# thanard/me-trpo

Measured on AMD Instinct MI355X. Metric: imagined env-steps/sec (KxBxH) over the full TRPO iteration, higher is better.
Workload: dtype f32

## Files before the change

include/metrpo.h:

```cpp
#ifndef METRPO_H
#define METRPO_H

#include <stddef.h>
#include <stdint.h>

#ifdef __cplusplus
extern "C" {
#endif

#define METRPO_ABI_VERSION 4
#define METRPO_MAX_LAYERS 6

typedef struct metrpo_ctx metrpo_ctx;

typedef enum {
    METRPO_OK = 0,
    METRPO_EINVAL = -1,
    METRPO_ENULL = -2,
    METRPO_EHIP = -3,
    METRPO_EUNSUPPORTED = -4,
    METRPO_ESTATE = -5,
    METRPO_UNSET = -100
} metrpo_status;

// ... 24 lines not shown
    int32_t pol_n_hidden;
    int32_t pol_hidden[METRPO_MAX_LAYERS];
} metrpo_dims;

int32_t metrpo_abi_version(void);
const char* metrpo_status_string(int32_t status);

int32_t metrpo_create(metrpo_ctx** out, int32_t device, const metrpo_dims* dims);
int32_t metrpo_destroy(metrpo_ctx* ctx);
int32_t metrpo_set_exclusive(metrpo_ctx* ctx, int32_t exclusive);
int32_t metrpo_set_option(metrpo_ctx* ctx, const char* key, const char* value);
int32_t metrpo_get_option(metrpo_ctx* ctx, const char* key, char* buf, int32_t cap);
const char* metrpo_option_name(int32_t index);
const char* metrpo_last_error(const metrpo_ctx* ctx);
int32_t metrpo_dyn_param_count(const metrpo_ctx* ctx);
int32_t metrpo_policy_param_count(const metrpo_ctx* ctx);

int32_t metrpo_set_dynamics(metrpo_ctx* ctx, const float* d_params, const float* d_in_mean,
                            const float* d_in_std, const float* d_diff_mean, const float* d_diff_std,
                            void* stream);
int32_t metrpo_set_policy(metrpo_ctx* ctx, const float* d_theta, void* stream);
int32_t metrpo_get_policy(metrpo_ctx* ctx, float* d_theta_out, void* stream);

int32_t metrpo_policy_actions(metrpo_ctx* ctx, const float* d_obs, const float* d_eps, int32_t B,
                              float* d_actions, float* d_mean, void* stream);
int32_t metrpo_step(metrpo_ctx* ctx, const float* d_s, const float* d_a, int32_t B, int32_t sam_mode,
                    const int32_t* d_model_idx, const float* d_noise, float* d_s_next, float* d_reward,
                    uint8_t* d_done, float* d_next_all, void* stream);

typedef struct {
    int32_t B, T, H;
    int32_t sam_mode;
    int32_t determ;
    int32_t eval_all_heads;
    const float* d_pool;
    int32_t n_pool;
    uint64_t seed;
    uint64_t stream_offset;
    const float* d_eps;
    const int32_t* d_model_idx;
    const float* d_sel_noise;
    const int32_t* d_reset_idx;
    const int32_t* d_reset_model;
    float* d_obs;
    float* d_act;
    float* d_rew;
    float* d_mean;
    uint8_t* d_done;
    int32_t* d_tpath;
    float* d_last_obs;
    int32_t t0;
    const float* d_init_obs;
    const int32_t* d_init_ts;
    const int32_t* d_init_model;
    int32_t* d_last_ts;
    int32_t* d_last_model;
    const int32_t* d_stop;
    int64_t stop_batch;
    const double* d_stop_cum;
} metrpo_rollout_args;
int32_t metrpo_rollout(metrpo_ctx* ctx, const metrpo_rollout_args* args, void* stream);
int32_t metrpo_last_rollout_kernel(const metrpo_ctx* ctx);
const char* metrpo_rollout_note(const metrpo_ctx* ctx);

typedef enum { METRPO_DYN_F32 = 0, METRPO_DYN_BF16 = 1 } metrpo_dyn_precision;
int32_t metrpo_set_dyn_precision(metrpo_ctx* ctx, int32_t precision);
int32_t metrpo_get_dyn_precision(const metrpo_ctx* ctx);

int32_t metrpo_sampler_progress(metrpo_ctx* ctx, const uint8_t* d_done, const int32_t* d_tpath, int32_t T, int32_t B,
                                int32_t t0, int64_t batch_size, double* d_counts, double* d_state, int32_t* d_stop,
                                void* stream);

int32_t metrpo_validation_cost(metrpo_ctx* ctx, const float* d_s0, int32_t Bv, int32_t T, double gamma,
                               double* d_costs, void* stream);

int32_t metrpo_gae(metrpo_ctx* ctx, const float* d_obs, const float* d_rew, const uint8_t* d_done,
                   const int32_t* d_tpath, int32_t T, int32_t B, const double* d_coeffs, double gamma,
                   double lam, float* d_adv, float* d_ret, uint8_t* d_valid, double* d_stats, void* stream);
int32_t metrpo_process_begin(metrpo_ctx* ctx, float* d_old_log_std, double* d_acc, int64_t n_acc, void* stream);
int32_t metrpo_center_advantages(metrpo_ctx* ctx, float* d_adv, const uint8_t* d_valid, int64_t N,
                                 const double* d_stats, void* stream);
int32_t metrpo_baseline_gram(metrpo_ctx* ctx, const float* d_obs, const float* d_ret, const int32_t* d_tpath,
                             const uint8_t* d_valid, int64_t N, double* d_AtA, double* d_Aty, void* stream);
int32_t metrpo_baseline_solve(metrpo_ctx* ctx, const double* d_AtA, const double* d_Aty, double reg_coeff, double* d_coeffs, void* stream);

typedef struct {
    const float* d_obs;
    const float* d_act;
    const float* d_adv;
    const float* d_old_mean;
    const float* d_old_log_std;
    int32_t old_log_std_stride;
    const uint8_t* d_valid;
    int64_t N;
    double inv_n_global;
} metrpo_batch;

int32_t metrpo_loss_grad(metrpo_ctx* ctx, const metrpo_batch* batch, double* d_out, void* stream);
int32_t metrpo_fvp(metrpo_ctx* ctx, const metrpo_batch* batch, const double* d_v, double* d_hv, void* stream);
int32_t metrpo_loss_kl(metrpo_ctx* ctx, const metrpo_batch* batch, const float* d_theta, double* d_out,
                       void* stream);

int32_t metrpo_vpg_loss_grad(metrpo_ctx* ctx, const metrpo_batch* batch, double* d_out, void* stream);
typedef struct {
    double lr, beta1, beta2, eps;
} metrpo_vpg_params;
int32_t metrpo_vpg_update(metrpo_ctx* ctx, const metrpo_batch* batch, const metrpo_vpg_params* params, double* d_loss, void* stream);

typedef struct {
    double clip_lr, entropy_bonus_coeff;
    double lr, beta1, beta2, eps;
} metrpo_ppo_params;
int32_t metrpo_ppo_loss_grad(metrpo_ctx* ctx, const metrpo_batch* batch, const metrpo_ppo_params* params, double* d_out, void* stream);
int32_t metrpo_ppo_update(metrpo_ctx* ctx, const metrpo_batch* batch, const metrpo_ppo_params* params, int32_t n_epochs, double* d_losses, void* stream);

typedef struct { double kl_penalty, step_size; } metrpo_ppo_kl_params;
int32_t metrpo_ppo_kl_loss_grad(metrpo_ctx* ctx, const metrpo_batch* batch, const metrpo_ppo_params* params, const metrpo_ppo_kl_params* kl,
                                const double* d_mean_kl, double* d_out, void* stream);
int32_t metrpo_ppo_kl_update(metrpo_ctx* ctx, const metrpo_batch* batch, const metrpo_ppo_params* params, const metrpo_ppo_kl_params* kl, int32_t n_epochs,
                             double* d_losses, double* d_mean_kls, void* stream);

#define METRPO_COMM_ID_BYTES 128
int32_t metrpo_comm_get_unique_id(void* id_out );
int32_t metrpo_comm_init(metrpo_ctx* ctx, const void* id , int32_t world, int32_t rank);
int32_t metrpo_comm_destroy(metrpo_ctx* ctx);
int32_t metrpo_allreduce_sum_f64(metrpo_ctx* ctx, double* d_buf, int64_t count, void* stream);

#define METRPO_COMM_IPC_BLOB_BYTES 128
int32_t metrpo_comm_ipc_export(metrpo_ctx* ctx, void* blob_out );
int32_t metrpo_comm_ipc_attach(metrpo_ctx* ctx, const void* blobs , int32_t world, int32_t rank);
int32_t metrpo_comm_ipc_detach(metrpo_ctx* ctx);
int32_t metrpo_comm_set_timeout_ms(metrpo_ctx* ctx, int64_t ms);
int32_t metrpo_comm_transport(const metrpo_ctx* ctx);
int32_t metrpo_comm_check(metrpo_ctx* ctx, void* stream);

typedef int32_t (*metrpo_allreduce_fn)(void* user, double* d_buf, int64_t count, void* stream);

typedef struct {
    double max_kl;
    int32_t cg_iters;
    double reg_coeff;
    double backtrack_ratio;
    int32_t max_backtracks;
    int32_t accept_violation;
    double residual_tol;
    metrpo_allreduce_fn allreduce;
    void* allreduce_user;
    int32_t explicit_final_hvp;
} metrpo_trpo_params;

typedef struct {
    double loss_before, loss, kl, beta;
    int32_t n_backtrack, accepted, cg_iters_run;
} metrpo_trpo_diag;

int32_t metrpo_trpo_update(metrpo_ctx* ctx, const metrpo_batch* batch, const metrpo_trpo_params* params,
                           metrpo_trpo_diag* diag, double* d_g_out, double* d_dir_out, void* stream);

int32_t metrpo_trpo_update_begin(metrpo_ctx* ctx, const metrpo_batch* batch, const metrpo_trpo_params* params, int32_t spec_trials,
                                 double* d_g_out, double* d_dir_out, void* stream);
int32_t metrpo_trpo_update_end(metrpo_ctx* ctx, metrpo_trpo_diag* diag, int32_t* late_out, void* stream);

int32_t metrpo_subsample_batch(metrpo_ctx* ctx, const metrpo_batch* batch, const int32_t* d_idx, int64_t m, double inv_n_global, metrpo_batch* out,
                               double* d_valid_count, void* stream);
int32_t metrpo_trpo_update_fvp(metrpo_ctx* ctx, const metrpo_batch* batch, const metrpo_batch* fvp_batch, const metrpo_trpo_params* params,
                               metrpo_trpo_diag* diag, double* d_g_out, double* d_dir_out, void* stream);
// ... 88 lines not shown
```

me-trpo_amd/_lib.py:

```python
import ctypes as C
import os

import torch

_HERE = os.path.dirname(os.path.abspath(__file__))
LIB_PATH = os.path.join(_HERE, "libmetrpo.so")
MAX_LAYERS = 6

ENV_IDS = {'swimmer': 0, 'half_cheetah': 1, 'half-cheetah': 1, 'ant': 2, 'humanoid': 3, 'hopper': 4, 'snake': 5}
SAM_MODES = {'step_rand': 0, 'eps_rand': 1, 'model_mean_std': 2, 'model_mean': 3, 'model_med': 4, 'one_model': 5}
DYN_PRECISIONS = {'f32': 0, 'bf16': 1}
ACTS = {'identity': 0, 'tf.identity': 0, 'relu': 1, 'tf.nn.relu': 1, 'tanh': 2, 'tf.nn.tanh': 2, 'tf.tanh': 2}


class Dims(C.Structure):
    _fields_ = [('env', C.c_int32), ('ns', C.c_int32), ('na', C.c_int32), ('n_models', C.c_int32),
                ('dyn_n_hidden', C.c_int32), ('dyn_hidden', C.c_int32 * MAX_LAYERS), ('dyn_act', C.c_int32 * MAX_LAYERS),
                ('n_drop', C.c_int32), ('pol_n_hidden', C.c_int32), ('pol_hidden', C.c_int32 * MAX_LAYERS)]


class RolloutArgs(C.Structure):
    _fields_ = [('B', C.c_int32), ('T', C.c_int32), ('H', C.c_int32), ('sam_mode', C.c_int32), ('determ', C.c_int32),
                ('eval_all_heads', C.c_int32), ('d_pool', C.c_void_p), ('n_pool', C.c_int32), ('seed', C.c_uint64),
                ('stream_offset', C.c_uint64), ('d_eps', C.c_void_p), ('d_model_idx', C.c_void_p),
# ... 21 lines not shown
                ('explicit_final_hvp', C.c_int32)]


class TrainParams(C.Structure):
    _fields_ = [('lr', C.c_double), ('beta1', C.c_double), ('beta2', C.c_double), ('eps', C.c_double),
                ('reg_constant', C.c_double), ('batch_size', C.c_int32)]


class TrpoDiag(C.Structure):
    _fields_ = [('loss_before', C.c_double), ('loss', C.c_double), ('kl', C.c_double), ('beta', C.c_double),
                ('n_backtrack', C.c_int32), ('accepted', C.c_int32), ('cg_iters_run', C.c_int32)]


class VpgParams(C.Structure):
    _fields_ = [('lr', C.c_double), ('beta1', C.c_double), ('beta2', C.c_double), ('eps', C.c_double)]


class PpoParams(C.Structure):
    _fields_ = [('clip_lr', C.c_double), ('entropy_bonus_coeff', C.c_double), ('lr', C.c_double), ('beta1', C.c_double), ('beta2', C.c_double),
                ('eps', C.c_double)]


class PpoKlParams(C.Structure):
    _fields_ = [('kl_penalty', C.c_double), ('step_size', C.c_double)]


class LbfgsOpts(C.Structure):
    _fields_ = [('m', C.c_int32), ('maxls', C.c_int32), ('maxiter', C.c_int32), ('maxfun', C.c_int32), ('ftol', C.c_double),
                ('gtol', C.c_double), ('lookahead', C.c_int32), ('round_f32', C.c_int32)]


class LbfgsResult(C.Structure):
    _fields_ = [('fun', C.c_double), ('nit', C.c_int32), ('nfev', C.c_int32), ('status', C.c_int32), ('task', C.c_int32),
                ('task_code', C.c_int32), ('pad_', C.c_int32)]


class ModelErrorArgs(C.Structure):
    _fields_ = [('d_Os', C.c_void_p), ('d_As', C.c_void_p), ('d_Rs', C.c_void_p), ('n', C.c_int32), ('T', C.c_int32),
                ('hs', C.POINTER(C.c_int32)), ('n_h', C.c_int32), ('model', C.c_int32), ('known_actions', C.c_int32), ('t0_only', C.c_int32),
                ('signed_diff', C.c_int32), ('d_state_diff', C.c_void_p), ('d_cost_diff', C.c_void_p), ('d_valid', C.c_void_p), ('d_sums', C.c_void_p),
                ('d_dbg_obs', C.c_void_p), ('d_dbg_rew', C.c_void_p), ('d_dbg_done', C.c_void_p), ('d_dbg_last_obs', C.c_void_p)]


class RolloutActionsArgs(C.Structure):
    _fields_ = [('B', C.c_int32), ('T', C.c_int32), ('sam_mode', C.c_int32), ('uniform_model', C.c_int32), ('force_step_loop', C.c_int32),
                ('d_init_obs', C.c_void_p), ('d_actions', C.c_void_p), ('d_model', C.c_void_p), ('d_model_idx', C.c_void_p), ('d_sel_noise', C.c_void_p),
                ('d_obs', C.c_void_p), ('d_rew', C.c_void_p), ('d_done', C.c_void_p)]


MODEL_ERROR_MAX_HORIZONS = 32


_P, _I, _L, _D = C.c_void_p, C.c_int32, C.c_int64, C.c_double
SYMBOLS = {
    'metrpo_abi_version': (_I, []),
    'metrpo_status_string': (C.c_char_p, [_I]),
    'metrpo_create': (_I, [C.POINTER(_P), _I, C.POINTER(Dims)]),
    'metrpo_destroy': (_I, [_P]),
    'metrpo_last_error': (C.c_char_p, [_P]),
    'metrpo_dyn_param_count': (_I, [_P]),
    'metrpo_policy_param_count': (_I, [_P]),
    'metrpo_set_dynamics': (_I, [_P, _P, _P, _P, _P, _P, _P]),
    'metrpo_set_policy': (_I, [_P, _P, _P]),
    'metrpo_get_policy': (_I, [_P, _P, _P]),
    'metrpo_policy_actions': (_I, [_P, _P, _P, _I, _P, _P, _P]),
    'metrpo_step': (_I, [_P, _P, _P, _I, _I, _P, _P, _P, _P, _P, _P, _P]),
    'metrpo_rollout': (_I, [_P, C.POINTER(RolloutArgs), _P]),
    'metrpo_comm_get_unique_id': (_I, [_P]),
    'metrpo_comm_init': (_I, [_P, _P, _I, _I]),
    'metrpo_comm_destroy': (_I, [_P]),
    'metrpo_allreduce_sum_f64': (_I, [_P, _P, _L, _P]),
    'metrpo_comm_ipc_export': (_I, [_P, _P]),
    'metrpo_comm_ipc_attach': (_I, [_P, _P, _I, _I]),
    'metrpo_comm_ipc_detach': (_I, [_P]),
    'metrpo_comm_set_timeout_ms': (_I, [_P, _L]),
    'metrpo_comm_transport': (_I, [_P]),
    'metrpo_comm_check': (_I, [_P, _P]),
    'metrpo_sampler_progress': (_I, [_P, _P, _P, _I, _I, _I, _L, _P, _P, _P, _P]),
    'metrpo_validation_cost': (_I, [_P, _P, _I, _I, _D, _P, _P]),
    'metrpo_gae': (_I, [_P, _P, _P, _P, _P, _I, _I, _P, _D, _D, _P, _P, _P, _P, _P]),
    'metrpo_process_begin': (_I, [_P, _P, _P, _L, _P]),
    'metrpo_center_advantages': (_I, [_P, _P, _P, _L, _P, _P]),
    'metrpo_baseline_gram': (_I, [_P, _P, _P, _P, _P, _L, _P, _P, _P]),
    'metrpo_baseline_solve': (_I, [_P, _P, _P, _D, _P, _P]),
    'metrpo_loss_grad': (_I, [_P, C.POINTER(Batch), _P, _P]),
    'metrpo_fvp': (_I, [_P, C.POINTER(Batch), _P, _P, _P]),
    'metrpo_loss_kl': (_I, [_P, C.POINTER(Batch), _P, _P, _P]),
    'metrpo_vpg_loss_grad': (_I, [_P, C.POINTER(Batch), _P, _P]),
    'metrpo_vpg_update': (_I, [_P, C.POINTER(Batch), C.POINTER(VpgParams), _P, _P]),
    'metrpo_ppo_loss_grad': (_I, [_P, C.POINTER(Batch), C.POINTER(PpoParams), _P, _P]),
    'metrpo_ppo_update': (_I, [_P, C.POINTER(Batch), C.POINTER(PpoParams), C.c_int32, _P, _P]),
    'metrpo_ppo_kl_loss_grad': (_I, [_P, C.POINTER(Batch), C.POINTER(PpoParams), C.POINTER(PpoKlParams), _P, _P, _P]),
    'metrpo_ppo_kl_update': (_I, [_P, C.POINTER(Batch), C.POINTER(PpoParams), C.POINTER(PpoKlParams), C.c_int32, _P, _P, _P]),
    'metrpo_trpo_update': (_I, [_P, C.POINTER(Batch), C.POINTER(TrpoParams), C.POINTER(TrpoDiag), _P, _P, _P]),
    'metrpo_trpo_update_begin': (_I, [_P, C.POINTER(Batch), C.POINTER(TrpoParams), _I, _P, _P, _P]),
    'metrpo_trpo_update_end': (_I, [_P, C.POINTER(TrpoDiag), C.POINTER(C.c_int32), _P]),
    'metrpo_subsample_batch': (_I, [_P, C.POINTER(Batch), _P, _L, _D, C.POINTER(Batch), _P, _P]),
    'metrpo_trpo_update_fvp': (_I, [_P, C.POINTER(Batch), C.POINTER(Batch), C.POINTER(TrpoParams), C.POINTER(TrpoDiag), _P, _P, _P]),
    'metrpo_trpo_update_fvp_begin': (_I, [_P, C.POINTER(Batch), C.POINTER(Batch), C.POINTER(TrpoParams), _I, _P, _P, _P]),
    'metrpo_model_error_windows': (_I, [_P, _P, _I, _I, _P, _P]),
    'metrpo_model_error': (_I, [_P, C.POINTER(ModelErrorArgs), _P]),
    'metrpo_rollout_actions': (_I, [_P, C.POINTER(RolloutActionsArgs), _P]),
    'metrpo_last_rollout_actions_kernel': (_I, [_P]),
    'metrpo_dyn_train_reset': (_I, [_P, _P]),
    'metrpo_dyn_train_step': (_I, [_P, _P, _P, C.POINTER(TrainParams), _P, _P]),
    'metrpo_dyn_eval_losses': (_I, [_P, _P, _P, _L, _D, _P, _P]),
    'metrpo_get_dynamics': (_I, [_P, _P, _P]),
    'metrpo_set_dynamics_model': (_I, [_P, _I, _P, _P]),
    'metrpo_set_normalizers': (_I, [_P, _P, _P, _P, _P, _P]),
    'metrpo_rms_accumulate': (_I, [_P, _P, _L, _I, _P, _P, _P]),
    'metrpo_bptt_grad': (_I, [_P, _P, _I, _I, _D, _P, _P, _P]),
    'metrpo_bptt_grad_stochastic': (_I, [_P, _P, _I, _I, _D, _P, C.c_uint64, _P, _P, _P, _P]),
    'metrpo_set_exclusive': (_I, [_P, _I]),
    'metrpo_set_option': (_I, [_P, C.c_char_p, C.c_char_p]),
    'metrpo_get_option': (_I, [_P, C.c_char_p, C.c_char_p, _I]),
    'metrpo_option_name': (C.c_char_p, [_I]),
    'metrpo_last_rollout_kernel': (_I, [_P]),
    'metrpo_rollout_note': (C.c_char_p, [_P]),
    'metrpo_set_dyn_precision': (_I, [_P, _I]),
    'metrpo_get_dyn_precision': (_I, [_P]),
    'metrpo_policy_adam_reset': (_I, [_P, _P]),
    'metrpo_policy_adam_step': (_I, [_P, _P, _D, _D, _D, _D, _D, _P]),
    'metrpo_lbfgs_begin': (_I, [_P, _I, _P, C.POINTER(LbfgsOpts), _P, _P]),
    'metrpo_lbfgs_iterate': (_I, [_P, _P, _P, _P, _P, _P]),
    'metrpo_lbfgs_get_result': (_I, [_P, C.POINTER(LbfgsResult), _P]),
    'metrpo_lbfgs_policy': (_I, [_P, _P, _I, _I, _D, C.POINTER(LbfgsOpts), C.POINTER(LbfgsResult), _P]),
    'metrpo_get_dyn_adam': (_I, [_P, _P, _P, C.POINTER(_L), _P]),
    'metrpo_set_dyn_adam': (_I, [_P, _P, _P, _L, _P]),
    'metrpo_get_policy_adam': (_I, [_P, _P, _P, C.POINTER(_L), _P]),
    'metrpo_set_policy_adam': (_I, [_P, _P, _P, _L, _P]),
}
EXTRA_SYMBOLS = {
    'metrpo_rollout_generic': (_I, [_P, C.POINTER(RolloutArgs), _P]),
    'metrpo_has_mfma_path': (_I, [_P]),
    'metrpo_set_update_path': (_I, [_P, _I]),
    'metrpo_update_path': (_I, [_P, _L]),
    'metrpo_set_rollout_variant': (_I, [_P, _I]),
    'metrpo_set_det_path': (_I, [_P, _I]),
    'metrpo_probe_peaks': (_I, [_P, _P, _P]),
    'metrpo_schedulable_cus': (_I, [_P, _P]),
    'metrpo_debug_fvp_us': (_I, [_P, _P, _P]),
    'metrpo_debug_last_update': (_I, [_P, _P]),
    'metrpo_debug_persist_stats': (_I, [_P, _P, _I, _P]),
    'metrpo_debug_ws_retired': (_I, [_P, _P, _I]),
}


def load():
    if not os.path.exists(LIB_PATH):
        raise ImportError("libmetrpo.so not found at %s -- build it with `python -c 'import __graft_entry__ as g; "
                          "g.build()'` (hipcc --offload-arch=gfx950); there is no CPU fallback" % LIB_PATH)
    lib = C.CDLL(LIB_PATH)
    for table in (SYMBOLS, EXTRA_SYMBOLS):
        for name, (res, args) in table.items():
            fn = getattr(lib, name)
            fn.restype, fn.argtypes = res, args
    if lib.metrpo_abi_version() != 4:
        raise ImportError("libmetrpo.so ABI version mismatch")
    return lib


lib = load()


class MetrpoError(RuntimeError):
    pass
# ... 9 lines not shown
```

me-trpo_amd/csrc/api.hip:

```cpp
#include "metrpo_internal.h"
#include <atomic>
#include <chrono>
#include <cstring>
#include "cg_device.h"
#include "trace.h"
#include <algorithm>
#include <cmath>
#include <cstring>
#include <mutex>
#include <new>

static std::mutex g_err_mutex;
int set_err(metrpo_ctx* c, int code, const std::string& msg) {
    if (c) { std::lock_guard<std::mutex> lock(g_err_mutex); c->err = msg; }
    return code;
}

extern "C" int32_t metrpo_abi_version(void) { return METRPO_ABI_VERSION; }

extern "C" const char* metrpo_status_string(int32_t s) {
    switch (s) {
    case METRPO_OK: return "ok";
    case METRPO_EINVAL: return "invalid argument";
    case METRPO_ENULL: return "null pointer";
// ... 370 lines not shown

extern "C" int32_t metrpo_sampler_progress(metrpo_ctx* c, const uint8_t* done, const int32_t* tpath, int32_t T, int32_t B, int32_t t0,
                                           int64_t batch_size, double* counts, double* state, int32_t* stop, void* stream) {
    if (!c) return METRPO_ENULL;
    if (!done || !tpath || !counts || !state || !stop) return set_err(c, METRPO_ENULL, "sampler_progress: NULL pointer");
    if (T < 0 || B < 0 || t0 < 0 || batch_size < 0) return set_err(c, METRPO_EINVAL, "sampler_progress: bad T/B/t0/batch_size");
    if (T == 0 || B == 0) return METRPO_OK;
    return launch_sampler_progress(c, done, tpath, T, B, t0, batch_size, counts, state, stop, (hipStream_t)stream);
}

extern "C" int32_t metrpo_rollout_generic(metrpo_ctx* c, const metrpo_rollout_args* a, void* stream) {
    if (!c) return METRPO_ENULL;
    if (!a) return set_err(c, METRPO_ENULL, "rollout: args NULL");
    NEED_DYN(c); NEED_POL(c);
    if (!sam_ok(a->sam_mode)) return set_err(c, METRPO_EINVAL, "sam mode is not defined");
    if (a->B <= 0 || a->T <= 0 || a->H <= 0 || a->n_pool <= 0) return set_err(c, METRPO_EINVAL, "rollout: bad B/T/H/n_pool");
    if (!a->d_pool || !a->d_obs || !a->d_act || !a->d_rew || !a->d_mean || !a->d_done || !a->d_tpath)
        return set_err(c, METRPO_ENULL, "rollout: required pointer is NULL");
    return launch_rollout_generic(c, a, (hipStream_t)stream);
}
extern "C" int32_t metrpo_has_mfma_path(const metrpo_ctx* c) { return (c && c->mfma_cfg >= 0) ? 1 : 0; }
extern "C" int32_t metrpo_set_rollout_variant(metrpo_ctx* c, int32_t v) {
    if (!c) return METRPO_ENULL;
    c->rollout_variant = v;
    return (v != 1 && (c->coop_cfg >= 0 || (v == 0 && c->coop_pad_cfg >= 0))) ? 2 : (c->mfma_cfg >= 0 ? 1 : (gemm_path_applicable(c) ? 3 : 0));
}
extern "C" int32_t metrpo_update_path(const metrpo_ctx* c, int64_t N) {
    if (!c) return METRPO_ENULL;
    return policy_gemm_applicable(c, N, false) ? 2 : ((c->pol_mfma >= 0 || f3_active(c, false)) ? 1 : 0);
}
extern "C" int32_t metrpo_set_update_path(metrpo_ctx* c, int32_t use_mfma) {
    if (!c) return METRPO_ENULL;
    c->pol_path = (use_mfma == 2) ? 2 : (use_mfma ? 1 : 0);
    c->pol_mfma = (use_mfma == 1) ? policy_mfma_select(c->pd) : -1;
    c->pol_f3 = (use_mfma == 1) ? policy_f3_select(c->pd) : 0;
    c->pg_fwd_rows = -1; c->f3_rows = -1;
    return (c->pol_mfma >= 0 || f3_active(c, false)) ? 1 : (c->pol_path == 2 ? 2 : 0);
}

extern "C" int32_t metrpo_validation_cost(metrpo_ctx* c, const float* s0, int32_t Bv, int32_t T, double gamma,
                                          double* costs, void* stream) {
    TraceRange trace_("metrpo:validation_cost");
    if (!c) return METRPO_ENULL;
    NEED_DYN(c); NEED_POL(c);
    if (!s0 || !costs) return set_err(c, METRPO_ENULL, "validation_cost: NULL pointer");
    if (Bv <= 0 || T < 0) return set_err(c, METRPO_EINVAL, "validation_cost: bad Bv/T");
    return launch_validation_cost(c, s0, Bv, T, gamma, costs, (hipStream_t)stream);
}

extern "C" int32_t metrpo_gae(metrpo_ctx* c, const float* obs, const float* rew, const uint8_t* done,
                              const int32_t* tpath, int32_t T, int32_t B, const double* coeffs, double gamma, double lam,
                              float* adv, float* ret, uint8_t* valid, double* stats, void* stream) {
    TraceRange trace_("metrpo:process_samples:gae");
    if (!c) return METRPO_ENULL;
    if (!obs || !rew || !done || !tpath || !adv || !ret || !valid || !stats) return set_err(c, METRPO_ENULL, "gae: NULL pointer");
    if (T < 0 || B < 0) return set_err(c, METRPO_EINVAL, "gae: bad T/B");
    if (T == 0 || B == 0) return METRPO_OK;
    return launch_gae(c, obs, rew, done, tpath, T, B, coeffs, gamma, lam, adv, ret, valid, stats, (hipStream_t)stream);
}

extern "C" int32_t metrpo_process_begin(metrpo_ctx* c, float* old_log_std, double* acc, int64_t n_acc, void* stream) {
    TraceRange trace_("metrpo:process_samples:begin");
    if (!c) return METRPO_ENULL;
    if (n_acc < 0 || n_acc > (1LL << 30) || (n_acc > 0 && !acc)) return set_err(c, METRPO_EINVAL, "process_begin: bad accumulator range");
    if (!old_log_std && n_acc == 0) return METRPO_OK;
    return launch_process_begin(c, old_log_std, n_acc > 0 ? acc : nullptr, n_acc, (hipStream_t)stream);
}

extern "C" int32_t metrpo_center_advantages(metrpo_ctx* c, float* adv, const uint8_t* valid, int64_t N,
                                            const double* stats, void* stream) {
    TraceRange trace_("metrpo:process_samples:center");
    if (!c) return METRPO_ENULL;
    if (!adv || !stats) return set_err(c, METRPO_ENULL, "center: NULL pointer");
    if (N <= 0) return METRPO_OK;
    return launch_center(c, adv, valid, N, stats, (hipStream_t)stream);
}

extern "C" int32_t metrpo_baseline_gram(metrpo_ctx* c, const float* obs, const float* ret, const int32_t* tpath,
                                        const uint8_t* valid, int64_t N, double* AtA, double* Aty, void* stream) {
    TraceRange trace_("metrpo:process_samples:baseline_gram");
    if (!c) return METRPO_ENULL;
    if (!obs || !ret || !tpath || !AtA || !Aty) return set_err(c, METRPO_ENULL, "gram: NULL pointer");
    if (N <= 0) return METRPO_OK;
    return launch_gram(c, obs, ret, tpath, valid, N, AtA, Aty, (hipStream_t)stream);
}

extern "C" int32_t metrpo_baseline_solve(metrpo_ctx* c, const double* AtA, const double* Aty, double reg_coeff, double* coeffs, void* stream) {
    TraceRange trace_("metrpo:process_samples:baseline_solve");
    if (!c) return METRPO_ENULL;
    if (!AtA || !Aty || !coeffs) return set_err(c, METRPO_ENULL, "baseline_solve: NULL pointer");
    if (!(reg_coeff >= 0.0)) return set_err(c, METRPO_EINVAL, "baseline_solve: reg_coeff must be >= 0");
    return launch_baseline_solve(c, AtA, Aty, reg_coeff, coeffs, (hipStream_t)stream);
}

extern "C" int32_t metrpo_loss_grad(metrpo_ctx* c, const metrpo_batch* b, double* out, void* stream) {
    if (!c) return METRPO_ENULL;
    NEED_POL(c);
    if (!out) return set_err(c, METRPO_ENULL, "loss_grad: out NULL");
    return launch_loss_grad(c, b, out, (hipStream_t)stream);
}
extern "C" int32_t metrpo_vpg_loss_grad(metrpo_ctx* c, const metrpo_batch* b, double* out, void* stream) {
    if (!c) return METRPO_ENULL;
    if (!out) return set_err(c, METRPO_ENULL, "vpg_loss_grad: out NULL");
    NEED_POL(c);
    return launch_vpg_loss_grad(c, b, out, (hipStream_t)stream);
}
extern "C" int32_t metrpo_vpg_update(metrpo_ctx* c, const metrpo_batch* b, const metrpo_vpg_params* pr, double* d_loss, void* stream) {
    if (!c) return METRPO_ENULL;
    if (!pr) return set_err(c, METRPO_ENULL, "vpg_update: params NULL");
    NEED_POL(c);
    if (c->upd_pending) return set_err(c, METRPO_ESTATE, "vpg_update: a TRPO update is still open (metrpo_trpo_update_end first)");
    return run_vpg_update(c, b, pr, d_loss, (hipStream_t)stream);
}
extern "C" int32_t metrpo_ppo_loss_grad(metrpo_ctx* c, const metrpo_batch* b, const metrpo_ppo_params* pr, double* out, void* stream) {
    if (!c) return METRPO_ENULL;
    if (!pr) return set_err(c, METRPO_ENULL, "ppo_loss_grad: params NULL");
    if (!out) return set_err(c, METRPO_ENULL, "ppo_loss_grad: out NULL");
    NEED_POL(c);
    return launch_ppo_loss_grad(c, b, pr, out, (hipStream_t)stream);
}
extern "C" int32_t metrpo_ppo_update(metrpo_ctx* c, const metrpo_batch* b, const metrpo_ppo_params* pr, int32_t n_epochs, double* d_losses, void* stream) {
    if (!c) return METRPO_ENULL;
    if (!pr) return set_err(c, METRPO_ENULL, "ppo_update: params NULL");
    NEED_POL(c);
    if (c->upd_pending) return set_err(c, METRPO_ESTATE, "ppo_update: a TRPO update is still open (metrpo_trpo_update_end first)");
    return run_ppo_update(c, b, pr, n_epochs, d_losses, (hipStream_t)stream);
}
extern "C" int32_t metrpo_ppo_kl_loss_grad(metrpo_ctx* c, const metrpo_batch* b, const metrpo_ppo_params* pr, const metrpo_ppo_kl_params* kp, const double* d_mean_kl,
                                           double* out, void* stream) {
    if (!c) return METRPO_ENULL;
    if (!pr || !kp) return set_err(c, METRPO_ENULL, "ppo_kl_loss_grad: params NULL");
    if (!out) return set_err(c, METRPO_ENULL, "ppo_kl_loss_grad: out NULL");
    NEED_POL(c);
    return launch_ppo_kl_loss_grad(c, b, pr, kp, d_mean_kl, out, (hipStream_t)stream);
}
extern "C" int32_t metrpo_ppo_kl_update(metrpo_ctx* c, const metrpo_batch* b, const metrpo_ppo_params* pr, const metrpo_ppo_kl_params* kp, int32_t n_epochs, double* d_losses,
                                        double* d_mean_kls, void* stream) {
    if (!c) return METRPO_ENULL;
    if (!pr || !kp) return set_err(c, METRPO_ENULL, "ppo_kl_update: params NULL");
    NEED_POL(c);
    if (c->upd_pending) return set_err(c, METRPO_ESTATE, "ppo_kl_update: a TRPO update is still open (metrpo_trpo_update_end first)");
    return run_ppo_kl_update(c, b, pr, kp, n_epochs, d_losses, d_mean_kls, (hipStream_t)stream);
}
static int lbfgs_opts_check(metrpo_ctx* c, const metrpo_lbfgs_opts* o, const char* who) {
    if (!o) return set_err(c, METRPO_ENULL, std::string(who) + ": opts NULL");
    if (o->m <= 0 || o->maxls <= 0) return set_err(c, METRPO_EINVAL, std::string(who) + ": m and maxls must be positive");
    if (!(o->ftol >= 0.0) || !(o->gtol >= 0.0)) return set_err(c, METRPO_EINVAL, std::string(who) + ": ftol and gtol must be >= 0");
    return METRPO_OK;
}
extern "C" int32_t metrpo_lbfgs_begin(metrpo_ctx* c, int32_t n, const double* x0, const metrpo_lbfgs_opts* o, double* x_eval, void* stream) {
    if (!c) return METRPO_ENULL;
    if (!x0 || !x_eval) return set_err(c, METRPO_ENULL, "lbfgs_begin: NULL pointer");
    if (n <= 0) return set_err(c, METRPO_EINVAL, "lbfgs_begin: n must be positive");
    int rc;
    if ((rc = lbfgs_opts_check(c, o, "lbfgs_begin"))) return rc;
    return lbfgs_begin(c, n, x0, nullptr, o, x_eval, (hipStream_t)stream);
}
extern "C" int32_t metrpo_lbfgs_iterate(metrpo_ctx* c, const double* f, const double* g, double* x_eval, int32_t* task, void* stream) {
    if (!c) return METRPO_ENULL;
    if (!f || !g || !x_eval || !task) return set_err(c, METRPO_ENULL, "lbfgs_iterate: NULL pointer");
    if (!c->lb_open) return set_err(c, METRPO_ESTATE, "lbfgs_iterate: no minimisation open (metrpo_lbfgs_begin first)");
    return lbfgs_iterate(c, f, g, x_eval, task, (hipStream_t)stream);
}
extern "C" int32_t metrpo_lbfgs_get_result(metrpo_ctx* c, metrpo_lbfgs_result* out, void* stream) {
    if (!c) return METRPO_ENULL;
    if (!out) return set_err(c, METRPO_ENULL, "lbfgs_get_result: out NULL");
    if (!c->lb_open) return set_err(c, METRPO_ESTATE, "lbfgs_get_result: no minimisation open (metrpo_lbfgs_begin first)");
// ... 536 lines not shown
```

me-trpo_amd/csrc/cg_device.h:

```cpp
#pragma once
#include "metrpo_internal.h"
#ifndef CG_MARK
#define CG_MARK(i)
#endif

enum { S_RDOTR = 0, S_DONE = 1, S_BETA = 2, S_XHX = 3, S_ITERS = 4, S_LOSS0 = 5, S_COMMERR = 6, S_ROLLERR = 7 };

struct CgTail {
    int op;
    int P, last;
    int implicit_hd;
    double reg, tol, max_kl;
    double *x, *r, *p, *z, *step, *scal;
    const double* gout;
    float* pf;
    const int* vpos; float* imgval;
    unsigned int* ticket;
    double* ls;
    const double* lk;
    float* th; const float* th_try;
    int trial, accept_violation;
    double* pub_dst;
    unsigned long long pub_stamp;
    float* nx_try = nullptr; const float* nx_prev = nullptr; double nx_ratio = 1.0; double* nx_ls = nullptr;
};

struct PfOut {
    float* pf; const int* vpos; float* imgval;
    __device__ __forceinline__ void put(int i, float v) const { pf[i] = v; if (vpos != nullptr) { const int q = vpos[i]; if (q >= 0) imgval[q] = v; } }
};
__device__ __forceinline__ void cg_init_body(int P, const double* gout, double* x, double* r, double* p, PfOut pf, double* scal, double* sh);

template <int CTRL> __device__ __forceinline__ double dpp_add_f64(double v) {
    const long long b = __double_as_longlong(v);
    const int lo = __builtin_amdgcn_update_dpp(0, (int)b, CTRL, 0xF, 0xF, true), hi = __builtin_amdgcn_update_dpp(0, (int)(b >> 32), CTRL, 0xF, 0xF, true);
    return v + __longlong_as_double(((long long)hi << 32) | (unsigned int)lo);
}
__device__ __forceinline__ double wave_sum_f64(double v) {
    v = dpp_add_f64<0xB1>(v); v = dpp_add_f64<0x4E>(v); v = dpp_add_f64<0x141>(v); v = dpp_add_f64<0x140>(v);
    const long long b = __double_as_longlong(v);
    double t = 0.0;
#pragma unroll
    for (int r = 0; r < 4; ++r) {
        const int lo = __builtin_amdgcn_readlane((int)b, 16 * r), hi = __builtin_amdgcn_readlane((int)(b >> 32), 16 * r);
        t += __longlong_as_double(((long long)hi << 32) | (unsigned int)lo);
    }
    return t;
}
__device__ __forceinline__ double blk_sum(double v, double* sh) {
    v = wave_sum_f64(v);
    const int w = threadIdx.x >> 6, l = threadIdx.x & 63;
    __syncthreads();
    if (l == 0) sh[w] = v;
    __syncthreads();
    double r = 0.0;
    const int nw = (blockDim.x + 63) >> 6;
    for (int i = 0; i < nw; ++i) r += sh[i];
    return r;
}

__device__ __forceinline__ void cg_finish_implicit(int P, double max_kl, const double* x, const double* r, const double* g,
                                                   double* step, double* scal, double* sh) {
    double acc = 0.0;
    for (int i = threadIdx.x; i < P; i += blockDim.x) acc += x[i] * (g[i] - r[i]);
    const double xhx = blk_sum(acc, sh);
    double beta = sqrt(2.0 * max_kl * (1.0 / (xhx + 1e-8)));
    if (isnan(beta)) beta = 1.0;
    for (int i = threadIdx.x; i < P; i += blockDim.x) step[i] = beta * x[i];
    if (threadIdx.x == 0) { scal[S_BETA] = beta; scal[S_XHX] = xhx; }
}

__device__ __forceinline__ void cg_init_body(int P, const double* gout, double* x, double* r, double* p, PfOut pf, double* scal, double* sh) {
    double acc = 0.0;
    for (int i = threadIdx.x; i < P; i += blockDim.x) {
        const double g = gout[1 + i];
        x[i] = 0.0; r[i] = g; p[i] = g; pf.put(i, (float)g);
        acc += g * g;
    }
    const double rdotr = blk_sum(acc, sh);
    if (threadIdx.x == 0) { scal[S_RDOTR] = rdotr; scal[S_DONE] = 0.0; scal[S_ITERS] = 0.0; scal[S_LOSS0] = gout[0]; }
}

constexpr int CG_R = 2;
constexpr int CG_RBIG = 13;
struct CgPre { double pv[CG_R], rv[CG_R], xv[CG_R], done, rdotr; bool have; };
__device__ __forceinline__ void cg_prefetch(const CgTail& t, CgPre& pre) {
    pre.have = (t.op == 1 && t.P <= CG_R * (int)blockDim.x);
    if (!pre.have) return;
    pre.done = t.scal[S_DONE]; pre.rdotr = t.scal[S_RDOTR];
// ... 17 lines not shown
            pv[j] = zv[j] = rv[j] = xv[j] = 0.0;
            const int ic = (i < P) ? i : P - 1;
            const double pl = pf_ ? 0.0 : p[ic], rl = pf_ ? 0.0 : r[ic], xl = pf_ ? 0.0 : x[ic], zl = z[ic];
            if (i < P) {
                if (pf_) { pv[j] = pre->pv[j < CG_R ? j : 0]; rv[j] = pre->rv[j < CG_R ? j : 0]; xv[j] = pre->xv[j < CG_R ? j : 0]; } else { pv[j] = pl; rv[j] = rl; xv[j] = xl; }
                zv[j] = zl + reg * pv[j]; acc += pv[j] * zv[j];
            }
        }
        CG_MARK(5)
        const double pz = blk_sum(acc, sh);
        CG_MARK(6)
        const double v = rdotr / pz;
        acc = 0.0;
#pragma unroll
        for (int j = 0; j < R; ++j) { xv[j] += v * pv[j]; rv[j] -= v * zv[j]; acc += rv[j] * rv[j]; }
        const double newrdotr = blk_sum(acc, sh);
        CG_MARK(7)
        const double mu = newrdotr / rdotr;
#pragma unroll
        for (int j = 0; j < R; ++j) {
            const int i = threadIdx.x + j * blockDim.x;
            if (i < P) {
                const double pn = rv[j] + mu * pv[j];
                z[i] = zv[j]; x[i] = xv[j]; r[i] = rv[j]; p[i] = pn;
                pf.put(i, last ? (float)xv[j] : (float)pn);
            }
        }
        __syncthreads();
        if (threadIdx.x == 0) {
            scal[S_RDOTR] = newrdotr;
            scal[S_ITERS] += 1.0;
            if (newrdotr < tol) scal[S_DONE] = 1.0;
        }
        }

__device__ __forceinline__ void cg_step_body(int P, double reg, double tol, int last, double* x, double* r, double* p, double* z,
                                             PfOut pf, double* scal, double* sh, const CgPre* pre = nullptr) {
    const bool pf_ = (pre != nullptr && pre->have);
    if ((pf_ ? pre->done : scal[S_DONE]) != 0.0) {
        if (last) for (int i = threadIdx.x; i < P; i += blockDim.x) pf.put(i, (float)x[i]);
        return;
    }
    const double rdotr = pf_ ? pre->rdotr : scal[S_RDOTR];
    if (P <= CG_R * (int)blockDim.x) { cg_step_regs<CG_R>(P, reg, tol, last, x, r, p, z, pf, scal, sh, rdotr, pre); return; }
    if (P <= 4 * (int)blockDim.x) { cg_step_regs<4>(P, reg, tol, last, x, r, p, z, pf, scal, sh, rdotr, nullptr); return; }
    if (P <= CG_RBIG * (int)blockDim.x) { cg_step_regs<CG_RBIG>(P, reg, tol, last, x, r, p, z, pf, scal, sh, rdotr, nullptr); return; }
    double acc = 0.0;
    for (int i = threadIdx.x; i < P; i += blockDim.x) { const double zi = z[i] + reg * p[i]; z[i] = zi; acc += p[i] * zi; }
    const double pz = blk_sum(acc, sh);
    const double v = rdotr / pz;
    acc = 0.0;
    for (int i = threadIdx.x; i < P; i += blockDim.x) {
        x[i] += v * p[i];
        const double ri = r[i] - v * z[i];
        r[i] = ri;
        acc += ri * ri;
    }
    const double newrdotr = blk_sum(acc, sh);
    const double mu = newrdotr / rdotr;
    for (int i = threadIdx.x; i < P; i += blockDim.x) {
        const double pn = r[i] + mu * p[i];
        p[i] = pn;
        pf.put(i, last ? (float)x[i] : (float)pn);
    }
    __syncthreads();
    if (threadIdx.x == 0) {
        scal[S_RDOTR] = newrdotr;
        scal[S_ITERS] += 1.0;
        if (newrdotr < tol) scal[S_DONE] = 1.0;
    }
}

__device__ __forceinline__ void cg_finish_body(int P, double reg, double max_kl, const double* x, double* z, double* step,
                                               double* scal, double* sh) {
    double acc = 0.0;
    for (int i = threadIdx.x; i < P; i += blockDim.x) acc += x[i] * (z[i] + reg * x[i]);
    const double xhx = blk_sum(acc, sh);
    double beta = sqrt(2.0 * max_kl * (1.0 / (xhx + 1e-8)));
    if (isnan(beta)) beta = 1.0;
    for (int i = threadIdx.x; i < P; i += blockDim.x) step[i] = beta * x[i];
    if (threadIdx.x == 0) { scal[S_BETA] = beta; scal[S_XHX] = xhx; }
}

__device__ __forceinline__ void ls_decide(const CgTail& t) {
    const double loss = t.lk[0], kl = t.lk[1], lb = t.scal[S_LOSS0];
    if (loss < lb && kl <= t.max_kl) {
        const bool acc = !(isnan(loss) || isnan(kl) || loss >= lb || kl >= t.max_kl) || t.accept_violation != 0;
        if (acc) for (int i = threadIdx.x; i < t.P; i += blockDim.x) t.th[i] = t.th_try[i];
        if (threadIdx.x == 0) { t.ls[0] = (double)t.trial; t.ls[1] = loss; t.ls[2] = kl; t.ls[3] = acc ? 1.0 : 0.0; }
    } else if (threadIdx.x == 0) { t.ls[1] = loss; t.ls[2] = kl; }
}

__device__ __forceinline__ void ls_next_theta(const CgTail& t) {
    for (int i = threadIdx.x; i < t.P; i += blockDim.x) t.nx_try[i] = (float)((double)t.nx_prev[i] - t.nx_ratio * t.step[i]);
}
__device__ __forceinline__ void ls_open_and_first_theta(const CgTail& t) {
    if (t.nx_try == nullptr) return;
    __syncthreads();
    if (t.nx_ls != nullptr && threadIdx.x == 0) { t.nx_ls[0] = -1.0; t.nx_ls[1] = NAN; t.nx_ls[2] = NAN; t.nx_ls[3] = 0.0; }
    ls_next_theta(t);
}

__device__ __forceinline__ void ls_publish(const double* __restrict__ src, double* dst, unsigned long long stamp) {
    if (threadIdx.x >= 64) return;
    if (threadIdx.x < 14) __hip_atomic_store(dst + threadIdx.x, src[threadIdx.x], __ATOMIC_RELAXED, __HIP_MEMORY_SCOPE_SYSTEM);
    asm volatile("s_waitcnt vmcnt(0)" ::: "memory");
    if (threadIdx.x == 0) __hip_atomic_store((unsigned long long*)(dst + 16), stamp, __ATOMIC_RELAXED, __HIP_MEMORY_SCOPE_SYSTEM);
}

__device__ __forceinline__ void cg_tail_run(const CgTail& t, double* sh, const CgPre* pre = nullptr) {
    if (t.op == 1) {
        cg_step_body(t.P, t.reg, t.tol, t.last, t.x, t.r, t.p, t.z, PfOut{t.pf, t.vpos, t.imgval}, t.scal, sh, pre);
        if (t.last && t.implicit_hd) {
            __syncthreads();
            cg_finish_implicit(t.P, t.max_kl, t.x, t.r, t.gout + 1, t.step, t.scal, sh);
            ls_open_and_first_theta(t);
        }
    } else if (t.op == 2) { cg_finish_body(t.P, t.reg, t.max_kl, t.x, t.z, t.step, t.scal, sh); ls_open_and_first_theta(t); }
    else if (t.op == 3) cg_init_body(t.P, t.gout, t.x, t.r, t.p, PfOut{t.pf, t.vpos, t.imgval}, t.scal, sh);
    else if (t.op == 4) {
        ls_decide(t);
        if (t.nx_try != nullptr && !(t.lk[0] < t.scal[S_LOSS0] && t.lk[1] <= t.max_kl)) ls_next_theta(t);
        if (t.pub_dst != nullptr) { asm volatile("s_waitcnt vmcnt(0)" ::: "memory"); __syncthreads(); ls_publish(t.scal, t.pub_dst, t.pub_stamp); }
    }
}
```

me-trpo_amd/csrc/metrpo_internal.h:

```cpp
#pragma once
#include <hip/hip_runtime.h>
#include <stdint.h>
#include <string>
#include <atomic>
#include <utility>
#include <vector>
#include "metrpo.h"
#include "xchg_device.h"

#define MAXL (METRPO_MAX_LAYERS + 1)
#define WAVE 64

struct NetDesc {
    int n_layers;
    int dims[MAXL + 1];
    int act[MAXL];
    int w_off[MAXL];
    int b_off[MAXL];
    int n_params;
    int api_w_off[MAXL];
    int api_b_off[MAXL];
    int api_n_params;
    int max_width;
};
// ... 131 lines not shown
struct RolloutK {
    int B, T, H, sam_mode, determ, eval_all, n_pool;
    uint64_t seed, stream_offset;
    const float* pool;
    const float* eps;
    const int32_t* model_idx;
    const float* sel_noise;
    const int32_t* reset_idx;
    const int32_t* reset_model;
    float* obs; float* act; float* rew; float* mean; uint8_t* done; int32_t* tpath; float* last_obs;
    int t0; const float* init_obs; const int32_t* init_ts; const int32_t* init_model;
    int32_t* last_ts; int32_t* last_model; const int32_t* stop;
    long long stop_batch; const double* stop_cum;
    int32_t* mig_flag; float* mig_obs; int32_t* mig_ts; int32_t* mig_model; int mig_epoch; double* mig_err;
    int vB, vR;
};
#define RK_ENV(r, b) ((r).vB ? (b) % (r).vB : (b))
#define RK_TOFF(r, b) ((r).vB ? ((b) / (r).vB) * (r).H : 0)
#define RK_STRIDE(r) ((r).vB ? (r).vB : (r).B)
#define RK_LAST_ROUND(r, b) (!(r).vB || (b) / (r).vB == (r).vR - 1)

static inline RolloutK make_rollout_k(const metrpo_rollout_args* a) {
    RolloutK r;
    r.B = a->B; r.T = a->T; r.H = a->H; r.sam_mode = a->sam_mode; r.determ = a->determ; r.eval_all = a->eval_all_heads;
    r.n_pool = a->n_pool; r.seed = a->seed; r.stream_offset = a->stream_offset; r.pool = a->d_pool; r.eps = a->d_eps;
    r.model_idx = a->d_model_idx; r.sel_noise = a->d_sel_noise; r.reset_idx = a->d_reset_idx;
    r.reset_model = a->d_reset_model; r.obs = a->d_obs; r.act = a->d_act; r.rew = a->d_rew; r.mean = a->d_mean;
    r.done = a->d_done; r.tpath = a->d_tpath; r.last_obs = a->d_last_obs;
    r.t0 = a->t0; r.init_obs = a->d_init_obs; r.init_ts = a->d_init_ts; r.init_model = a->d_init_model;
    r.last_ts = a->d_last_ts; r.last_model = a->d_last_model; r.stop = a->d_stop;
    r.stop_batch = a->stop_batch; r.stop_cum = a->d_stop_cum;
    r.mig_flag = nullptr; r.mig_obs = nullptr; r.mig_ts = nullptr; r.mig_model = nullptr; r.mig_epoch = 0; r.mig_err = nullptr;
    r.vB = 0; r.vR = 0;
    return r;
}

struct PolK {
    const float* obs; const float* act; const float* adv; const float* old_mean; const float* old_ls;
    int ls_stride;
    float clip_lo;
    const uint8_t* valid; long long N; float inv_n;
    float clip_hi;
    const float* gm;
    const int* img_map;
    const double* skip;
    float* imgval;
    float* hcache;
    const double* mean_kl; double kl_delta; float kl_beta;
};

enum UpdOp {
    OP_GRAD = 0,
    OP_FVP = 1,
    OP_LOSSKL = 2,
    OP_FVPC = 3,
    OP_VPG = 4,
    OP_PPO = 5,
    OP_PPOKL = 6,
};
struct SolveScope {
    bool cache_activations = false;
    bool publish_image = false;
    bool exchange_in_tail = false;
};
struct CgTail;
struct AdamTail;
struct UpdCall {
    UpdOp op;
    PolK k;
    const float* theta;
    const float* vf;
    const double* v64;
    double* out;
    const CgTail* tail;
    const AdamTail* adam;
    double ent_coeff;
    bool ent_in_reduction;
    SolveScope scope;
};

int policy_mfma_select(const ProblemDesc& pd);
int policy_mfma_image_buffers(metrpo_ctx*);
int policy_mfma_launch(metrpo_ctx*, const UpdCall&, float* partials, int nblocks, hipStream_t);

#define HIP_TRY(c, expr)                                                                      \
    do {                                                                                      \
        hipError_t _e = (expr);                                                               \
        if (_e != hipSuccess)                                                                 \
            return set_err((c), METRPO_EHIP, std::string(#expr) + ": " + hipGetErrorString(_e)); \
    } while (0)

int launch_policy_actions(metrpo_ctx*, const float*, const float*, int, float*, float*, hipStream_t);
int launch_step(metrpo_ctx*, const float*, const float*, int, int, const int32_t*, const float*, float*, float*,
                uint8_t*, float*, hipStream_t);
int launch_rollout_generic(metrpo_ctx*, const metrpo_rollout_args*, hipStream_t);
bool gemm_path_applicable(const metrpo_ctx*);
int sched_cus(metrpo_ctx*, hipStream_t);
bool grid_is_coresident(metrpo_ctx*, const void* kernel, int threads, size_t lds, long long grid, hipStream_t);
int launch_rollout_gemm(metrpo_ctx*, const metrpo_rollout_args*, hipStream_t);
struct Bf16Img { int Kp[MAXL]; size_t off[MAXL]; size_t per_head; };
Bf16Img bf16_img_layout(const ProblemDesc&);
int launch_bf16_dyn_image(metrpo_ctx*, hipStream_t);
size_t bf16_hidden_floats(const ProblemDesc&, int B);
int launch_bf16_layers(metrpo_ctx*, const float* X, int ldx, void* HA, void* HB, float* OUT, int B, hipStream_t);
int launch_rollout_resident(metrpo_ctx*, const metrpo_rollout_args*, hipStream_t);
struct BpttNoise {
    const float* eps;
    const float* log_std;
    int* n_sat;
    unsigned long long seed;
    int T;
};
int launch_bptt_grad(metrpo_ctx*, const float* init, int B, int T, double gamma, double* costs, double* grad, hipStream_t, const BpttNoise* nz = nullptr);
int launch_policy_adam(metrpo_ctx*, const double* grad, double lr, double b1, double b2, double eps, double clip_val, bool reset, hipStream_t);
int ensure_policy_adam(metrpo_ctx*);
int ensure_dyn_adam(metrpo_ctx*);
size_t dyn_adam_floats(const metrpo_ctx*);
int det_mfma_select(const metrpo_ctx*);
int launch_det_forward(metrpo_ctx*, int idx, const float* s0, int B, int T, double gamma, float* XS, float* WT, double* part, double* costs, hipStream_t,
                       const BpttNoise* nz = nullptr);
int launch_det_backward(metrpo_ctx*, int idx, int B, int T, const float* XS, const float* WT, float* GM, hipStream_t, const BpttNoise* nz = nullptr);
int ensure_detpart(metrpo_ctx*, int B);
int ensure_detpart_n(metrpo_ctx*, size_t n_doubles);
int launch_det_cost_reduce(metrpo_ctx*, int n_part, const double* part, double* costs, hipStream_t, const double* err = nullptr);
int launch_validation_resident(metrpo_ctx*, const float* s0, int Bv, int T, double gamma, double* costs, hipStream_t);
bool det_gemm_applicable(const metrpo_ctx*);
int launch_dg_forward(metrpo_ctx*, const float* s0, int B, int T, double gamma, float* XS, float* WT, double* costs, hipStream_t,
                      const BpttNoise* nz = nullptr);
int launch_dg_backward(metrpo_ctx*, int B, int T, const float* XS, const float* WT, float* GM, hipStream_t, const BpttNoise* nz = nullptr);
int launch_policy_vjp(metrpo_ctx*, const float* obs, const float* gm, long long N, double* out, hipStream_t);
int launch_dyn_train_step(metrpo_ctx*, const float*, const float*, const metrpo_train_params*, double*, hipStream_t);
int launch_dyn_eval_losses(metrpo_ctx*, const float*, const float*, long long, double, double*, hipStream_t);
int launch_rms_accumulate(metrpo_ctx*, const float*, long long, int, double*, double*, hipStream_t);
int launch_rollout_mfma(metrpo_ctx*, const metrpo_rollout_args*, hipStream_t, int* coop = nullptr);
int mfma_prepare_dynamics(metrpo_ctx*, hipStream_t);
int mfma_prepare_policy(metrpo_ctx*, hipStream_t);
int mfma_select_config(metrpo_ctx*);
int mfma_shape_config(const metrpo_ctx*);
int coop_select_config(metrpo_ctx*);
int launch_rollout_coop(metrpo_ctx*, int idx, const RolloutK&, hipStream_t, bool padded = false);
int launch_pad_dyn(metrpo_ctx*, hipStream_t);
int launch_validation_cost(metrpo_ctx*, const float*, int, int, double, double*, hipStream_t);
int launch_gae(metrpo_ctx*, const float*, const float*, const uint8_t*, const int32_t*, int, int, const double*,
               double, double, float*, float*, uint8_t*, double*, hipStream_t);
int launch_center(metrpo_ctx*, float*, const uint8_t*, int64_t, const double*, hipStream_t);
int launch_process_begin(metrpo_ctx*, float*, double*, int64_t, hipStream_t);
int launch_sampler_progress(metrpo_ctx*, const uint8_t*, const int32_t*, int, int, int, long long, double*, double*, int32_t*, hipStream_t);
int launch_baseline_solve(metrpo_ctx*, const double* AtA, const double* Aty, double reg, double* coeffs, hipStream_t);
int launch_gram(metrpo_ctx*, const float*, const float*, const int32_t*, const uint8_t*, int64_t, double*, double*,
                hipStream_t);
int launch_loss_grad(metrpo_ctx*, const metrpo_batch*, double*, hipStream_t, const CgTail* tail = nullptr, SolveScope = {});
int launch_vpg_loss_grad(metrpo_ctx*, const metrpo_batch*, double* out, hipStream_t);
int run_vpg_update(metrpo_ctx*, const metrpo_batch*, const metrpo_vpg_params*, double* d_loss, hipStream_t);
int launch_ppo_loss_grad(metrpo_ctx*, const metrpo_batch*, const metrpo_ppo_params*, double* out, hipStream_t);
int run_ppo_update(metrpo_ctx*, const metrpo_batch*, const metrpo_ppo_params*, int n_epochs, double* d_losses, hipStream_t);
int launch_ppo_kl_loss_grad(metrpo_ctx*, const metrpo_batch*, const metrpo_ppo_params*, const metrpo_ppo_kl_params*, const double* d_mean_kl, double* out, hipStream_t);
int run_ppo_kl_update(metrpo_ctx*, const metrpo_batch*, const metrpo_ppo_params*, const metrpo_ppo_kl_params*, int n_epochs, double* d_losses, double* d_mean_kls, hipStream_t);
int lbfgs_begin(metrpo_ctx*, int n, const double* x0, const float* x0_f32, const metrpo_lbfgs_opts*, double* x_eval, hipStream_t);
int lbfgs_iterate(metrpo_ctx*, const double* f, const double* g, double* x_eval, int32_t* task, hipStream_t);
int lbfgs_get_result(metrpo_ctx*, metrpo_lbfgs_result*, hipStream_t);
int run_lbfgs_policy(metrpo_ctx*, const float* init, int B, int T, double gamma, const metrpo_lbfgs_opts*, metrpo_lbfgs_result*, hipStream_t);
int comm_allreduce_f64(metrpo_ctx*, double* buf, long long count, hipStream_t);
XchgK xchg_next(metrpo_ctx*);
static inline XchgK xchg_none() { XchgK x = {}; return x; }
static inline double* comm_err_cell(metrpo_ctx* c) { return c->d_cg.p + (size_t)(1 + c->pd.P) + 5 * (size_t)c->pd.P + 6; }
static inline double* val_err_cell(metrpo_ctx* c) { return comm_err_cell(c) + 8; }
static inline double* sub_err_cell(metrpo_ctx* c) { return comm_err_cell(c) + 9; }
static inline int rollout_error_seen(metrpo_ctx* c, hipStream_t st) {
    (void)hipMemsetAsync(comm_err_cell(c) + 1, 0, sizeof(double), st);
    const bool was_resident = (c->last_rollout_kernel == 4);
    if (was_resident) c->res_failed = 1;
    if (c->last_rollout_kernel == 6) {
        c->persist_failed = 1;
        return set_err(c, METRPO_EHIP, "rollout: the persistent stream-K kernel's wait for a row block timed out (a workgroup of its grid never ran: is another process using "
                                       "this GPU?); the trajectories of that launch are invalid, later rollouts of this context use the launch-per-step path");
    }
    return set_err(c, METRPO_EHIP, was_resident ? "rollout: the resident kernel's hand-over timed out (a workgroup of its grid never ran: is another process using this GPU?); "
                                                  "the trajectories of that launch are invalid, later rollouts of this context use the step-wise path"
                                                : "rollout: a migrating tile's hand-over timed out (producer workgroup never ran); trajectories are invalid");
}
bool policy_gemm_applicable(const metrpo_ctx*, long long N, bool vjp);
struct UpdFusion {
    bool fused;
    bool exchange_in_tail;
    bool finalize_reduces;
    bool carries_next_step() const { return fused && finalize_reduces; }
};
static inline UpdFusion update_fusion(const metrpo_ctx* c, long long N, bool has_callback) {
    const bool xg = !has_callback && c->xg_world > 1;
    UpdFusion f;
    f.finalize_reduces = !policy_gemm_applicable(c, N, false);
    f.exchange_in_tail = xg && f.finalize_reduces && c->pd.P + 1 <= c->xg_cap;
    f.fused = !has_callback && ((c->nccl_comm == nullptr && !xg) || f.exchange_in_tail);
    return f;
}
int policy_f3_select(const ProblemDesc& pd);
int policy_f3_launch(metrpo_ctx*, const UpdCall&, float* partials, int nblocks, hipStream_t);
int policy_gemm_run(metrpo_ctx*, const UpdCall&, hipStream_t);
int launch_fvp(metrpo_ctx*, const metrpo_batch*, const double*, double*, hipStream_t);
int launch_fvp_tail(metrpo_ctx*, const metrpo_batch*, const float* vf, const double* v, double* hv, const CgTail* tail, hipStream_t, SolveScope = {});
int launch_loss_kl(metrpo_ctx*, const metrpo_batch*, const float*, double*, hipStream_t, const CgTail* decide = nullptr, SolveScope = {});
int run_trpo_update(metrpo_ctx*, const metrpo_batch*, const metrpo_trpo_params*, metrpo_trpo_diag*, double*,
                    double*, hipStream_t, int phase = 0, int spec = 0, const metrpo_batch* fvp_batch = nullptr);
int launch_window_starts(metrpo_ctx*, const float* Os, int n, int T, int Tw, float* init_obs, hipStream_t);
int run_model_error(metrpo_ctx*, const metrpo_model_error_args*, hipStream_t);
int run_rollout_actions(metrpo_ctx*, const metrpo_rollout_actions_args*, hipStream_t);
int launch_subsample(metrpo_ctx*, const metrpo_batch* b, const int32_t* d_idx, long long m, double inv_n_global, metrpo_batch* out, double* d_valid_count, hipStream_t);
```

me-trpo_amd/csrc/policy_mfma.hip:

```cpp
#include <type_traits>
#include "device_common.h"
#include "cg_device.h"

typedef float f32x4 __attribute__((ext_vector_type(4)));
typedef float f32x2 __attribute__((ext_vector_type(2)));
#define PKFMA(a, b, c) __builtin_elementwise_fma((a), (b), (c))
#define MFMA16(a, b, c) __builtin_amdgcn_mfma_f32_16x16x4f32((a), (b), (c), 0, 0, 0)
#define PART_EXTRA 3
#ifndef POL_SKIP
#define POL_SKIP 0
#endif
#ifndef POL_SPLIT_R
#define POL_SPLIT_R 13
#endif
#ifndef POL_SPLIT_R_FVP
#define POL_SPLIT_R_FVP 7
#endif
#ifndef NWAVES
#define NWAVES 8
#endif
constexpr int cdiv_(int a, int b) { return (a + b - 1) / b; }
static_assert(POL_SPLIT_R == 0 || (NWAVES == 8 && (POL_SPLIT_R & 1) == 1 && POL_SPLIT_R >= 3 && (POL_SPLIT_R_FVP & 1) == 1 && POL_SPLIT_R_FVP >= 3), "the uneven deal pairs wave w with wave w + 4");
#ifdef POL_TIMING
__device__ unsigned long long g_pol_phase[16][8];
#define PT_MARK(i) { if (MODE_ == OP_FVPC && blockIdx.x == 0 && lane == 0) g_pol_phase[wave][i] = __builtin_readcyclecounter(); }
extern "C" int32_t metrpo_debug_pol_phases(unsigned long long* out) { return hipMemcpyFromSymbol(out, HIP_SYMBOL(g_pol_phase), sizeof(unsigned long long) * 128) == hipSuccess ? 0 : -1; }
#else
#define PT_MARK(i)
#endif


__device__ __forceinline__ void wave_sync_lds() {
    __builtin_amdgcn_fence(__ATOMIC_SEQ_CST, "wavefront");
    __builtin_amdgcn_wave_barrier();
}
__device__ __forceinline__ float xsum_q(float v) {
    typedef unsigned u32x2_ __attribute__((ext_vector_type(2)));
    const u32x2_ a = __builtin_amdgcn_permlane16_swap(__float_as_uint(v), __float_as_uint(v), false, false);
    const float s = __uint_as_float(a[0]) + __uint_as_float(a[1]);
    const u32x2_ b = __builtin_amdgcn_permlane32_swap(__float_as_uint(s), __float_as_uint(s), false, false);
    return __uint_as_float(b[0]) + __uint_as_float(b[1]);
}
template <int CTRL> __device__ __forceinline__ float dpp_add(float v) {
    return v + __int_as_float(__builtin_amdgcn_update_dpp(0, __float_as_int(v), CTRL, 0xF, 0xF, true));
}
__device__ __forceinline__ float xsum_c(float v) {
    v = dpp_add<0xB1>(v); v = dpp_add<0x4E>(v); v = dpp_add<0x141>(v); v = dpp_add<0x140>(v);
    return v;
}


template <int NS, int NA, int PH>
struct PolImg {
    static constexpr int NS_KS = cdiv_(NS, 4), HB = cdiv_(PH, 16), KK = HB * 4;
    static constexpr int O_W0F = 0, O_W1F = O_W0F + NS_KS * 64 * HB, O_V0F = O_W1F + KK * 64 * HB, O_V1F = O_V0F + NS_KS * 64 * HB,
                         O_W2B = O_V1F + KK * 64 * HB, O_W1B = O_W2B + 4 * 64 * HB, O_W2F = O_W1B + KK * 64 * HB,
                         O_V2F = O_W2F + KK * 64, TOTAL = O_V2F + KK * 64;
};


template <int NS, int NA, int PH, int MODE_>
__device__ __forceinline__ void pol_body(const PolK& k, const float* __restrict__ theta, const float* __restrict__ v, float* __restrict__ partials) {
    using I = PolImg<NS, NA, PH>;
    constexpr bool CACHED = (MODE_ == OP_FVPC), VPG = (MODE_ == OP_VPG), PPOKL = (MODE_ == OP_PPOKL), PPO = (MODE_ == OP_PPO) || PPOKL;
    constexpr int MODE = CACHED ? OP_FVP : (VPG || PPO) ? OP_GRAD : MODE_;
    constexpr int NS_KS = I::NS_KS, NSI = cdiv_(NS, 16), HB = I::HB, KK = I::KK;
    constexpr int pW0 = 0, pb0 = NS * PH, pW1 = pb0 + PH, pb1 = pW1 + PH * PH, pW2 = pb1 + PH, pb2 = pW2 + PH * NA,
                  pLS = pb2 + NA, P = pLS + NA, ROW = P + PART_EXTRA;
    constexpr int TS = 20, TILE = 16 * TS;
    constexpr int WTL = (3 * HB + (NA <= 2 ? 0 : 1)) * TILE;
    extern __shared__ __attribute__((aligned(16))) float lds[];
    const int tid = threadIdx.x, lane = tid & 63, wave = __builtin_amdgcn_readfirstlane(tid >> 6);
    const int c = lane & 15, q = lane >> 4;
    if (MODE_ == OP_LOSSKL && k.skip != nullptr && k.skip[0] >= 0.0) return;
    float* IMG = lds;
    float* TL = lds + I::TOTAL + wave * WTL;
    PT_MARK(0)
    const long long ntiles = (k.N + 15) / 16;
    const f32x4* __restrict__ hc = (const f32x4*)k.hcache;
    const bool ols_const = !VPG && (MODE != OP_FVP) && k.ls_stride == 0 && k.old_ls != nullptr;
    struct TileIn {
        float xB[NS_KS]; float xTs[4][NSI]; float ols[4], omu[4], act[4], adv; f32x4 gmv; int vld, nrem; f32x4 h[2 * HB];
    };
    auto fetch = [&](long long tile_, TileIn& in) {
        const long long tile = (tile_ < ntiles) ? tile_ : ntiles - 1;
        const long long n0 = tile * 16;
        const int nrem = (int)((k.N - n0 < 16) ? k.N - n0 : 16);
        in.nrem = nrem;
        const int cl = (c < nrem) ? c : nrem - 1;
        const float* __restrict__ ob = k.obs + n0 * NS;
#pragma unroll
        for (int s = 0; s < NS_KS; ++s) { const int f = 4 * s + q; in.xB[s] = ob[cl * NS + ((f < NS) ? f : NS - 1)]; }
        if (MODE != OP_LOSSKL) {
#pragma unroll
            for (int s = 0; s < 4; ++s) {
                const int sl = 4 * q + s, slc = (sl < nrem) ? sl : nrem - 1;
#pragma unroll
                for (int ci = 0; ci < NSI; ++ci) { const int f = 16 * ci + c; in.xTs[s][ci] = ob[slc * NS + ((f < NS) ? f : NS - 1)]; }
            }
        }
        in.vld = (k.valid == nullptr) ? 1 : (int)k.valid[n0 + cl];
        if (MODE != OP_FVP) {
            const long long nl = n0 + cl;
            if (MODE == OP_GRAD && k.gm != nullptr) {
#pragma unroll
                for (int r = 0; r < 4; ++r) { const int d = 4 * q + r; in.gmv[r] = k.gm[nl * NA + ((d < NA) ? d : NA - 1)]; }
            } else {
#pragma unroll
                for (int r = 0; r < 4; ++r) {
                    const int d = 4 * q + r, dc = (d < NA) ? d : NA - 1;
                    if (VPG) { in.act[r] = k.act[nl * NA + dc]; continue; }
                    in.ols[r] = ols_const ? 0.f : k.old_ls[(size_t)nl * k.ls_stride + dc]; in.omu[r] = k.old_mean[nl * NA + dc]; in.act[r] = k.act[nl * NA + dc];
                }
                in.adv = k.adv[nl];
            }
        }
        if (CACHED) {
            const f32x4* __restrict__ hb_ = hc + tile * (2 * HB) * 64;
#pragma unroll
            for (int j = 0; j < 2 * HB; ++j) in.h[j] = hb_[j * 64 + lane];
        }
    };
    auto mask_tile = [&](TileIn& in) {
#pragma unroll
        for (int s = 0; s < NS_KS; ++s) if (4 * s + 3 >= NS && 4 * s + q >= NS) in.xB[s] = 0.f;
        if (in.nrem == 16) return;
        const bool inr = c < in.nrem;
#pragma unroll
        for (int s = 0; s < NS_KS; ++s) if (!inr) in.xB[s] = 0.f;
#pragma unroll
        for (int s = 0; s < 4; ++s)
#pragma unroll
            for (int ci = 0; ci < NSI; ++ci) if (4 * q + s >= in.nrem) in.xTs[s][ci] = 0.f;
        if (!inr) { in.vld = 0; in.adv = 0.f; }
#pragma unroll
        for (int r = 0; r < 4; ++r) if (!inr) { in.ols[r] = 0.f; in.omu[r] = 0.f; in.act[r] = 0.f; in.gmv[r] = 0.f; }
    };
    TileIn nxt;

#define FRAG2(off, row, cb) IMG[(off) + ((row) * 64 + lane) * HB + (cb)]
#define FRAG1(off, row) IMG[(off) + (row) * 64 + lane]
    f32x4 b0f[HB], b1f[HB], b2f;
#pragma unroll
    for (int cb = 0; cb < HB; ++cb)
#pragma unroll
        for (int r = 0; r < 4; ++r) { const int u = 16 * cb + 4 * q + r; b0f[cb][r] = (u < PH) ? theta[pb0 + u] : 0.f; b1f[cb][r] = (u < PH) ? theta[pb1 + u] : 0.f; }
#pragma unroll
    for (int r = 0; r < 4; ++r) b2f[r] = (4 * q + r < NA) ? theta[pb2 + 4 * q + r] : 0.f;
    float ls[4], inv_std[4];
#pragma unroll
    for (int r = 0; r < 4; ++r) { ls[r] = (4 * q + r < NA) ? fmaxf(theta[pLS + 4 * q + r], LOG_MIN_STD) : 0.f; inv_std[r] = expf(-ls[r]); }
    float fisher_w[4];
#pragma unroll
    for (int r = 0; r < 4; ++r) fisher_w[r] = 1.0f / (expf(2.f * ls[r]) + 0.5f * KL_EPS);
    float ols_c[4] = {0.f, 0.f, 0.f, 0.f}, eo_c[4] = {1.f, 1.f, 1.f, 1.f}, os2_c[4] = {1.f, 1.f, 1.f, 1.f};
    if (ols_const) {
#pragma unroll
// ... 369 lines not shown
            for (int ci = 0; ci < HB; ++ci)
#pragma unroll
                for (int cj = 0; cj < HB; ++cj) gW1[ci][cj] = MFMA16(a0_[ci], b1_[cj], gW1[ci][cj]);
#pragma unroll
            for (int ci = 0; ci < NSI; ++ci)
#pragma unroll
                for (int cj = 0; cj < HB; ++cj) gW0[ci][cj] = MFMA16(xT[ci], b0_[cj], gW0[ci][cj]);
        }
        wave_sync_lds();
    }
#undef FRAG2
#undef FRAG1

    PT_MARK(3)
    __syncthreads();
    PT_MARK(4)
    float* RB = lds;
    float* row = RB + wave * ROW;
    if (MODE != OP_GRAD && lane < NA) row[pLS + lane] = 0.f;
    wave_sync_lds();
    if (MODE != OP_LOSSKL) {
#pragma unroll
        for (int r = 0; r < 4; ++r) {
#pragma unroll
            for (int cj = 0; cj < HB; ++cj) {
                const int j = 16 * cj + c;
#pragma unroll
                for (int ci = 0; ci < NSI; ++ci) { const int i = 16 * ci + 4 * q + r; if (i < NS && j < PH) row[pW0 + i * PH + j] = gW0[ci][cj][r]; }
#pragma unroll
                for (int ci = 0; ci < HB; ++ci) { const int i = 16 * ci + 4 * q + r; if (i < PH && j < PH) row[pW1 + i * PH + j] = gW1[ci][cj][r]; }
            }
            if (L2V) {
#pragma unroll
                for (int ci = 0; ci < HB; ++ci)
#pragma unroll
                    for (int d = 0; d < NAV; ++d) {
                        const float sg = xsum_c(gw2l[ci][r][d]);
                        const int i = 16 * ci + 4 * q + r;
                        if (c == 0 && i < PH) row[pW2 + i * NA + d] = sg;
                    }
            } else {
#pragma unroll
                for (int ci = 0; ci < HB; ++ci) { const int i = 16 * ci + 4 * q + r; if (i < PH && c < NA) row[pW2 + i * NA + c] = gW2[ci][r]; }
            }
#pragma unroll
            for (int cb = 0; cb < HB; ++cb) {
                const float s1 = xsum_c(gb1[cb][r]);
                const int u = 16 * cb + 4 * q + r;
                if (c == 0 && u < PH) row[pb1 + u] = s1;
            }
            if (r == 0) {
#pragma unroll
                for (int cb = 0; cb < HB; ++cb) {
                    const float s0 = xsum_q((gb0[cb][0] + gb0[cb][1]) + (gb0[cb][2] + gb0[cb][3]));
                    if (q == 0 && 16 * cb + c < PH) row[pb0 + 16 * cb + c] = s0;
                }
            }
            const float s2 = xsum_c(gb2[r]), sl = xsum_c(dls[r]);
            if (c == 0 && 4 * q + r < NA) {
                row[pb2 + 4 * q + r] = s2;
                if (MODE == OP_GRAD) row[pLS + 4 * q + r] = (theta[pLS + 4 * q + r] > LOG_MIN_STD) ? sl : 0.f;
            }
        }
    }
    if (PPO) {
        acc1 = 0.f;
        if (blockIdx.x == 0 && wave == 0 && c == 0) {
            acc1 = (q == 0) ? NA * ENTROPY_CONST : 0.f;
#pragma unroll
            for (int r = 0; r < 4; ++r) if (4 * q + r < NA) acc1 += ls[r];
        }
    }
    {
        const float a0 = xsum_c(xsum_q(acc0)), a1 = xsum_c(xsum_q(acc1)), aw = xsum_c(xsum_q(accw));
        if (lane == 0) { row[P] = a0; row[P + 1] = a1; row[P + 2] = aw; }
    }
    __syncthreads();
    PT_MARK(5)
    float* out = partials + (size_t)blockIdx.x * ROW;
    for (int i = (MODE == OP_LOSSKL ? P : 0) + tid; i < ROW; i += NWAVES * 64) {
        float a = 0.f;
#pragma unroll
        for (int w = 0; w < NWAVES; w += 4) a += (RB[w * ROW + i] + RB[(w + 1) * ROW + i]) + (RB[(w + 2) * ROW + i] + RB[(w + 3) * ROW + i]);
        out[i] = a;
    }
    PT_MARK(6)
}

template <int NS, int NA, int PH, int MODE_>
__global__ void __launch_bounds__(NWAVES * 64, 1) k_policy_mfma(PolK k, const float* __restrict__ theta, const float* __restrict__ v,
                                                        float* __restrict__ partials) {
    if constexpr (MODE_ == OP_PPOKL) {
        if (!ppo_kl_open(k.mean_kl, k.kl_delta)) { pol_body<NS, NA, PH, OP_PPO>(k, theta, v, partials); return; }
    }
    pol_body<NS, NA, PH, MODE_>(k, theta, v, partials);
}


template <int NS, int NA, int PH>
static void pol_image_map(std::vector<int>& map) {
    using I = PolImg<NS, NA, PH>;
    constexpr int HB = I::HB;
    constexpr int pW0 = 0, pb0 = NS * PH, pW1 = pb0 + PH, pb1 = pW1 + PH * PH, pW2 = pb1 + PH;
    const int VFLAG = 0x40000000;
    map.assign(I::TOTAL, -1);
    for (int i = 0; i < I::TOTAL; ++i) {
        int m = -1;
        if (i < I::O_W2F) {
            int t, base;
            if (i < I::O_W1F) { t = 0; base = I::O_W0F; } else if (i < I::O_V0F) { t = 1; base = I::O_W1F; }
            else if (i < I::O_V1F) { t = 2; base = I::O_V0F; } else if (i < I::O_W2B) { t = 3; base = I::O_V1F; }
            else if (i < I::O_W1B) { t = 4; base = I::O_W2B; } else { t = 5; base = I::O_W1B; }
            const int j = i - base, cb = j % HB, ln = (j / HB) & 63, row = j / (HB * 64), cc = ln & 15, qq = ln >> 4;
            const int flag = (t == 2 || t == 3) ? VFLAG : 0;
            if (t == 0 || t == 2) { const int in = 4 * row + qq, o = 16 * cb + cc; if (in < NS && o < PH) m = (pW0 + in * PH + o) | flag; }
            else if (t == 1 || t == 3) { const int in = 16 * (row >> 2) + 4 * qq + (row & 3), o = 16 * cb + cc; if (in < PH && o < PH) m = (pW1 + in * PH + o) | flag; }
            else if (t == 4) { const int ii = 16 * cb + cc, d = 4 * qq + row; if (ii < PH && d < NA) m = pW2 + ii * NA + d; }
            else { const int ii = 16 * cb + cc, jj = 16 * (row >> 2) + 4 * qq + (row & 3); if (ii < PH && jj < PH) m = pW1 + ii * PH + jj; }
        } else {
            const bool isv = i >= I::O_V2F;
            const int j = i - (isv ? I::O_V2F : I::O_W2F), ln = j & 63, row = j >> 6, cc = ln & 15, qq = ln >> 4;
            const int in = 16 * (row >> 2) + 4 * qq + (row & 3);
            if (in < PH && cc < NA) m = (pW2 + in * NA + cc) | (isv ? VFLAG : 0);
        }
        map[i] = m;
    }
}

typedef void (*pol_kernel_t)(PolK, const float*, const float*, float*);
struct PolEntry { int ns, na, ph; pol_kernel_t kern[7] ; int lds_floats, lds_floats_eval; void (*build_map)(std::vector<int>&); };
template <int NS, int NA, int PH> constexpr int pol_lds() {
    constexpr int HB = cdiv_(PH, 16);
    constexpr int a = PolImg<NS, NA, PH>::TOTAL + NWAVES * (3 * HB + (NA <= 2 ? 0 : 1)) * 16 * 20;
    constexpr int P = NS * PH + PH + PH * PH + PH + PH * NA + NA + NA;
    constexpr int b = NWAVES * (P + PART_EXTRA);
    return a > b ? a : b;
}
template <int NS, int NA, int PH> constexpr int pol_lds_eval() {
    constexpr int P = NS * PH + PH + PH * PH + PH + PH * NA + NA + NA;
    constexpr int a = PolImg<NS, NA, PH>::TOTAL, b = NWAVES * (P + PART_EXTRA);
    return a > b ? a : b;
}
#define PENTRY(NS, NA, PH) {NS, NA, PH, {k_policy_mfma<NS, NA, PH, OP_GRAD>, k_policy_mfma<NS, NA, PH, OP_FVP>, k_policy_mfma<NS, NA, PH, OP_LOSSKL>, k_policy_mfma<NS, NA, PH, OP_FVPC>, k_policy_mfma<NS, NA, PH, OP_VPG>, k_policy_mfma<NS, NA, PH, OP_PPO>, k_policy_mfma<NS, NA, PH, OP_PPOKL>}, pol_lds<NS, NA, PH>(), pol_lds_eval<NS, NA, PH>(), pol_image_map<NS, NA, PH>}
static const PolEntry kPol[] = {
    PENTRY(10, 2, 32),
    PENTRY(18, 6, 32),
    PENTRY(11, 3, 32),
    PENTRY(14, 4, 32),
    PENTRY(29, 8, 32),
};

int policy_mfma_select(const ProblemDesc& pd) {
    if (pd.pol.n_layers != 3 || pd.pol.dims[1] != pd.pol.dims[2]) return -1;
    for (int i = 0; i < (int)(sizeof(kPol) / sizeof(kPol[0])); ++i)
        if (kPol[i].ns == pd.ns && kPol[i].na == pd.na && kPol[i].ph == pd.pol.dims[1]) return i;
    return -1;
}

int policy_mfma_image_buffers(metrpo_ctx* c) {
    const int idx = c->pol_mfma;
    if (idx < 0) return set_err(c, METRPO_EUNSUPPORTED, "no MFMA policy kernels for this shape");
    if (c->pol_img_idx == idx) return METRPO_OK;
    const PolEntry& en = kPol[idx];
    std::vector<int> map;
    en.build_map(map);
    std::vector<int> vpos((size_t)c->pd.P, -1);
    for (size_t i = 0; i < map.size(); ++i)
        if (map[i] >= 0 && (map[i] & 0x40000000)) {
            const int j = map[i] & 0x3FFFFFFF;
            if (j >= c->pd.P || vpos[j] != -1) return set_err(c, METRPO_EINVAL, "policy image map: tangent entry out of range or stored twice");
            vpos[j] = (int)i;
        }
    c->pol_img_idx = -1;
    int rc;
    if ((rc = ws_grow(c, c->d_pol_img, sizeof(int) * map.size())) || (rc = ws_grow(c, c->d_pol_vpos, sizeof(int) * vpos.size())) ||
        (rc = ws_grow(c, c->d_pol_imgval, sizeof(float) * map.size())))
        return rc;
    HIP_TRY(c, hipMemcpy(c->d_pol_img.p, map.data(), sizeof(int) * map.size(), hipMemcpyHostToDevice));
    HIP_TRY(c, hipMemcpy(c->d_pol_vpos.p, vpos.data(), sizeof(int) * vpos.size(), hipMemcpyHostToDevice));
    HIP_TRY(c, hipMemset(c->d_pol_imgval.p, 0, sizeof(float) * map.size()));
    c->pol_img_idx = idx;
    return METRPO_OK;
}

int policy_mfma_launch(metrpo_ctx* c, const UpdCall& u, float* partials, int nblocks, hipStream_t st) {
    const PolEntry& en = kPol[c->pol_mfma];
    { const int rc = policy_mfma_image_buffers(c); if (rc) return rc; }
    PolK k = u.k;
    int mode = u.op;
    k.img_map = (const int*)c->d_pol_img.p;
    k.hcache = nullptr;
    const bool cached = u.scope.cache_activations && (mode == OP_GRAD || mode == OP_FVP) && k.gm == nullptr;
    k.imgval = (u.scope.publish_image && cached) ? c->d_pol_imgval.p : nullptr;
    if (cached) {
        const size_t need = (size_t)((k.N + 15) / 16) * 2 * (size_t)cdiv_(en.ph, 16) * 64 * 4;
        { const int rc = ws_grow(c, c->d_hcache, need * sizeof(float)); if (rc) return rc; }
        k.hcache = c->d_hcache.p;
        if (mode == OP_FVP) mode = OP_FVPC;
    }
    size_t sh = sizeof(float) * (size_t)en.lds_floats;
    if (mode == OP_LOSSKL) sh = sizeof(float) * (size_t)en.lds_floats_eval;
    if (sh > 64 * 1024) HIP_TRY(c, hipFuncSetAttribute((const void*)en.kern[mode], hipFuncAttributeMaxDynamicSharedMemorySize, (int)sh));
    hipLaunchKernelGGL(en.kern[mode], dim3(nblocks), dim3(NWAVES * 64), sh, st, k, u.theta, u.vf, partials);
    HIP_TRY(c, hipGetLastError());
    return METRPO_OK;
}
```

me-trpo_amd/csrc/policy_update.hip:

```cpp
#include "device_common.h"
#ifdef FIN_TIMING
__device__ unsigned long long g_fin_phase[512][8];
#define CG_MARK(i) { if (threadIdx.x == 0 && blockIdx.x < 512) g_fin_phase[blockIdx.x][i] = __builtin_readcyclecounter(); }
#endif
#include "cg_device.h"



__device__ __forceinline__ int hrow(const NetDesc& net, int l) {
    int o = 0;
    for (int i = 0; i < l; ++i) o += net.dims[i];
    return o;
}

template <int PT>
__device__ __forceinline__ void forward_store(const NetDesc& net, const float* __restrict__ th, float* H, float* DM, int tid) {
    constexpr int PLD = PT + 1;
    for (int l = 0; l < net.n_layers; ++l) {
        float* dst = (l == net.n_layers - 1) ? DM : (H + hrow(net, l + 1) * PLD);
        dense_col(th + net.w_off[l], th + net.b_off[l], net.dims[l], net.dims[l + 1], net.act[l], H + hrow(net, l) * PLD,
                  dst, PLD, tid);
    }
}

// ... 186 lines not shown
                dst[(j0 + jj) * PLD + tid] = o;
            }
    }
}

template <int PT>
__global__ void __launch_bounds__(PT) k_fvp(ProblemDesc pd, PolK k, const float* __restrict__ theta, const float* __restrict__ v,
                                            float* __restrict__ partials) {
    constexpr int PLD = PT + 1;
    extern __shared__ __attribute__((aligned(16))) float lds[];
    __shared__ double red[16];
    const NetDesc& net = pd.pol;
    const int tid = threadIdx.x, ns = pd.ns, na = pd.na, P = pd.P, L = net.n_layers;
    int hrows = 0;
    for (int l = 0; l < L; ++l) hrows += net.dims[l];
    float* H = lds;
    float* DM = H + hrows * PLD;
    float* dH = DM + na * PLD;
    float* part = partials + (size_t)blockIdx.x * (P + PART_EXTRA);
    for (int p = tid; p < P + PART_EXTRA; p += PT) part[p] = 0.0f;
    const float* __restrict__ raw_ls = theta + net.n_params;
    double wsum = 0.0;
    for (long long base = (long long)blockIdx.x * PT; base < k.N; base += (long long)gridDim.x * PT) {
        __syncthreads();
        const bool ok = load_obs_tile<PT>(k, ns, base, H, tid);
        forward_store<PT>(net, theta, H, DM, tid);
        for (int l = 0; l < L; ++l) {
            const float* Hl = H + hrow(net, l) * PLD;
            const float* dHl = (l == 0) ? nullptr : dH + (hrow(net, l) - net.dims[0]) * PLD;
            const float* Hn = (l == L - 1) ? nullptr : H + hrow(net, l + 1) * PLD;
            float* dst = (l == L - 1) ? DM : dH + (hrow(net, l + 1) - net.dims[0]) * PLD;
            tangent_layer<PT>(net, l, theta, v, Hl, dHl, Hn, dst, tid);
        }
        for (int d = 0; d < na; ++d) {
            const float ls = fmaxf(raw_ls[d], LOG_MIN_STD);
            const float s2 = expf(2.0f * ls);
            DM[d * PLD + tid] = ok ? DM[d * PLD + tid] / (s2 + 0.5f * KL_EPS) * k.inv_n : 0.0f;
        }
        if (ok) wsum += (double)k.inv_n;
        backward_accumulate<PT>(net, theta, H, DM, part, tid);
    }
    const double wtot = block_sum(wsum, red);
    if (tid == 0) part[P + 2] = (float)wtot;
}

template <int PT>
__global__ void __launch_bounds__(PT) k_loss_kl(ProblemDesc pd, PolK k, const float* __restrict__ theta, float* __restrict__ partials) {
    constexpr int PLD = PT + 1;
    extern __shared__ __attribute__((aligned(16))) float lds[];
    __shared__ double red[16];
    if (k.skip != nullptr && k.skip[0] >= 0.0) return;
    const NetDesc& net = pd.pol;
    const int tid = threadIdx.x, ns = pd.ns, na = pd.na;
    float* S = lds;
    float* A = S + ns * PLD;
    float* Bq = A + net.max_width * PLD;
    const float* __restrict__ raw_ls = theta + net.n_params;
    double loss_acc = 0.0, kl_acc = 0.0;
    for (long long base = (long long)blockIdx.x * PT; base < k.N; base += (long long)gridDim.x * PT) {
        const bool ok = load_obs_tile<PT>(k, ns, base, S, tid);
        const float* m = mlp_col(net, theta, S, A, Bq, PLD, tid);
        if (ok) {
            const long long n = base + tid;
            float llr = 0.0f, kl = 0.0f;
            for (int d = 0; d < na; ++d) {
                const float ls = fmaxf(raw_ls[d], LOG_MIN_STD), ols = k.old_ls[(size_t)n * k.ls_stride + d];
                const float mu = m[d * PLD + tid], omu = k.old_mean[n * na + d], a = k.act[n * na + d];
                const float z = (a - mu) * expf(-ls), zo = (a - omu) * expf(-ols);
                llr += (ols - ls) + 0.5f * (zo * zo - z * z);
                const float s2 = expf(2.0f * ls), os2 = expf(2.0f * ols);
                const float dm = omu - mu;
                kl += (dm * dm + os2 - s2) / (2.0f * s2 + KL_EPS) + ls - ols;
            }
            loss_acc -= (double)(expf(llr) * k.adv[n]) * (double)k.inv_n;
            kl_acc += (double)kl * (double)k.inv_n;
        }
    }
    const double l = block_sum(loss_acc, red);
    const double q = block_sum(kl_acc, red);
    if (tid == 0) { partials[blockIdx.x * 2] = (float)l; partials[blockIdx.x * 2 + 1] = (float)q; }
}

#define FIN_C 32
#ifdef FIN_TIMING
#define FT_MARK(i) { if (threadIdx.x == 0 && tail.op == 1 && blockIdx.x < 512) g_fin_phase[blockIdx.x][i] = __builtin_readcyclecounter(); }
extern "C" int32_t metrpo_debug_fin_phases(unsigned long long* out) { return hipMemcpyFromSymbol(out, HIP_SYMBOL(g_fin_phase), sizeof(unsigned long long) * 4096) == hipSuccess ? 0 : -1; }
#else
#define FT_MARK(i)
#endif
struct AdamTail {
    float* theta; float* m; float* v;
    float lr_t, b1, b2, eps;
    double* loss;
    double ent_coeff;
};
__device__ __forceinline__ double ppo_entropy_term(const ProblemDesc& pd, int p, const float* __restrict__ partials, const float* __restrict__ theta, double coeff) {
    if (p == 0) return -coeff * (double)partials[pd.P + 1];
    return (p - 1 >= pd.pol.n_params && theta[p - 1] > LOG_MIN_STD) ? -coeff : 0.0;
}
template <bool ADAM, bool ENT>
__global__ void __launch_bounds__(1024) k_finalize(ProblemDesc pd, int mode, int nrows, int stride, int lk_col,
                                                   const float* __restrict__ partials, const float* __restrict__ theta,
                                                   const double* __restrict__ v, double* __restrict__ out, CgTail tail, XchgK xc, AdamTail ad) {
    constexpr int NSL = 1024 / FIN_C;
    __shared__ double sh[NSL][FIN_C + 1];
    if (tail.op == 4 && tail.ls[0] >= 0.0) {
        if (xc.world > 1 && blockIdx.x == 0 && threadIdx.x < 2) { xchg_push(xc, (int)threadIdx.x, 0.0); (void)xchg_pull_sum(xc, (int)threadIdx.x); }
        if (tail.pub_dst != nullptr && blockIdx.x == 0) ls_publish(tail.scal, tail.pub_dst, tail.pub_stamp);
        return;
    }
    FT_MARK(0)
    CgPre pre;
    cg_prefetch(tail, pre);
    const int P = pd.P;
    const int nout = (mode == 0) ? P + 1 : (mode == 1) ? P : 2;
    const int lc = threadIdx.x % FIN_C, sl = threadIdx.x / FIN_C;
    const int p = blockIdx.x * FIN_C + lc;
    int col = p;
    if (mode == 0) col = (p == 0) ? P : p - 1;
    if (mode == 2) col = lk_col + p;
    const bool lsrow = (mode == 1 && p >= pd.pol.n_params && p < nout);
    if (lsrow) col = P + 2;
    double a = 0.0;
    if (p < nout) {
        int b = sl;
        for (; b + 3 * NSL < nrows; b += 4 * NSL) {
            const float v0 = partials[(size_t)b * stride + col], v1 = partials[(size_t)(b + NSL) * stride + col];
            const float v2 = partials[(size_t)(b + 2 * NSL) * stride + col], v3 = partials[(size_t)(b + 3 * NSL) * stride + col];
            a += (double)v0; a += (double)v1; a += (double)v2; a += (double)v3;
        }
        for (; b < nrows; b += NSL) a += (double)partials[(size_t)b * stride + col];
    }
    FT_MARK(1)
    sh[sl][lc] = a;
    __syncthreads();
    if (sl == 0 && p < nout) {
        double t = 0.0;
        for (int w = 0; w < NSL; ++w) t += sh[w][lc];
        if (lsrow) {
            const double raw = (double)theta[p];
            const double s2 = exp(2.0 * fmax(raw, (double)LOG_MIN_STD));
            const double c = 4.0 * s2 * (2.0 * s2 - 1e-8) / ((2.0 * s2 + 1e-8) * (2.0 * s2 + 1e-8));
            t = (raw > (double)LOG_MIN_STD) ? c * v[p] * t : 0.0;
        }
        if (ADAM) {
            if (xc.world > 1) { xchg_push(xc, p, t); t = xchg_pull_sum(xc, p); }
            if (ENT) t += ppo_entropy_term(pd, p, partials, ad.theta, ad.ent_coeff);
            out[p] = t;
            if (p == 0) { if (ad.loss != nullptr) *ad.loss = t; }
            else tf_adam_elem((float)t, ad.theta, ad.m, ad.v, p - 1, ad.lr_t, ad.b1, ad.b2, ad.eps);
            return;
        }
#if !defined(__gfx942__) && !defined(__gfx950__) && defined(__HIP_DEVICE_COMPILE__)
#error "k_finalize's fence-free hand-over is written for gfx942 / gfx950 (sc1 write-through stores); other targets need fence(release, agent) before the ticket"
#endif
        if (ENT) t += ppo_entropy_term(pd, p, partials, theta, ad.ent_coeff);
        if (tail.op != 0 || xc.world > 1) __hip_atomic_store(out + p, t, __ATOMIC_RELAXED, __HIP_MEMORY_SCOPE_AGENT);
        else out[p] = t;
        if (xc.world > 1) xchg_push(xc, p, t);
    }
    if (ADAM || (tail.op == 0 && xc.world <= 1)) return;
    __shared__ unsigned int s_last;
    __shared__ double cgsh[16];
    FT_MARK(2)
    asm volatile("s_waitcnt vmcnt(0)" ::: "memory");
    __syncthreads();
    FT_MARK(3)
    if (threadIdx.x == 0) {
        const unsigned int tk = __hip_atomic_fetch_add(tail.ticket, 1u, __ATOMIC_RELAXED, __HIP_MEMORY_SCOPE_AGENT);
        s_last = (tk == gridDim.x - 1) ? 1u : 0u;
        if (s_last) __builtin_amdgcn_fence(__ATOMIC_ACQUIRE, "agent");
    }
    __syncthreads();
    FT_MARK(4)
    if (!s_last) return;
    if (xc.world > 1) {
        for (int i = threadIdx.x; i < nout; i += blockDim.x) out[i] = xchg_pull_sum(xc, i);
        __syncthreads();
    }
    if (tail.op != 0) cg_tail_run(tail, cgsh, &pre);
    if (threadIdx.x == 0) __hip_atomic_store(tail.ticket, 0u, __ATOMIC_RELAXED, __HIP_MEMORY_SCOPE_AGENT);
}

__global__ void k_d2f(const double* __restrict__ in, float* __restrict__ out, int n) {
    const int i = blockIdx.x * blockDim.x + threadIdx.x;
    if (i < n) out[i] = (float)in[i];
}

static int ensure_partials(metrpo_ctx* c, int nrows) {
    const size_t need = (size_t)nrows * (c->pd.P + PART_EXTRA);
    return ws_grow(c, c->d_partials, need * sizeof(float));
}

static int make_call(metrpo_ctx* c, UpdOp op, const metrpo_batch* b, UpdCall* u, const metrpo_ppo_params* pr = nullptr, const metrpo_ppo_kl_params* kp = nullptr) {
    const bool vpg = (op == OP_VPG), ppo = (op == OP_PPO || op == OP_PPOKL);
    if (!b || !b->d_obs) return set_err(c, METRPO_ENULL, "batch/d_obs is NULL");
    if (b->N <= 0) return set_err(c, METRPO_EINVAL, "batch N must be positive");
    if (c->pd.na > 32) return set_err(c, METRPO_EUNSUPPORTED, "na > 32");
    if (ppo) {
        if (!pr) return set_err(c, METRPO_ENULL, "ppo: params NULL");
        if (!b->d_old_mean || !b->d_old_log_std)
            return set_err(c, METRPO_EINVAL, "ppo: the PPO surrogate needs the old distribution (batch d_old_mean / d_old_log_std is NULL)");
        if (!(pr->clip_lr >= 0.0) || !std::isfinite(pr->entropy_bonus_coeff))
            return set_err(c, METRPO_EINVAL, "ppo: need clip_lr >= 0 and a finite entropy_bonus_coeff");
    }
    if (op == OP_PPOKL) {
        if (!kp) return set_err(c, METRPO_ENULL, "ppo_kl: KL penalty params NULL");
        if (!(kp->kl_penalty >= 0.0) || !std::isfinite(kp->kl_penalty) || !std::isfinite(kp->step_size))
            return set_err(c, METRPO_EINVAL, "ppo_kl: need a finite kl_penalty >= 0 and a finite step_size");
    }
    if (op != OP_FVP && (!b->d_act || !b->d_adv || (!vpg && (!b->d_old_mean || !b->d_old_log_std))))
        return set_err(c, METRPO_ENULL, "batch pointer is NULL");
    if ((vpg || ppo) && !(b->inv_n_global > 0.0)) return set_err(c, METRPO_EINVAL, "batch inv_n_global must be positive");
    *u = UpdCall{};
    u->op = op; u->theta = c->d_theta.p;
    PolK& k = u->k;
    k.obs = b->d_obs; k.act = b->d_act; k.adv = b->d_adv; k.old_mean = b->d_old_mean; k.old_ls = b->d_old_log_std;
    k.ls_stride = b->old_log_std_stride; k.valid = b->d_valid; k.N = b->N; k.inv_n = (float)b->inv_n_global;
    if (op == OP_PPOKL) { k.kl_beta = (float)kp->kl_penalty; k.kl_delta = kp->step_size; }
    if (ppo) { k.clip_lo = (float)(1.0 - pr->clip_lr); k.clip_hi = (float)(1.0 + pr->clip_lr); u->ent_coeff = pr->entropy_bonus_coeff; u->ent_in_reduction = true; }
    return METRPO_OK;
}

struct PartRows { int rc, nrows, stride, lk_col; };

static void finalize(metrpo_ctx* c, const UpdCall& u, const PartRows& r, hipStream_t st) {
    const int mode = (u.op == OP_LOSSKL) ? 2 : (u.op == OP_FVP) ? 1 : 0;
    const int nout = (mode == 0) ? c->pd.P + 1 : (mode == 1) ? c->pd.P : 2;
    CgTail none; none.op = 0; none.ticket = c->d_ticket.p; none.vpos = nullptr; none.imgval = nullptr; none.ls = nullptr; none.pub_dst = nullptr;
    const XchgK xc = (u.scope.exchange_in_tail && c->xg_world > 1) ? xchg_next(c) : xchg_none();
    const dim3 grid((nout + FIN_C - 1) / FIN_C);
    const bool ppo = (u.op == OP_PPO || u.op == OP_PPOKL);
    if (ppo && u.adam)
        hipLaunchKernelGGL((k_finalize<true, true>), grid, dim3(1024), 0, st, c->pd, mode, r.nrows, r.stride, r.lk_col,
                           c->d_partials.p, c->d_theta.p, u.v64, u.out, none, xc, *u.adam);
    else if (ppo && u.ent_in_reduction) {
        AdamTail ent = {}; ent.ent_coeff = u.ent_coeff;
        hipLaunchKernelGGL((k_finalize<false, true>), grid, dim3(1024), 0, st, c->pd, mode, r.nrows, r.stride, r.lk_col,
                           c->d_partials.p, c->d_theta.p, u.v64, u.out, none, xc, ent);
    }
    else if (u.adam)
        hipLaunchKernelGGL((k_finalize<true, false>), dim3((nout + FIN_C - 1) / FIN_C), dim3(1024), 0, st, c->pd, mode, r.nrows, r.stride, r.lk_col,
                           c->d_partials.p, c->d_theta.p, u.v64, u.out, none, xc, *u.adam);
    else
        hipLaunchKernelGGL((k_finalize<false, false>), dim3((nout + FIN_C - 1) / FIN_C), dim3(1024), 0, st, c->pd, mode, r.nrows, r.stride, r.lk_col,
                           c->d_partials.p, c->d_theta.p, u.v64, u.out, u.tail ? *u.tail : none, xc, AdamTail{});
}

template <int PT>
static int launch_generic(metrpo_ctx* c, const UpdCall& u, int* nrows, hipStream_t st) {
    const NetDesc& net = c->pd.pol;
    const PolK& k = u.k;
    int hrows = 0; for (int l = 0; l < net.n_layers; ++l) hrows += net.dims[l];
    size_t rows = (u.op == OP_GRAD || u.op == OP_VPG || u.op == OP_PPO || u.op == OP_PPOKL) ? hrows + c->pd.na : (u.op == OP_FVP) ? hrows + c->pd.na + (hrows - net.dims[0])
                                                                         : (size_t)c->pd.ns + 2 * net.max_width;
    const size_t sh = rows * (PT + 1) * sizeof(float);
    if (sh > 160 * 1024) return METRPO_EUNSUPPORTED;
    const long long tiles = (k.N + PT - 1) / PT;
    const int g = (int)std::max<long long>(1, std::min<long long>(tiles, (long long)c->n_sm * 2));
    int rc = ensure_partials(c, g); if (rc) return rc;
    *nrows = g;
    c->upd_last = {0, (int)u.op, -1, PT, g, 0, 0};
    if (u.op == OP_GRAD) {
        if (sh > 64 * 1024) HIP_TRY(c, hipFuncSetAttribute((const void*)k_loss_grad<PT, OP_GRAD>, hipFuncAttributeMaxDynamicSharedMemorySize, (int)sh));
        hipLaunchKernelGGL((k_loss_grad<PT, OP_GRAD>), dim3(g), dim3(PT), sh, st, c->pd, k, u.theta, c->d_partials.p);
    } else if (u.op == OP_VPG) {
        if (sh > 64 * 1024) HIP_TRY(c, hipFuncSetAttribute((const void*)k_loss_grad<PT, OP_VPG>, hipFuncAttributeMaxDynamicSharedMemorySize, (int)sh));
        hipLaunchKernelGGL((k_loss_grad<PT, OP_VPG>), dim3(g), dim3(PT), sh, st, c->pd, k, u.theta, c->d_partials.p);
    } else if (u.op == OP_PPO) {
        if (sh > 64 * 1024) HIP_TRY(c, hipFuncSetAttribute((const void*)k_loss_grad<PT, OP_PPO>, hipFuncAttributeMaxDynamicSharedMemorySize, (int)sh));
        hipLaunchKernelGGL((k_loss_grad<PT, OP_PPO>), dim3(g), dim3(PT), sh, st, c->pd, k, u.theta, c->d_partials.p);
    } else if (u.op == OP_PPOKL) {
        if (sh > 64 * 1024) HIP_TRY(c, hipFuncSetAttribute((const void*)k_loss_grad<PT, OP_PPOKL>, hipFuncAttributeMaxDynamicSharedMemorySize, (int)sh));
        hipLaunchKernelGGL((k_loss_grad<PT, OP_PPOKL>), dim3(g), dim3(PT), sh, st, c->pd, k, u.theta, c->d_partials.p);
    } else if (u.op == OP_FVP) {
        if (sh > 64 * 1024) HIP_TRY(c, hipFuncSetAttribute((const void*)k_fvp<PT>, hipFuncAttributeMaxDynamicSharedMemorySize, (int)sh));
        hipLaunchKernelGGL(k_fvp<PT>, dim3(g), dim3(PT), sh, st, c->pd, k, u.theta, u.vf, c->d_partials.p);
    } else {
        if (sh > 64 * 1024) HIP_TRY(c, hipFuncSetAttribute((const void*)k_loss_kl<PT>, hipFuncAttributeMaxDynamicSharedMemorySize, (int)sh));
        hipLaunchKernelGGL(k_loss_kl<PT>, dim3(g), dim3(PT), sh, st, c->pd, k, u.theta, c->d_partials.p);
    }
    return METRPO_OK;
}

static PartRows run_mode(metrpo_ctx* c, const UpdCall& u, hipStream_t st) {
    const int P = c->pd.P;
    const long long tiles = (u.k.N + 15) / 16;
    PartRows r = {METRPO_OK, 0, P + PART_EXTRA, P};
    const bool mfma = c->pol_mfma >= 0;
    if (mfma || f3_active(c, u.k.gm != nullptr)) {
        const long long per_block = (mfma ? 8ll : 4ll) * std::max(1, c->upd_tiles_per_wave);
        const long long max_blocks = (long long)c->n_sm * ((mfma && u.op == OP_LOSSKL) ? 2 : 1);
        r.nrows = (int)std::max<long long>(1, std::min<long long>((tiles + per_block - 1) / per_block, max_blocks));
        const bool fvpc = mfma && u.scope.cache_activations && u.op == OP_FVP && u.k.gm == nullptr;
        c->upd_last = {mfma ? 1 : 3, fvpc ? (int)OP_FVPC : (int)u.op, mfma ? c->pol_mfma : -1, 0, r.nrows, 0, 0};
        if (!(r.rc = ensure_partials(c, r.nrows)))
            r.rc = mfma ? policy_mfma_launch(c, u, c->d_partials.p, r.nrows, st) : policy_f3_launch(c, u, c->d_partials.p, r.nrows, st);
        return r;
    }
    r.stride = (u.op == OP_LOSSKL) ? 2 : P + PART_EXTRA; r.lk_col = 0;
    r.rc = launch_generic<128>(c, u, &r.nrows, st);
    if (r.rc == METRPO_EUNSUPPORTED) r.rc = launch_generic<64>(c, u, &r.nrows, st);
    if (r.rc == METRPO_EUNSUPPORTED) r.rc = launch_generic<32>(c, u, &r.nrows, st);
    if (r.rc == METRPO_EUNSUPPORTED) r.rc = set_err(c, r.rc, "policy too wide for the update kernels' LDS tile");
    return r;
}

static int run_update(metrpo_ctx* c, const UpdCall& u, hipStream_t st) {
    if (policy_gemm_applicable(c, u.k.N, u.k.gm != nullptr)) {
        if (u.op == OP_LOSSKL && u.tail) return set_err(c, METRPO_EUNSUPPORTED, "device-side line search: not on the GEMM update path");
        return policy_gemm_run(c, u, st);
    }
    const bool timed = u.op == OP_FVP && ctx_opt(c, OPT_TIME_FVP) != nullptr && c->fvp_ev_n + 2 <= 32;
    if (timed) {
        for (; c->fvp_ev_made < 32; ++c->fvp_ev_made) HIP_TRY(c, hipEventCreate(&c->fvp_ev[c->fvp_ev_made]));
        HIP_TRY(c, hipEventRecord(c->fvp_ev[c->fvp_ev_n], st));
    }
    const PartRows r = run_mode(c, u, st);
    if (r.rc) return r.rc;
    if (timed) { HIP_TRY(c, hipEventRecord(c->fvp_ev[c->fvp_ev_n + 1], st)); c->fvp_ev_n += 2; }
    finalize(c, u, r, st);
    HIP_TRY(c, hipGetLastError());
    return METRPO_OK;
}

int launch_loss_grad(metrpo_ctx* c, const metrpo_batch* b, double* out, hipStream_t st, const CgTail* tail, SolveScope scope) {
    UpdCall u; int rc = make_call(c, OP_GRAD, b, &u); if (rc) return rc;
    u.out = out; u.tail = tail; u.scope = scope;
    return run_update(c, u, st);
}

int launch_policy_vjp(metrpo_ctx* c, const float* obs, const float* gm, long long N, double* out, hipStream_t st) {
    if (!obs || !gm || !out) return set_err(c, METRPO_ENULL, "policy_vjp: NULL pointer");
    if (c->pd.na > 32) return set_err(c, METRPO_EUNSUPPORTED, "na > 32");
    UpdCall u = {};
    u.op = OP_GRAD; u.theta = c->d_theta.p; u.out = out;
    u.k.obs = obs; u.k.N = N; u.k.inv_n = 1.0f; u.k.gm = gm;
    return run_update(c, u, st);
}

int launch_fvp(metrpo_ctx* c, const metrpo_batch* b, const double* v, double* hv, hipStream_t st) {
    if (!v || !hv) return set_err(c, METRPO_ENULL, "v/hv is NULL");
    const int P = c->pd.P;
    hipLaunchKernelGGL(k_d2f, dim3((P + 127) / 128), dim3(128), 0, st, v, c->d_vf.p, P);
    return launch_fvp_tail(c, b, c->d_vf.p, v, hv, nullptr, st);
}

int launch_fvp_tail(metrpo_ctx* c, const metrpo_batch* b, const float* vf, const double* v, double* hv, const CgTail* tail, hipStream_t st, SolveScope scope) {
    UpdCall u; int rc = make_call(c, OP_FVP, b, &u); if (rc) return rc;
    u.vf = vf; u.v64 = v; u.out = hv; u.tail = tail; u.scope = scope;
    return run_update(c, u, st);
}

int launch_loss_kl(metrpo_ctx* c, const metrpo_batch* b, const float* theta, double* out, hipStream_t st, const CgTail* decide, SolveScope scope) {
    UpdCall u; int rc = make_call(c, OP_LOSSKL, b, &u); if (rc) return rc;
    if (theta) u.theta = theta;
    if (decide) u.k.skip = decide->ls;
    u.out = out; u.tail = decide; u.scope = scope;
    return run_update(c, u, st);
}

int launch_vpg_loss_grad(metrpo_ctx* c, const metrpo_batch* b, double* out, hipStream_t st) {
    UpdCall u; int rc = make_call(c, OP_VPG, b, &u); if (rc) return rc;
    u.out = out;
    return run_update(c, u, st);
}

__global__ void k_vpg_adam(const double* __restrict__ gout, int P, AdamTail ad) {
    const int i = blockIdx.x * blockDim.x + threadIdx.x;
    if (i == 0 && ad.loss != nullptr) *ad.loss = gout[0];
    if (i < P) tf_adam_elem((float)gout[1 + i], ad.theta, ad.m, ad.v, i, ad.lr_t, ad.b1, ad.b2, ad.eps);
}

int run_vpg_update(metrpo_ctx* c, const metrpo_batch* b, const metrpo_vpg_params* pr, double* d_loss, hipStream_t st) {
    const int P = c->pd.P;
    if (!pr) return set_err(c, METRPO_ENULL, "vpg_update: params NULL");
    if (!(pr->lr >= 0.0) || !(pr->beta1 >= 0.0 && pr->beta1 < 1.0) || !(pr->beta2 >= 0.0 && pr->beta2 < 1.0) || !(pr->eps >= 0.0))
        return set_err(c, METRPO_EINVAL, "vpg_update: need lr >= 0, 0 <= beta1, beta2 < 1, eps >= 0");
    UpdCall u; int rc = make_call(c, OP_VPG, b, &u); if (rc) return rc;
    if ((rc = ensure_policy_adam(c))) return rc;
    const int t1 = c->pol_adam_t + 1;
    const double lr_t = pr->lr * std::sqrt(1.0 - std::pow(pr->beta2, (double)t1)) / (1.0 - std::pow(pr->beta1, (double)t1));
    float* am = (float*)c->d_pol_adam.p;
    const AdamTail ad = {c->d_theta.p, am, am + P, (float)lr_t, (float)pr->beta1, (float)pr->beta2, (float)pr->eps, d_loss};
    double* gout = c->d_cg.p;
    const UpdFusion f = update_fusion(c, b->N, false);
    const bool fused = f.carries_next_step();
    u.out = gout; u.adam = fused ? &ad : nullptr; u.scope.exchange_in_tail = f.exchange_in_tail;
    if ((rc = run_update(c, u, st))) return rc;
    if (!fused) {
        if ((c->xg_world > 1 || c->nccl_comm) && (rc = comm_allreduce_f64(c, gout, P + 1, st))) return rc;
        hipLaunchKernelGGL(k_vpg_adam, dim3((P + 255) / 256), dim3(256), 0, st, (const double*)gout, P, ad);
    }
    HIP_TRY(c, hipGetLastError());
    c->pol_adam_t = t1;
    return METRPO_OK;
}

__global__ void __launch_bounds__(1024) k_ppo_step(double* __restrict__ gout, int P, int n_params, int na, int step, AdamTail ad) {
    const double coeff = ad.ent_coeff;
    __shared__ float s_h;
    if (threadIdx.x == 0) {
        float h = (float)na * ENTROPY_CONST;
        for (int d = 0; d < na; ++d) h += fmaxf(ad.theta[n_params + d], LOG_MIN_STD);
// ... 117 lines not shown
```

me-trpo_amd/csrc/process.hip:

```cpp
#include "device_common.h"

__device__ __forceinline__ double baseline_value(const float* __restrict__ obs_row, int ns, int tpath,
                                                 const double* __restrict__ coeffs) {
    double v = 0.0;
    for (int i0 = 0; i0 < ns; i0 += 8) {
        float ob[8];
#pragma unroll
        for (int u = 0; u < 8; ++u) ob[u] = (i0 + u < ns) ? obs_row[i0 + u] : 0.0f;
#pragma unroll
        for (int u = 0; u < 8; ++u) {
            if (i0 + u < ns) {
                const double o = fmin(fmax((double)ob[u], -10.0), 10.0);
                v += coeffs[i0 + u] * o + coeffs[ns + i0 + u] * o * o;
            }
        }
    }
    const double al = (double)tpath / 100.0;
    v += coeffs[2 * ns] * al + coeffs[2 * ns + 1] * al * al + coeffs[2 * ns + 2] * al * al * al + coeffs[2 * ns + 3];
    return v;
}

#ifndef GAE_CHUNK
#define GAE_CHUNK 7
#endif
// ... 68 lines not shown
#pragma unroll
            for (int i = 0; i < NR; ++i) { const int e = i * 64 + lane0; r[i] = (e < nv * NS) ? src[e] : 0.0f; }
        };
        int tp_cur = 0, tp_nxt = 0;
        auto load_tp = [&](int t) { return (lane0 < nv) ? tpath[(size_t)t * B + b0 + lane0] : 0; };
        if (w0 < T) { if (NS) load(w0, nxt); tp_nxt = load_tp(w0); }
        for (int t = w0; t < T; t += NW) {
            tp_cur = tp_nxt;
            if (t + NW < T) tp_nxt = load_tp(t + NW);
            if (NS) {
#pragma unroll
                for (int i = 0; i < NR; ++i) cur[i] = nxt[i];
                if (t + NW < T) load(t + NW, nxt);
#pragma unroll
                for (int i = 0; i < NR; ++i) S[i * 64 + lane0] = cur[i];
            } else {
                const float* __restrict__ src = obs + ((size_t)t * B + b0) * ns;
                for (int e = lane0; e < nv * ns; e += 64) S[e] = src[e];
            }
            __builtin_amdgcn_fence(__ATOMIC_SEQ_CST, "wavefront"); __builtin_amdgcn_wave_barrier();
            if (lane0 < nv) V[(size_t)t * B + b0 + lane0] = baseline_value(S + lane0 * ns, ns, tp_cur, coeffs);
            __builtin_amdgcn_fence(__ATOMIC_SEQ_CST, "wavefront"); __builtin_amdgcn_wave_barrier();
        }
        __syncthreads();
    } else V = nullptr;
    __shared__ double red[16];
    __shared__ double agg[NW][5][64];
    __shared__ uint8_t cut[NW][64];
    const int lane = threadIdx.x & 63, w = threadIdx.x >> 6;
    const int b = blockIdx.x * 64 + lane;
    const int Tc = (T + NW - 1) / NW;
    const int t_lo = min(T, w * Tc), t_hi = min(T, (w + 1) * Tc);
    const bool act = b < B;
    double s1 = 0.0, s2 = 0.0, cnt = 0.0;
    {
        double a_n = 0.0, v_n = 0.0, r_n = 0.0; bool comp = false;
        if (act) gae_chunk_pass<false>(V, rew, done, t_lo, t_hi, B, b, gamma, lam, a_n, v_n, r_n, comp, adv, ret, valid, s1, s2, cnt);
        const int len = t_hi - t_lo;
        agg[w][0][lane] = a_n; agg[w][1][lane] = r_n; agg[w][2][lane] = v_n;
        agg[w][3][lane] = (comp || len == 0) ? 0.0 : pow(gamma * lam, (double)(len - 1));
        agg[w][4][lane] = (comp || len == 0) ? 0.0 : pow(gamma, (double)len);
        cut[w][lane] = comp ? 1 : 0;
    }
    __syncthreads();
    double a_in = 0.0, v_in = 0.0, r_in = 0.0; bool c_in = false;
    for (int j = NW - 1; j > w; --j) {
        const int lo = min(T, j * Tc), hi = min(T, (j + 1) * Tc);
        if (hi <= lo) continue;
        const double E = gamma * v_in + gamma * lam * a_in;
        a_in = agg[j][0][lane] + agg[j][3][lane] * E;
        r_in = agg[j][1][lane] + agg[j][4][lane] * r_in;
        v_in = agg[j][2][lane];
        c_in = c_in || cut[j][lane];
    }
    if (act) gae_chunk_pass<true>(V, rew, done, t_lo, t_hi, B, b, gamma, lam, a_in, v_in, r_in, c_in, adv, ret, valid, s1, s2, cnt);
    const double t1s = block_sum(s1, red), t2s = block_sum(s2, red), t3s = block_sum(cnt, red);
    __shared__ unsigned int s_last;
    unsigned int* ticket = (unsigned int*)gpart;
    gpart += 1;
    if (threadIdx.x == 0) {
        gpart[3 * blockIdx.x + 0] = t1s; gpart[3 * blockIdx.x + 1] = t2s; gpart[3 * blockIdx.x + 2] = t3s;
        __builtin_amdgcn_fence(__ATOMIC_RELEASE, "agent");
        asm volatile("s_waitcnt vmcnt(0)" ::: "memory");
        const unsigned int tk = __hip_atomic_fetch_add(ticket, 1u, __ATOMIC_RELAXED, __HIP_MEMORY_SCOPE_AGENT);
        s_last = (tk == gridDim.x - 1) ? 1u : 0u;
        if (s_last) __builtin_amdgcn_fence(__ATOMIC_ACQUIRE, "agent");
    }
    __syncthreads();
    if (!s_last || threadIdx.x >= 64) return;
    double a0 = 0.0, a1 = 0.0, a2 = 0.0;
    for (int j = threadIdx.x; j < (int)gridDim.x; j += 64) {
        a0 += __hip_atomic_load(gpart + 3 * j + 0, __ATOMIC_RELAXED, __HIP_MEMORY_SCOPE_AGENT);
        a1 += __hip_atomic_load(gpart + 3 * j + 1, __ATOMIC_RELAXED, __HIP_MEMORY_SCOPE_AGENT);
        a2 += __hip_atomic_load(gpart + 3 * j + 2, __ATOMIC_RELAXED, __HIP_MEMORY_SCOPE_AGENT);
    }
#pragma unroll
    for (int o = 32; o > 0; o >>= 1) { a0 += __shfl_xor(a0, o, 64); a1 += __shfl_xor(a1, o, 64); a2 += __shfl_xor(a2, o, 64); }
    if (threadIdx.x == 0) {
        stats[0] += a0; stats[1] += a1; stats[2] += a2;
        __hip_atomic_store(ticket, 0u, __ATOMIC_RELAXED, __HIP_MEMORY_SCOPE_AGENT);
    }
}

__global__ void k_center(float* __restrict__ adv, const uint8_t* __restrict__ valid, int64_t N,
                         const double* __restrict__ stats) {
    const double n = stats[2];
    const double mean = stats[0] / n;
    const double var = fmax(stats[1] / n - mean * mean, 0.0);
    const double inv = 1.0 / (sqrt(var) + 1e-8);
    for (int64_t i = (int64_t)blockIdx.x * blockDim.x + threadIdx.x; i < N; i += (int64_t)gridDim.x * blockDim.x)
        adv[i] = (valid == nullptr || valid[i]) ? (float)(((double)adv[i] - mean) * inv) : 0.0f;
}

#define GRAM_TILE 64
__global__ void k_gram(const float* __restrict__ obs, const float* __restrict__ ret, const int32_t* __restrict__ tpath,
                       const uint8_t* __restrict__ valid, int64_t N, int ns, double* __restrict__ part) {
    extern __shared__ __attribute__((aligned(16))) double feat[];
    const int F = 2 * ns + 4, LDF = F + 1;
    const int nout = F * F + F;
    for (int p0 = 0; p0 < nout; p0 += blockDim.x * 8) {
        double acc[8] = {0, 0, 0, 0, 0, 0, 0, 0};
        for (int64_t base = (int64_t)blockIdx.x * GRAM_TILE; base < N; base += (int64_t)gridDim.x * GRAM_TILE) {
            __syncthreads();
            for (int e = threadIdx.x; e < GRAM_TILE * LDF; e += blockDim.x) {
                const int sidx = e / LDF, f = e % LDF;
                const int64_t n = base + sidx;
                double v = 0.0;
                if (n < N && (valid == nullptr || valid[n])) {
                    if (f < ns) v = fmin(fmax((double)obs[n * ns + f], -10.0), 10.0);
                    else if (f < 2 * ns) { const double o = fmin(fmax((double)obs[n * ns + f - ns], -10.0), 10.0); v = o * o; }
                    else if (f == F) v = (double)ret[n];
                    else {
                        const double al = (double)tpath[n] / 100.0;
                        const int q = f - 2 * ns;
                        v = (q == 0) ? al : (q == 1) ? al * al : (q == 2) ? al * al * al : 1.0;
                    }
                }
                feat[e] = v;
            }
            __syncthreads();
#pragma unroll
            for (int u = 0; u < 8; ++u) {
                const int p = p0 + u * blockDim.x + threadIdx.x;
                if (p < nout) {
                    const int i = (p < F * F) ? p / F : p - F * F;
                    const int j = (p < F * F) ? p % F : F;
                    double a = 0.0;
                    for (int sidx = 0; sidx < GRAM_TILE; ++sidx) a += feat[sidx * LDF + i] * feat[sidx * LDF + j];
                    acc[u] += a;
                }
            }
        }
#pragma unroll
        for (int u = 0; u < 8; ++u) {
            const int p = p0 + u * blockDim.x + threadIdx.x;
            if (p < nout) part[(size_t)blockIdx.x * nout + p] = acc[u];
        }
    }
}

typedef float f32x4 __attribute__((ext_vector_type(4)));
template <int NFB>
__global__ void __launch_bounds__(256) k_gram_mfma(const float* __restrict__ obs, const float* __restrict__ ret,
                                                   const int32_t* __restrict__ tpath, const uint8_t* __restrict__ valid,
                                                   long long N, int ns, double* __restrict__ part) {
    extern __shared__ __attribute__((aligned(16))) double red[];
    constexpr int M = NFB * 16;
    const int lane = threadIdx.x & 63, wave = threadIdx.x >> 6, c = lane & 15, q = lane >> 4;
    const int F = 2 * ns + 4;
    double acc[NFB][NFB][4];
#pragma unroll
    for (int a = 0; a < NFB; ++a)
#pragma unroll
        for (int b = 0; b < NFB; ++b)
#pragma unroll
            for (int r = 0; r < 4; ++r) acc[a][b][r] = 0.0;
    const long long ntiles = (N + 15) / 16;
    struct TileIn { float o[4][NFB]; float rv[4]; int tp[4]; int ok[4]; };
    auto fetch = [&](long long tile, TileIn& in) {
#pragma unroll
        for (int s = 0; s < 4; ++s) {
            const long long n = tile * 16 + 4 * s + q;
            const bool inr = tile < ntiles && n < N;
            const long long nc = inr ? n : 0;
            in.ok[s] = inr ? ((valid == nullptr) ? 1 : (int)valid[nc]) : 0;
            in.tp[s] = tpath[nc];
            in.rv[s] = ret[nc];
#pragma unroll
            for (int cb = 0; cb < NFB; ++cb) {
                const int f = 16 * cb + c;
                const int fo = (f < ns) ? f : ((f < 2 * ns) ? f - ns : 0);
                in.o[s][cb] = obs[nc * ns + fo];
            }
        }
    };
    TileIn nxt;
    fetch((long long)blockIdx.x * 4 + wave, nxt);
    __builtin_amdgcn_s_waitcnt(0x0F70);
    for (long long tile = (long long)blockIdx.x * 4 + wave; tile < ntiles; tile += (long long)gridDim.x * 4) {
        const TileIn in = nxt;
        fetch(tile + (long long)gridDim.x * 4, nxt);
        asm volatile("" ::: "memory");
        f32x4 g[NFB][NFB];
#pragma unroll
        for (int a = 0; a < NFB; ++a)
#pragma unroll
            for (int b = 0; b < NFB; ++b) g[a][b] = f32x4{0.f, 0.f, 0.f, 0.f};
        float val[4][NFB];
#pragma unroll
        for (int s = 0; s < 4; ++s) {
            const float al = (float)in.tp[s] / 100.0f;
            const float rv = in.rv[s];
#pragma unroll
            for (int cb = 0; cb < NFB; ++cb) {
                const int f = 16 * cb + c;
                const float o = fminf(fmaxf(in.o[s][cb], -10.f), 10.f);
                const int kq = f - 2 * ns;
                float x = (f < ns) ? o : o * o;
                x = (kq == 0) ? al : x;
                x = (kq == 1) ? al * al : x;
                x = (kq == 2) ? al * al * al : x;
                x = (kq == 3) ? 1.0f : x;
                x = (f == F) ? rv : x;
                x = (f > F) ? 0.0f : x;
                val[s][cb] = in.ok[s] ? x : 0.0f;
            }
        }
#pragma unroll
        for (int s = 0; s < 4; ++s)
#pragma unroll
            for (int a = 0; a < NFB; ++a)
#pragma unroll
                for (int b = 0; b < NFB; ++b) g[a][b] = __builtin_amdgcn_mfma_f32_16x16x4f32(val[s][a], val[s][b], g[a][b], 0, 0, 0);
#pragma unroll
        for (int a = 0; a < NFB; ++a)
#pragma unroll
            for (int b = 0; b < NFB; ++b)
#pragma unroll
                for (int r = 0; r < 4; ++r) acc[a][b][r] += (double)g[a][b][r];
    }
    double* mine = red + (size_t)wave * M * M;
#pragma unroll
    for (int a = 0; a < NFB; ++a)
#pragma unroll
        for (int b = 0; b < NFB; ++b)
#pragma unroll
            for (int r = 0; r < 4; ++r) mine[(16 * a + 4 * q + r) * M + 16 * b + c] = acc[a][b][r];
    __syncthreads();
    const int nout = F * F + F;
    double* out = part + (size_t)blockIdx.x * nout;
    for (int p = threadIdx.x; p < nout; p += 256) {
        const int i = (p < F * F) ? p / F : p - F * F, j = (p < F * F) ? p % F : F;
        const int e = i * M + j;
        out[p] = (red[e] + red[M * M + e]) + (red[2 * M * M + e] + red[3 * M * M + e]);
    }
}

__global__ void __launch_bounds__(1024) k_gram_final(const double* __restrict__ part, int nblocks, int M, int F,
                                                     double* __restrict__ AtA, double* __restrict__ Aty) {
    __shared__ double sh[64][17];
    const int lc = threadIdx.x & 15, sl = threadIdx.x >> 4;
    const int p = blockIdx.x * 16 + lc;
    const int nout = F * F + F;
    double a = 0.0;
    if (p < nout)
        for (int b = sl; b < nblocks; b += 64) a += part[(size_t)b * nout + p];
    sh[sl][lc] = a;
    __syncthreads();
    if (sl == 0 && p < nout) {
        double s = 0.0;
        for (int w = 0; w < 64; ++w) s += sh[w][lc];
        if (p < F * F) AtA[p] += s; else Aty[p - F * F] += s;
    }
}

template <int NFB>
__global__ void __launch_bounds__(256) k_gram_mfma_wide(const float* __restrict__ obs, const float* __restrict__ ret,
                                                        const int32_t* __restrict__ tpath, const uint8_t* __restrict__ valid,
                                                        long long N, int ns, double* __restrict__ part) {
    constexpr int M = NFB * 16, NPAIR = NFB * (NFB + 1) / 2, NPW = (NPAIR + 3) / 4, NV = (16 * M + 255) / 256;
    extern __shared__ __attribute__((aligned(16))) double red[];
    float* FT = (float*)red;
    const int tid = threadIdx.x, lane = tid & 63, wave = tid >> 6, c = lane & 15, q = lane >> 4;
    const int F = 2 * ns + 4;
    int pa[NPW], pb[NPW];
#pragma unroll
    for (int j = 0; j < NPW; ++j) {
        int p = wave + 4 * j, a = 0;
        if (p >= NPAIR) { pa[j] = -1; pb[j] = -1; continue; }
        while (p >= NFB - a) { p -= NFB - a; ++a; }
        pa[j] = a; pb[j] = a + p;
    }
    double acc[NPW][4];
#pragma unroll
    for (int j = 0; j < NPW; ++j)
#pragma unroll
        for (int r = 0; r < 4; ++r) acc[j][r] = 0.0;
    const long long ntiles = (N + 15) / 16;
    struct Raw { float o[NV]; float rv[NV]; int tp[NV]; int ok[NV]; };
    auto fetch = [&](long long tile, Raw& in) {
#pragma unroll
        for (int v = 0; v < NV; ++v) {
            const int e = tid + 256 * v, sl = e / M, f = e % M;
            const long long n = tile * 16 + sl;
            const bool inr = e < 16 * M && tile < ntiles && n < N;
            const long long nc = inr ? n : 0;
            const int fo = (f < ns) ? f : ((f < 2 * ns) ? f - ns : 0);
            in.ok[v] = inr ? ((valid == nullptr) ? 1 : (int)valid[nc]) : 0;
            in.tp[v] = tpath[nc]; in.rv[v] = ret[nc]; in.o[v] = obs[nc * ns + fo];
        }
    };
    auto publish = [&](const Raw& in, float* dst) {
#pragma unroll
        for (int v = 0; v < NV; ++v) {
            const int e = tid + 256 * v, sl = e / M, f = e % M;
            if (e >= 16 * M) continue;
            const float al = (float)in.tp[v] / 100.0f, o = fminf(fmaxf(in.o[v], -10.f), 10.f);
            const int kq = f - 2 * ns;
            float x = (f < ns) ? o : o * o;
            x = (kq == 0) ? al : x;
            x = (kq == 1) ? al * al : x;
            x = (kq == 2) ? al * al * al : x;
            x = (kq == 3) ? 1.0f : x;
            x = (f == F) ? in.rv[v] : x;
            x = (f > F) ? 0.0f : x;
            dst[((sl >> 2) * 4 + (sl & 3)) * M + f] = in.ok[v] ? x : 0.0f;
        }
    };
    Raw nxt;
    long long tile = blockIdx.x;
    fetch(tile, nxt);
    __builtin_amdgcn_s_waitcnt(0x0F70);
    int buf = 0;
    if (tile < ntiles) publish(nxt, FT);
    fetch(tile + gridDim.x, nxt);
    __syncthreads();
    for (; tile < ntiles; tile += gridDim.x) {
        const float* cur = FT + buf * 16 * M;
        f32x4 g[NPW];
#pragma unroll
        for (int j = 0; j < NPW; ++j) g[j] = f32x4{0.f, 0.f, 0.f, 0.f};
#pragma unroll
        for (int s4 = 0; s4 < 4; ++s4) {
            const float* row = cur + (s4 * 4 + q) * M + c;
#pragma unroll
            for (int j = 0; j < NPW; ++j)
                if (pa[j] >= 0) g[j] = __builtin_amdgcn_mfma_f32_16x16x4f32(row[16 * pa[j]], row[16 * pb[j]], g[j], 0, 0, 0);
        }
        if (tile + gridDim.x < ntiles) publish(nxt, FT + (buf ^ 1) * 16 * M);
        fetch(tile + 2LL * gridDim.x, nxt);
        asm volatile("" ::: "memory");
#pragma unroll
        for (int j = 0; j < NPW; ++j)
#pragma unroll
            for (int r = 0; r < 4; ++r) acc[j][r] += (double)g[j][r];
        __syncthreads();
        buf ^= 1;
    }
    __syncthreads();
#pragma unroll
    for (int j = 0; j < NPW; ++j) {
        if (pa[j] < 0) continue;
#pragma unroll
        for (int r = 0; r < 4; ++r) {
            const int i = 16 * pa[j] + 4 * q + r, jj = 16 * pb[j] + c;
            red[i * M + jj] = acc[j][r];
            if (pa[j] != pb[j]) red[jj * M + i] = acc[j][r];
        }
    }
    __syncthreads();
    const int nout = F * F + F;
    double* out = part + (size_t)blockIdx.x * nout;
    for (int p = tid; p < nout; p += 256) {
        const int i = (p < F * F) ? p / F : p - F * F, j = (p < F * F) ? p % F : F;
        out[p] = red[i * M + j];
    }
}

template <int NFB>
static int launch_gram_mfma_wide(metrpo_ctx* c, const float* obs, const float* ret, const int32_t* tpath, const uint8_t* valid,
                                 int64_t N, double* AtA, double* Aty, hipStream_t st) {
    constexpr int M = NFB * 16;
    const int F = 2 * c->pd.ns + 4;
    const long long tiles = (N + 15) / 16;
    const int g = (int)std::max<long long>(1, std::min<long long>(tiles, (long long)c->n_sm * 2));
    const size_t need = (size_t)g * (F * F + F);
    { const int rc = ws_grow(c, c->d_gram_part, need * sizeof(double)); if (rc) return rc; }
    const size_t sh = sizeof(double) * M * M;
    if (sh > 64 * 1024) HIP_TRY(c, hipFuncSetAttribute((const void*)k_gram_mfma_wide<NFB>, hipFuncAttributeMaxDynamicSharedMemorySize, (int)sh));
    hipLaunchKernelGGL(k_gram_mfma_wide<NFB>, dim3(g), dim3(256), sh, st, obs, ret, tpath, valid, (long long)N, c->pd.ns, c->d_gram_part.p);
    const int nout = F * F + F;
    hipLaunchKernelGGL(k_gram_final, dim3((nout + 15) / 16), dim3(1024), 0, st, c->d_gram_part.p, g, M, F, AtA, Aty);
    HIP_TRY(c, hipGetLastError());
    return METRPO_OK;
}

template <int NFB>
static int launch_gram_mfma(metrpo_ctx* c, const float* obs, const float* ret, const int32_t* tpath, const uint8_t* valid,
                            int64_t N, double* AtA, double* Aty, hipStream_t st) {
    constexpr int M = NFB * 16;
    const int F = 2 * c->pd.ns + 4;
    const long long tiles = (N + 15) / 16;
    const int g = (int)std::max<long long>(1, std::min<long long>((tiles + 3) / 4, (long long)c->n_sm * 2));
    const size_t need = (size_t)g * (F * F + F);
    { const int rc = ws_grow(c, c->d_gram_part, need * sizeof(double)); if (rc) return rc; }
    const size_t sh = sizeof(double) * 4 * M * M;
    if (sh > 64 * 1024) HIP_TRY(c, hipFuncSetAttribute((const void*)k_gram_mfma<NFB>, hipFuncAttributeMaxDynamicSharedMemorySize, (int)sh));
    hipLaunchKernelGGL(k_gram_mfma<NFB>, dim3(g), dim3(256), sh, st, obs, ret, tpath, valid, (long long)N, c->pd.ns, c->d_gram_part.p);
    const int nout = F * F + F;
    hipLaunchKernelGGL(k_gram_final, dim3((nout + 15) / 16), dim3(1024), 0, st, c->d_gram_part.p, g, M, F, AtA, Aty);
    HIP_TRY(c, hipGetLastError());
    return METRPO_OK;
}

int launch_gae(metrpo_ctx* c, const float* obs, const float* rew, const uint8_t* done, const int32_t* tpath, int T,
               int B, const double* coeffs, double gamma, double lam, float* adv, float* ret, uint8_t* valid,
               double* stats, hipStream_t st) {
    const long long N = (long long)T * B;
    double* V = nullptr;
    if (coeffs != nullptr) {
        { const int rc = ws_grow(c, c->d_vbuf, sizeof(double) * (size_t)N); if (rc) return rc; }
        V = c->d_vbuf.p;
    }
    const int nblk = (B + 63) / 64;
    bool grew = false;
    { const int rc = ws_grow(c, c->d_gae_part, sizeof(double) * std::max<size_t>((size_t)nblk * 3 + 2, 1024), &grew); if (rc) return rc; }
    if (grew) HIP_TRY(c, hipMemsetAsync(c->d_gae_part.p, 0, c->d_gae_part.bytes, st));
    const int ns = c->pd.ns;
    const bool wide = (B <= 256 && T >= 128 && ns <= 18);
    const int nw = wide ? 16 : GAE_NW;
    const int pre_v = (coeffs != nullptr && nblk <= 32 && T >= 16) ? 1 : 0;
    if (pre_v) {
        const size_t shp = sizeof(float) * 4 * 64 * (size_t)ns;
        if (shp > 64 * 1024) HIP_TRY(c, hipFuncSetAttribute((const void*)k_baseline_predict, hipFuncAttributeMaxDynamicSharedMemorySize, (int)shp));
        hipLaunchKernelGGL(k_baseline_predict, dim3(nblk, (T + 3) / 4), dim3(256), shp, st, obs, tpath, coeffs, ns, V, T, B);
        HIP_TRY(c, hipGetLastError());
    }
    const size_t sh = (coeffs != nullptr && !pre_v) ? sizeof(float) * nw * 64 * (size_t)ns : 0;
#define GAE_LAUNCH_NW(NSV, NWV) do { \
        if (sh > 48 * 1024) HIP_TRY(c, hipFuncSetAttribute((const void*)k_gae<NSV, NWV>, hipFuncAttributeMaxDynamicSharedMemorySize, (int)sh)); \
        hipLaunchKernelGGL((k_gae<NSV, NWV>), dim3((B + 63) / 64), dim3(64 * NWV), sh, st, obs, tpath, coeffs, ns, pre_v, V, rew, done, T, B, gamma, lam, adv, ret, valid, stats, c->d_gae_part.p); } while (0)
#define GAE_LAUNCH(NSV) do { if (wide) GAE_LAUNCH_NW(NSV, 16); else GAE_LAUNCH_NW(NSV, GAE_NW); } while (0)
#define GAE_LAUNCH8(NSV) GAE_LAUNCH_NW(NSV, GAE_NW)
    if (sh + 48 * 1024 > 160 * 1024) return set_err(c, METRPO_EUNSUPPORTED, "gae: observation too wide for the staging buffer");
    switch (ns) {
    case 10: GAE_LAUNCH(10); break; case 11: GAE_LAUNCH(11); break; case 14: GAE_LAUNCH(14); break;
    case 18: GAE_LAUNCH(18); break; case 29: GAE_LAUNCH8(29); break; case 55: GAE_LAUNCH8(55); break;
    default: GAE_LAUNCH8(0);
    }
#undef GAE_LAUNCH8
#undef GAE_LAUNCH_NW
#undef GAE_LAUNCH
    HIP_TRY(c, hipGetLastError());
    return METRPO_OK;
}

__global__ void k_process_begin(const float* __restrict__ theta, int P, int na, float* __restrict__ ls_out, double* __restrict__ acc, int64_t n_acc) {
    const int64_t i = (int64_t)blockIdx.x * blockDim.x + threadIdx.x;
    if (acc != nullptr && i < n_acc) acc[i] = 0.0;
    if (ls_out != nullptr && i < na) { const float v = theta[P - na + i]; ls_out[i] = (v < LOG_MIN_STD) ? LOG_MIN_STD : v; }
}
int launch_process_begin(metrpo_ctx* c, float* ls_out, double* acc, int64_t n_acc, hipStream_t st) {
    const int64_t n = std::max<int64_t>(n_acc, (int64_t)c->pd.na);
    hipLaunchKernelGGL(k_process_begin, dim3((unsigned)((n + 255) / 256)), dim3(256), 0, st, (const float*)c->d_theta.p, c->pd.P, c->pd.na, ls_out, acc, n_acc);
    HIP_TRY(c, hipGetLastError());
    return METRPO_OK;
}

int launch_center(metrpo_ctx* c, float* adv, const uint8_t* valid, int64_t N, const double* stats, hipStream_t st) {
    const int bs = 256;
    const int grid = (int)std::min<int64_t>((N + bs - 1) / bs, (int64_t)c->n_sm * 8);
    hipLaunchKernelGGL(k_center, dim3(grid), dim3(bs), 0, st, adv, valid, N, stats);
    HIP_TRY(c, hipGetLastError());
    return METRPO_OK;
}

__global__ void __launch_bounds__(1024) k_baseline_solve(int F, const double* __restrict__ AtA, const double* __restrict__ Aty, double reg0, double* __restrict__ coeffs) {
    extern __shared__ __attribute__((aligned(16))) double Ms[];
    __shared__ int s_bad;
    const int tid = threadIdx.x, lane = tid & 63, W = F + 1;
    double* x = Ms + (size_t)F * W;
    double reg = reg0;
    for (int attempt = 0; attempt < 5; ++attempt) {
        for (int i = tid; i < F * W; i += (int)blockDim.x) { const int r = i / W, c = i % W; Ms[i] = (c < F) ? AtA[r * F + c] + (r == c ? reg : 0.0) : Aty[r]; }
        if (tid == 0) s_bad = 0;
        __syncthreads();
        for (int k = 0; k < F; ++k) {
            if (tid == 0 && !(Ms[k * W + k] > 0.0)) s_bad = 1;
            const double inv = 1.0 / Ms[k * W + k];
            const int RS = (int)blockDim.x >> 7;
            for (int c = k + 1 + (tid & 127); c < W; c += 128) {
// ... 5 lines not shown
                    Ms[r * W + c] = m0 - f0 * mkc; Ms[(r + RS) * W + c] = m1 - f1 * mkc; Ms[(r + 2 * RS) * W + c] = m2 - f2 * mkc; Ms[(r + 3 * RS) * W + c] = m3 - f3 * mkc;
                }
                for (; r < F; r += RS) Ms[r * W + c] -= (Ms[r * W + k] * inv) * mkc;
            }
            __syncthreads();
        }
        if (tid < 64) {
            for (int k = F - 1; k >= 0; --k) {
                double a = 0.0;
                for (int c = k + 1 + lane; c < F; c += 64) a += Ms[k * W + c] * x[c];
                for (int o = 32; o > 0; o >>= 1) a += __shfl_xor(a, o, 64);
                if (lane == 0) { const double v = (Ms[k * W + F] - a) / Ms[k * W + k]; x[k] = v; if (!(fabs(v) <= 1.7e308)) s_bad = 1; }
                __builtin_amdgcn_fence(__ATOMIC_SEQ_CST, "wavefront"); __builtin_amdgcn_wave_barrier();
            }
        }
        __syncthreads();
        if (!s_bad) break;
        reg *= 10.0;
        __syncthreads();
    }
    for (int i = tid; i < F; i += (int)blockDim.x) coeffs[i] = x[i];
}

__device__ __forceinline__ double readlane_f64(double v, int l) {
    const long long b = __double_as_longlong(v);
    const unsigned int lo = (unsigned int)__builtin_amdgcn_readlane((int)b, l), hi = (unsigned int)__builtin_amdgcn_readlane((int)(b >> 32), l);
    return __longlong_as_double((long long)(((unsigned long long)hi << 32) | lo));
}
template <int FT>
__global__ void __launch_bounds__(64) k_baseline_solve_wave(const double* __restrict__ AtA, const double* __restrict__ Aty, double reg0, double* __restrict__ coeffs) {
    const int lane = threadIdx.x;
    const bool live = lane < FT;
    double reg = reg0;
    double x[FT];
    for (int attempt = 0; attempt < 5; ++attempt) {
        double row[FT + 1];
        bool bad = false;
#pragma unroll
        for (int c = 0; c < FT; ++c) row[c] = live ? AtA[lane * FT + c] + (lane == c ? reg : 0.0) : 0.0;
        row[FT] = live ? Aty[lane] : 0.0;
#pragma unroll
        for (int k = 0; k < FT; ++k) {
            double pv[FT + 1];
#pragma unroll
            for (int c = k; c <= FT; ++c) pv[c] = readlane_f64(row[c], k);
            bad = bad || !(pv[k] > 0.0);
            const double f = row[k] * (1.0 / pv[k]);
            if (lane > k) {
#pragma unroll
                for (int c = k + 1; c <= FT; ++c) row[c] = fma(-f, pv[c], row[c]);
            }
        }
#pragma unroll
        for (int k = FT - 1; k >= 0; --k) {
            double a = row[FT];
#pragma unroll
            for (int c = k + 1; c < FT; ++c) a = fma(-row[c], x[c], a);
            x[k] = readlane_f64(a / row[k], k);
            bad = bad || !isfinite(x[k]);
        }
        if (!bad) break;
        reg *= 10.0;
    }
    if (lane == 0) {
#pragma unroll
        for (int k = 0; k < FT; ++k) coeffs[k] = x[k];
    }
}

int launch_baseline_solve(metrpo_ctx* c, const double* AtA, const double* Aty, double reg, double* coeffs, hipStream_t st) {
    const int F = 2 * c->pd.ns + 4;
#define SOLVE_WAVE(FT_) case FT_: hipLaunchKernelGGL(k_baseline_solve_wave<FT_>, dim3(1), dim3(64), 0, st, AtA, Aty, reg, coeffs); HIP_TRY(c, hipGetLastError()); return METRPO_OK;
    switch (F) { SOLVE_WAVE(24) SOLVE_WAVE(26) SOLVE_WAVE(32) SOLVE_WAVE(40) SOLVE_WAVE(62) default: break; }
#undef SOLVE_WAVE
    const size_t sh = sizeof(double) * ((size_t)F * (F + 1) + F);
    if (sh > 160 * 1024) return set_err(c, METRPO_EUNSUPPORTED, "baseline_solve: feature count too large for one workgroup's LDS");
    if (sh > 64 * 1024) HIP_TRY(c, hipFuncSetAttribute((const void*)k_baseline_solve, hipFuncAttributeMaxDynamicSharedMemorySize, (int)sh));
    hipLaunchKernelGGL(k_baseline_solve, dim3(1), dim3(1024), sh, st, F, AtA, Aty, reg, coeffs);
    HIP_TRY(c, hipGetLastError());
    return METRPO_OK;
}

int launch_gram(metrpo_ctx* c, const float* obs, const float* ret, const int32_t* tpath, const uint8_t* valid,
                int64_t N, double* AtA, double* Aty, hipStream_t st) {
    const int F = 2 * c->pd.ns + 4;
    const int nfb = (F + 1 + 15) / 16;
    if (nfb <= 2) return launch_gram_mfma<2>(c, obs, ret, tpath, valid, N, AtA, Aty, st);
    if (nfb == 3) return launch_gram_mfma<3>(c, obs, ret, tpath, valid, N, AtA, Aty, st);
    if (nfb == 4) return launch_gram_mfma<4>(c, obs, ret, tpath, valid, N, AtA, Aty, st);
    if (nfb == 5) return launch_gram_mfma_wide<5>(c, obs, ret, tpath, valid, N, AtA, Aty, st);
    if (nfb == 6) return launch_gram_mfma_wide<6>(c, obs, ret, tpath, valid, N, AtA, Aty, st);
    if (nfb == 7) return launch_gram_mfma_wide<7>(c, obs, ret, tpath, valid, N, AtA, Aty, st);
    if (nfb == 8) return launch_gram_mfma_wide<8>(c, obs, ret, tpath, valid, N, AtA, Aty, st);
    const int bs = 256;
    const size_t sh = sizeof(double) * GRAM_TILE * (F + 1);
    const int grid = (int)std::min<int64_t>((N + GRAM_TILE - 1) / GRAM_TILE, (int64_t)c->n_sm * 4);
    const int nout = F * F + F;
    const size_t need = (size_t)grid * nout;
    { const int rc = ws_grow(c, c->d_gram_part, sizeof(double) * need); if (rc) return rc; }
    if (sh > 64 * 1024) HIP_TRY(c, hipFuncSetAttribute((const void*)k_gram, hipFuncAttributeMaxDynamicSharedMemorySize, (int)sh));
    hipLaunchKernelGGL(k_gram, dim3(grid), dim3(bs), sh, st, obs, ret, tpath, valid, N, c->pd.ns, c->d_gram_part.p);
    hipLaunchKernelGGL(k_gram_final, dim3((nout + 15) / 16), dim3(1024), 0, st, c->d_gram_part.p, grid, 0, F, AtA, Aty);
    HIP_TRY(c, hipGetLastError());
    return METRPO_OK;
}

__global__ void __launch_bounds__(256) k_path_counts(const uint8_t* __restrict__ done, const int32_t* __restrict__ tpath, int B,
                                                     double* __restrict__ counts, const int32_t* __restrict__ stop) {
    __shared__ double sh[16];
    if (*stop != 0) return;
    const size_t row = (size_t)blockIdx.x * B;
    long long acc = 0;
    for (int b = threadIdx.x; b < B; b += 256)
        if (done[row + b]) acc += (long long)tpath[row + b] + 1;
    const double tot = block_sum((double)acc, sh);
    if (threadIdx.x == 0) counts[blockIdx.x] = tot;
}

__global__ void k_stop_scan(const double* __restrict__ counts, int T, int t0, double batch_size, double* __restrict__ state,
                            int32_t* __restrict__ stop) {
    if (threadIdx.x != 0 || blockIdx.x != 0 || *stop != 0) return;
    double cum = state[0];
    for (int t = 0; t < T; ++t) {
        cum += counts[t];
        if (cum >= batch_size) { state[0] = cum; state[1] = (double)(t0 + t); *stop = 1; __threadfence(); return; }
    }
    state[0] = cum;
}

int launch_sampler_progress(metrpo_ctx* c, const uint8_t* done, const int32_t* tpath, int T, int B, int t0, long long batch_size,
                            double* counts, double* state, int32_t* stop, hipStream_t st) {
    hipLaunchKernelGGL(k_path_counts, dim3(T), dim3(256), 0, st, done, tpath, B, counts, stop);
    hipLaunchKernelGGL(k_stop_scan, dim3(1), dim3(64), 0, st, counts, T, t0, (double)batch_size, state, stop);
    HIP_TRY(c, hipGetLastError());
    return METRPO_OK;
}
```

me-trpo_amd/engine.py:

```python
import ctypes as C
from collections import namedtuple

import numpy as np
import torch

from . import _lib
from ._lib import lib, check

METRPO_UNSET = -100

Trajectory = namedtuple('Trajectory', 'obs act rew mean done tpath last_obs B T H')
"""Time-major device tensors of one rollout: obs [T,B,ns], act [T,B,na] (unclipped), rew [T,B],
mean [T,B,na], done [T,B] uint8, tpath [T,B] int32, last_obs [B,ns]."""


def _ptr(t):
    return C.c_void_p(t.data_ptr()) if t is not None else C.c_void_p(0)


def _f32(t, dev, shape=None):
    if t is None:
        return None
    t = torch.as_tensor(t, device=dev).to(torch.float32).contiguous()
    if shape is not None:
# ... 316 lines not shown
        self._keep = (pool, eps, model_idx, sel_noise, reset_idx, reset_model, resume, last_state, stop, stop_cum)
        if no_draws and not chunked and not force_generic:
            self._ra_cache = ((id(out), pool.data_ptr(), B, T, H, sam_mode, bool(determ), bool(eval_all_heads), int(stream_offset)), a, out, pool)
        return out

    def sampler_progress(self, done, tpath, t0, batch_size, counts, state, stop):
        T, B = done.shape
        assert counts.dtype == torch.float64 and counts.numel() >= T and state.dtype == torch.float64 and stop.dtype == torch.int32
        self._chk(lib.metrpo_sampler_progress(self._ctx, _ptr(done), _ptr(tpath), int(T), int(B), int(t0), int(batch_size),
                                              _ptr(counts), _ptr(state), _ptr(stop), self._stream()))

    def rollout_path(self):
        if self.dyn_precision == 'bf16':
            return 7
        return int(lib.metrpo_set_rollout_variant(self._ctx, int(getattr(self, '_variant', 0))))

    def last_rollout_kernel(self):
        k = int(lib.metrpo_last_rollout_kernel(self._ctx))
        return {0: 'generic', 1: 'mfma-head-per-wave', 2: 'mfma-cooperative', 3: 'gemm-stepwise', 4: 'resident', 5: 'gemm-streamk', 6: 'streamk-persistent', 7: 'gemm-bf16'}.get(k)

    def rollout_note(self):
        return lib.metrpo_rollout_note(self._ctx).decode()

    def alloc_trajectory(self, B, T, H):
        dev, f = self.device, torch.float32
        return Trajectory(torch.empty(T, B, self.ns, dtype=f, device=dev), torch.empty(T, B, self.na, dtype=f, device=dev),
                          torch.empty(T, B, dtype=f, device=dev), torch.empty(T, B, self.na, dtype=f, device=dev),
                          torch.empty(T, B, dtype=torch.uint8, device=dev), torch.empty(T, B, dtype=torch.int32, device=dev),
                          torch.empty(B, self.ns, dtype=f, device=dev), B, T, H)

    def validation_cost(self, s0, T, gamma):
        s0 = _f32(s0, self.device); assert s0.shape[1] == self.ns
        costs = torch.empty(self.K, dtype=torch.float64, device=self.device)
        self._chk(lib.metrpo_validation_cost(self._ctx, _ptr(s0), s0.shape[0], int(T), float(gamma), _ptr(costs), self._stream()))
        return costs

    def gae(self, traj, coeffs, gamma, lam, stats=None):
        dev = self.device
        T, B = traj.T, traj.B
        adv = torch.empty(T, B, dtype=torch.float32, device=dev); ret = torch.empty_like(adv)
        valid = torch.empty(T, B, dtype=torch.uint8, device=dev)
        if stats is None:
            stats = torch.zeros(3, dtype=torch.float64, device=dev)
        if coeffs is not None:
            if isinstance(coeffs, torch.Tensor) and coeffs.is_cuda:
                coeffs = coeffs.to(torch.float64).contiguous()
            else:
                F = 2 * self.ns + 4
                if getattr(self, '_coef_pin', None) is None:
                    self._coef_pin = [torch.empty(F, dtype=torch.float64).pin_memory() for _ in range(2)]
                    self._coef_dev = [torch.empty(F, dtype=torch.float64, device=dev) for _ in range(2)]
                    self._coef_i = 0
                self._coef_i ^= 1
                pin, cd = self._coef_pin[self._coef_i], self._coef_dev[self._coef_i]
                pin.copy_(torch.as_tensor(np.asarray(coeffs, dtype=np.float64)))
                cd.copy_(pin, non_blocking=True)
                coeffs = cd
            assert coeffs.numel() == 2 * self.ns + 4
        self._chk(lib.metrpo_gae(self._ctx, _ptr(traj.obs), _ptr(traj.rew), _ptr(traj.done), _ptr(traj.tpath), T, B,
                                 _ptr(coeffs), float(gamma), float(lam), _ptr(adv), _ptr(ret), _ptr(valid), _ptr(stats),
                                 self._stream()))
        return adv, ret, valid, stats

    def process_begin(self, n_acc):
        self._close_open_update()
        ls = torch.empty(self.na, dtype=torch.float32, device=self.device)
        acc = torch.empty(int(n_acc), dtype=torch.float64, device=self.device)
        self._chk(lib.metrpo_process_begin(self._ctx, _ptr(ls), _ptr(acc), int(n_acc), self._stream()))
        return ls, acc

    def center_advantages(self, adv, valid, stats):
        self._chk(lib.metrpo_center_advantages(self._ctx, _ptr(adv), _ptr(valid), adv.numel(), _ptr(stats), self._stream()))
        return adv

    def baseline_gram(self, obs, ret, tpath, valid, out=None):
        F = 2 * self.ns + 4
        if out is None:
            out = torch.zeros(F * F + F, dtype=torch.float64, device=self.device)
        AtA, Aty = out[:F * F].view(F, F), out[F * F:]
        self._chk(lib.metrpo_baseline_gram(self._ctx, _ptr(obs), _ptr(ret), _ptr(tpath), _ptr(valid), ret.numel(),
                                           _ptr(AtA), _ptr(Aty), self._stream()))
        return AtA, Aty

    def baseline_solve(self, gram, reg_coeff=1e-5, out=None):
        F = 2 * self.ns + 4
        assert gram.is_cuda and gram.dtype == torch.float64 and gram.numel() == F * F + F and gram.is_contiguous()
        if out is None:
            out = torch.empty(F, dtype=torch.float64, device=self.device)
        self._chk(lib.metrpo_baseline_solve(self._ctx, _ptr(gram), C.c_void_p(gram.data_ptr() + 8 * F * F), float(reg_coeff), _ptr(out), self._stream()))
        return out

    def make_batch(self, obs, act, adv, old_mean, old_log_std, valid=None, n_global=None):
        dev = self.device
        obs = _f32(obs, dev).reshape(-1, self.ns); N = obs.shape[0]
        act = _f32(act, dev).reshape(N, self.na); adv = _f32(adv, dev).reshape(N)
        stride = 0
        if old_mean is not None:
            old_mean = _f32(old_mean, dev).reshape(N, self.na)
        if old_log_std is not None:
            old_log_std = _f32(old_log_std, dev)
            stride = 0 if old_log_std.numel() == self.na else self.na
            if stride:
                old_log_std = old_log_std.reshape(N, self.na)
        if valid is not None:
            valid = torch.as_tensor(valid, device=dev).to(torch.uint8).contiguous().reshape(N)
        if n_global is None:
            n_global = int(valid.sum().item()) if valid is not None else N
        b = _lib.Batch()
        b.d_obs, b.d_act, b.d_adv = obs.data_ptr(), act.data_ptr(), adv.data_ptr()
        b.d_old_mean = old_mean.data_ptr() if old_mean is not None else None
        b.d_old_log_std, b.old_log_std_stride = (old_log_std.data_ptr() if old_log_std is not None else None), stride
        b.d_valid = valid.data_ptr() if valid is not None else None
        b.N, b.inv_n_global = N, 1.0 / float(n_global)
        b._keep = (obs, act, adv, old_mean, old_log_std, valid)
        return b

    def subsample_batch(self, batch, idx, n_global_sub=None):
        idx = _i32(idx, self.device).reshape(-1)
        m = int(idx.numel())
        if m == 0:
            raise ValueError("subsample_batch: empty index vector")
        count = torch.zeros(1, dtype=torch.float64, device=self.device)
        sub = _lib.Batch()
        inv = 1.0 / float(n_global_sub) if n_global_sub is not None else 1.0 / m
        self._chk(lib.metrpo_subsample_batch(self._ctx, C.byref(batch), _ptr(idx), m, inv, C.byref(sub), _ptr(count), self._stream()))
        sub.valid_count = count
        sub._keep = (idx, batch)
        if n_global_sub is None and batch.d_valid:
            n = int(count.item())
            if n == 0:
                raise ValueError("subsample_batch: none of the %d gathered rows is valid" % m)
            sub.inv_n_global = 1.0 / n
        return sub

    def batch_tensors(self, batch):
        N, dev = int(batch.N), self.device

        def view(ptr, count, typestr, shape):
            return torch.as_tensor(_DevView(ptr, count, typestr), device=dev).clone().reshape(shape) if ptr else None
        n_ls = N * self.na if batch.old_log_std_stride else self.na
        return dict(obs=view(batch.d_obs, N * self.ns, '<f4', (N, self.ns)), old_mean=view(batch.d_old_mean, N * self.na, '<f4', (N, self.na)),
                    old_log_std=view(batch.d_old_log_std, n_ls, '<f4', (-1, self.na)), valid=view(batch.d_valid, N, '|u1', (N,)))

    def loss_grad(self, batch):
        out = torch.empty(self.P + 1, dtype=torch.float64, device=self.device)
        self._chk(lib.metrpo_loss_grad(self._ctx, C.byref(batch), _ptr(out), self._stream()))
        return out

    def vpg_loss_grad(self, batch):
        out = torch.empty(self.P + 1, dtype=torch.float64, device=self.device)
        self._chk(lib.metrpo_vpg_loss_grad(self._ctx, C.byref(batch), _ptr(out), self._stream()))
        return out

    def vpg_update(self, batch, lr=1e-3, beta1=0.9, beta2=0.999, eps=1e-8, want_loss=True):
        self._close_open_update()
        p = _lib.VpgParams()
        p.lr, p.beta1, p.beta2, p.eps = float(lr), float(beta1), float(beta2), float(eps)
        loss = torch.empty(1, dtype=torch.float64, device=self.device) if want_loss else None
        self._chk(lib.metrpo_vpg_update(self._ctx, C.byref(batch), C.byref(p), _ptr(loss), self._stream()))
        return loss

    @staticmethod
    def _ppo_params(clip_lr, entropy_bonus_coeff, lr=1e-3, beta1=0.9, beta2=0.999, eps=1e-8):
        p = _lib.PpoParams()
        p.clip_lr, p.entropy_bonus_coeff = float(clip_lr), float(entropy_bonus_coeff)
        p.lr, p.beta1, p.beta2, p.eps = float(lr), float(beta1), float(beta2), float(eps)
# ... 280 lines not shown
```

me-trpo_amd/sampler.py:

```python
import numpy as np
import torch

from .parallel import Comm


class DevicePaths(object):

    def __init__(self, traj, log_std, n_complete_samples):
        self.traj, self.log_std, self.n_complete_samples = traj, log_std, n_complete_samples
        self.acc = None

    def __len__(self):
        return int(self.traj.done.sum().item())

    def to_paths(self):
        tr = self.traj
        obs, act, rew, mean = (x.double().cpu().numpy() for x in (tr.obs, tr.act, tr.rew, tr.mean))
        done = tr.done.cpu().numpy().astype(bool)
        ls = self.log_std.double().cpu().numpy()
        T, B = rew.shape
        start = np.zeros(B, dtype=int)
        paths = []
        for t, b in zip(*np.nonzero(done)):
            sl = slice(start[b], t + 1)
            paths.append(dict(observations=obs[sl, b], actions=act[sl, b], rewards=rew[sl, b], env_infos={},
                              agent_infos=dict(mean=mean[sl, b], log_std=np.broadcast_to(ls, mean[sl, b].shape).copy())))
            start[b] = t + 1
        return paths


class BaseSampler(object):
    def __init__(self, algo):
        self.algo = algo

    def process_samples(self, itr, paths):
        algo, eng = self.algo, self.algo.engine
        comm = getattr(algo, 'comm', None) or Comm()
        tr = paths.traj
        self.finish_baseline_fit()
        coeffs = getattr(algo.baseline, 'coeffs_for_kernel', None) if hasattr(algo.baseline, 'coeffs_for_kernel') else algo.baseline.coeffs
        F = 2 * eng.ns + 4
        acc = getattr(paths, 'acc', None)
        if acc is None or acc.numel() != 3 + F * F + F:
            acc = torch.zeros(3 + F * F + F, dtype=torch.float64, device=eng.device)
        paths.acc = None
        adv, ret, valid, stats = eng.gae(tr, coeffs, algo.discount, algo.gae_lambda, stats=acc[:3])
        comm.allreduce_sum_(stats)
        static = (eng.env_name != 'ant') and (tr.T % tr.H == 0)
        n_global = comm.world * tr.T * tr.B if static and self._uniform_B(comm, tr.B) else int(stats[2].item())
        if algo.center_adv:
            eng.center_advantages(adv, valid, stats)
        if algo.positive_adv:
            lo = torch.where(valid.bool(), adv, torch.full_like(adv, float('inf'))).min().reshape(1)
            comm.allreduce_min_(lo)
            adv.sub_(lo).add_(1e-8)
        gram = acc[3:]
        eng.baseline_gram(tr.obs, ret, tr.tpath, valid, out=gram)
        comm.allreduce_sum_(gram)
        if getattr(algo, 'device_baseline_fit', False) and gram.is_cuda and hasattr(algo.baseline, 'solve_device'):
            algo.baseline.solve_device(eng, gram)
            self._pending_gram = None
            self._gram_event = None
        else:
            self._pending_gram = gram.to('cpu', non_blocking=True) if gram.is_cuda else gram
            self._gram_event = torch.cuda.Event() if gram.is_cuda else None
            if self._gram_event is not None:
                self._gram_event.record()
        samples_data = dict(observations=tr.obs.reshape(-1, eng.ns), actions=tr.act.reshape(-1, eng.na),
                            rewards=tr.rew.reshape(-1), returns=ret.reshape(-1), advantages=adv.reshape(-1),
                            env_infos={}, agent_infos=dict(mean=tr.mean.reshape(-1, eng.na), log_std=paths.log_std),
                            valids=valid.reshape(-1), n_valid_global=n_global, paths=paths)
        if not getattr(algo, 'defer_baseline_fit', False):
            self.finish_baseline_fit()
        return samples_data

    def _uniform_B(self, comm, B):
        return getattr(self.algo, 'uniform_shards', True)

    def finish_baseline_fit(self):
        gram = getattr(self, '_pending_gram', None)
        if gram is None:
            return
        if self._gram_event is not None:
            self._gram_event.synchronize()
        F = 2 * self.algo.engine.ns + 4
        g = gram.numpy()
        self.algo.baseline.solve(g[:F * F].reshape(F, F), g[F * F:])
        self._pending_gram = None


class VectorizedSampler(BaseSampler):
    def __init__(self, algo, n_envs=None):
        super(VectorizedSampler, self).__init__(algo)
        self.n_envs = n_envs
        self._itr_seed = 0

    def start_worker(self):
        n_envs = self.n_envs
        if n_envs is None:
            n_envs = int(self.algo.batch_size / self.algo.max_path_length)
            n_envs = max(1, min(n_envs, 100))
        assert getattr(self.algo.env, 'vectorized', False), "the imagined env must be vectorized"
        self.vec_env = self.algo.env.vec_env_executor(n_envs=n_envs, max_path_length=self.algo.max_path_length, fused=True)
        self.env_spec = self.algo.env.spec
        self._n_envs = n_envs

    def shutdown_worker(self):
        self.vec_env.terminate()

    def obtain_samples(self, itr, determ=False, draws=None):
        algo, eng = self.algo, self.algo.engine
        comm = getattr(algo, 'comm', None) or Comm()
        B, H = self._n_envs, algo.max_path_length
        nne = algo.env
        pool = nne.env.device_tensor(eng.device) if hasattr(nne.env, 'device_tensor') else \
            torch.as_tensor(np.stack([nne.env.reset() for _ in range(max(B, 1))]), dtype=torch.float32, device=eng.device)
        seed = (getattr(algo, 'seed', 0) * 1000003 + self._itr_seed * 7919 + (1 if determ else 0)) & 0xFFFFFFFFFFFFFFFF
        self._itr_seed += 1
        offset = comm.rank * B
        draws = draws or {}
        ev = getattr(algo, 'rollout_events', None)
        if ev is not None:
            from .tracing import timing_event
            e0, e1 = timing_event(), timing_event()
            e0.record()
        common = dict(determ=determ, eval_all_heads=getattr(algo, 'eval_all_heads', True), seed=seed, stream_offset=offset)
        if eng.env_name == 'ant':
            traj = self._obtain_until_enough(B, H, nne.sam_mode, pool, draws, common)
        else:
            rounds = max(1, -(-algo.batch_size // (B * H)))
            T = rounds * H
            out = None
            if getattr(algo, 'reuse_trajectory_buffers', False):
                key = (B, T, H)
                if getattr(self, '_traj_key', None) != key:
                    self._traj_buf, self._traj_key = eng.alloc_trajectory(B, T, H), key
                out = self._traj_buf
            traj = eng.rollout(B, T, H, nne.sam_mode, pool, out=out, **common, **draws)
        if ev is not None:
            e1.record()
# ... 60 lines not shown
```

Baseline: 1.947 billion.

## Fuse advantage centering into gram kernel and fold loss/KL reduction into policy kernel

Advantage centering now runs inside the baseline gram MFMA kernel, so the separate centering kernel launch and its extra pass over the advantages are skipped. The gram kernel also gains a deeper prefetch ring and computes only the upper-triangle MFMA blocks, mirroring them on write-out. The loss/KL policy evaluation kernel now has its last-arriving block reduce the partial rows through a ticket atomic and run the line-search decision in place, which removes the separate finalize launch. These add atomic hand-off logic that is tied to gfx942/gfx950, and the fused paths only apply under specific conditions.

```diff
diff --git a/include/metrpo.h b/include/metrpo.h
--- a/include/metrpo.h
+++ b/include/metrpo.h
@@ -130,6 +130,9 @@
                                  const double* d_stats, void* stream);
 int32_t metrpo_baseline_gram(metrpo_ctx* ctx, const float* d_obs, const float* d_ret, const int32_t* d_tpath,
                              const uint8_t* d_valid, int64_t N, double* d_AtA, double* d_Aty, void* stream);
+int32_t metrpo_baseline_gram_center(metrpo_ctx* ctx, const float* d_obs, const float* d_ret, const int32_t* d_tpath,
+                                    const uint8_t* d_valid, int64_t N, double* d_AtA, double* d_Aty, float* d_adv,
+                                    const double* d_stats, void* stream);
 int32_t metrpo_baseline_solve(metrpo_ctx* ctx, const double* d_AtA, const double* d_Aty, double reg_coeff, double* d_coeffs, void* stream);
 
 typedef struct {
diff --git a/me-trpo_amd/_lib.py b/me-trpo_amd/_lib.py
--- a/me-trpo_amd/_lib.py
+++ b/me-trpo_amd/_lib.py
@@ -127,6 +127,7 @@
     'metrpo_process_begin': (_I, [_P, _P, _P, _L, _P]),
     'metrpo_center_advantages': (_I, [_P, _P, _P, _L, _P, _P]),
     'metrpo_baseline_gram': (_I, [_P, _P, _P, _P, _P, _L, _P, _P, _P]),
+    'metrpo_baseline_gram_center': (_I, [_P, _P, _P, _P, _P, _L, _P, _P, _P, _P, _P]),
     'metrpo_baseline_solve': (_I, [_P, _P, _P, _D, _P, _P]),
     'metrpo_loss_grad': (_I, [_P, C.POINTER(Batch), _P, _P]),
     'metrpo_fvp': (_I, [_P, C.POINTER(Batch), _P, _P, _P]),
diff --git a/me-trpo_amd/csrc/api.hip b/me-trpo_amd/csrc/api.hip
--- a/me-trpo_amd/csrc/api.hip
+++ b/me-trpo_amd/csrc/api.hip
@@ -476,7 +476,17 @@
     if (!c) return METRPO_ENULL;
     if (!obs || !ret || !tpath || !AtA || !Aty) return set_err(c, METRPO_ENULL, "gram: NULL pointer");
     if (N <= 0) return METRPO_OK;
-    return launch_gram(c, obs, ret, tpath, valid, N, AtA, Aty, (hipStream_t)stream);
+    return launch_gram(c, obs, ret, tpath, valid, N, AtA, Aty, nullptr, nullptr, (hipStream_t)stream);
+}
+
+extern "C" int32_t metrpo_baseline_gram_center(metrpo_ctx* c, const float* obs, const float* ret, const int32_t* tpath,
+                                               const uint8_t* valid, int64_t N, double* AtA, double* Aty, float* adv,
+                                               const double* stats, void* stream) {
+    TraceRange trace_("metrpo:process_samples:baseline_gram_center");
+    if (!c) return METRPO_ENULL;
+    if (!obs || !ret || !tpath || !AtA || !Aty || !adv || !stats) return set_err(c, METRPO_ENULL, "gram_center: NULL pointer");
+    if (N <= 0) return METRPO_OK;
+    return launch_gram(c, obs, ret, tpath, valid, N, AtA, Aty, adv, stats, (hipStream_t)stream);
 }
 
 extern "C" int32_t metrpo_baseline_solve(metrpo_ctx* c, const double* AtA, const double* Aty, double reg_coeff, double* coeffs, void* stream) {
diff --git a/me-trpo_amd/csrc/cg_device.h b/me-trpo_amd/csrc/cg_device.h
--- a/me-trpo_amd/csrc/cg_device.h
+++ b/me-trpo_amd/csrc/cg_device.h
@@ -5,6 +5,8 @@
 #endif
 
 enum { S_RDOTR = 0, S_DONE = 1, S_BETA = 2, S_XHX = 3, S_ITERS = 4, S_LOSS0 = 5, S_COMMERR = 6, S_ROLLERR = 7 };
+
+constexpr int LK_NSL = 32;
 
 struct CgTail {
     int op;
@@ -188,8 +190,7 @@
     if (threadIdx.x == 0) { scal[S_BETA] = beta; scal[S_XHX] = xhx; }
 }
 
-__device__ __forceinline__ void ls_decide(const CgTail& t) {
-    const double loss = t.lk[0], kl = t.lk[1], lb = t.scal[S_LOSS0];
+__device__ __forceinline__ void ls_decide(const CgTail& t, double loss, double kl, double lb) {
     if (loss < lb && kl <= t.max_kl) {
         const bool acc = !(isnan(loss) || isnan(kl) || loss >= lb || kl >= t.max_kl) || t.accept_violation != 0;
         if (acc) for (int i = threadIdx.x; i < t.P; i += blockDim.x) t.th[i] = t.th_try[i];
@@ -212,6 +213,12 @@
     if (threadIdx.x < 14) __hip_atomic_store(dst + threadIdx.x, src[threadIdx.x], __ATOMIC_RELAXED, __HIP_MEMORY_SCOPE_SYSTEM);
     asm volatile("s_waitcnt vmcnt(0)" ::: "memory");
     if (threadIdx.x == 0) __hip_atomic_store((unsigned long long*)(dst + 16), stamp, __ATOMIC_RELAXED, __HIP_MEMORY_SCOPE_SYSTEM);
+}
+
+__device__ __forceinline__ void cg_tail_ls(const CgTail& t, double loss, double kl, double lb) {
+    ls_decide(t, loss, kl, lb);
+    if (t.nx_try != nullptr && !(loss < lb && kl <= t.max_kl)) ls_next_theta(t);
+    if (t.pub_dst != nullptr) { asm volatile("s_waitcnt vmcnt(0)" ::: "memory"); __syncthreads(); ls_publish(t.scal, t.pub_dst, t.pub_stamp); }
 }
 
 __device__ __forceinline__ void cg_tail_run(const CgTail& t, double* sh, const CgPre* pre = nullptr) {
@@ -224,9 +231,5 @@
         }
     } else if (t.op == 2) { cg_finish_body(t.P, t.reg, t.max_kl, t.x, t.z, t.step, t.scal, sh); ls_open_and_first_theta(t); }
     else if (t.op == 3) cg_init_body(t.P, t.gout, t.x, t.r, t.p, PfOut{t.pf, t.vpos, t.imgval}, t.scal, sh);
-    else if (t.op == 4) {
-        ls_decide(t);
-        if (t.nx_try != nullptr && !(t.lk[0] < t.scal[S_LOSS0] && t.lk[1] <= t.max_kl)) ls_next_theta(t);
-        if (t.pub_dst != nullptr) { asm volatile("s_waitcnt vmcnt(0)" ::: "memory"); __syncthreads(); ls_publish(t.scal, t.pub_dst, t.pub_stamp); }
-    }
-}
+    else if (t.op == 4) cg_tail_ls(t, t.lk[0], t.lk[1], t.scal[S_LOSS0]);
+}
diff --git a/me-trpo_amd/csrc/metrpo_internal.h b/me-trpo_amd/csrc/metrpo_internal.h
--- a/me-trpo_amd/csrc/metrpo_internal.h
+++ b/me-trpo_amd/csrc/metrpo_internal.h
@@ -237,6 +237,7 @@
 int policy_mfma_select(const ProblemDesc& pd);
 int policy_mfma_image_buffers(metrpo_ctx*);
 int policy_mfma_launch(metrpo_ctx*, const UpdCall&, float* partials, int nblocks, hipStream_t);
+bool policy_mfma_reduces_itself(const metrpo_ctx*, const UpdCall&);
 
 #define HIP_TRY(c, expr)                                                                      \
     do {                                                                                      \
@@ -303,7 +304,7 @@
 int launch_sampler_progress(metrpo_ctx*, const uint8_t*, const int32_t*, int, int, int, long long, double*, double*, int32_t*, hipStream_t);
 int launch_baseline_solve(metrpo_ctx*, const double* AtA, const double* Aty, double reg, double* coeffs, hipStream_t);
 int launch_gram(metrpo_ctx*, const float*, const float*, const int32_t*, const uint8_t*, int64_t, double*, double*,
-                hipStream_t);
+                float* adv, const double* stats, hipStream_t);
 int launch_loss_grad(metrpo_ctx*, const metrpo_batch*, double*, hipStream_t, const CgTail* tail = nullptr, SolveScope = {});
 int launch_vpg_loss_grad(metrpo_ctx*, const metrpo_batch*, double* out, hipStream_t);
 int run_vpg_update(metrpo_ctx*, const metrpo_batch*, const metrpo_vpg_params*, double* d_loss, hipStream_t);
diff --git a/me-trpo_amd/csrc/policy_mfma.hip b/me-trpo_amd/csrc/policy_mfma.hip
--- a/me-trpo_amd/csrc/policy_mfma.hip
+++ b/me-trpo_amd/csrc/policy_mfma.hip
@@ -59,8 +59,47 @@
 };
 
 
-template <int NS, int NA, int PH, int MODE_>
-__device__ __forceinline__ void pol_body(const PolK& k, const float* __restrict__ theta, const float* __restrict__ v, float* __restrict__ partials) {
+template <int COL0, int STRIDE>
+__device__ __forceinline__ void losskl_fold_tail(const CgTail& t, const float* partials, double* lk) {
+    __shared__ unsigned int s_last;
+    __shared__ double fsh[LK_NSL][2];
+    asm volatile("s_waitcnt vmcnt(0)" ::: "memory");
+    __syncthreads();
+    if (threadIdx.x == 0) {
+        const unsigned int tk = __hip_atomic_fetch_add(t.ticket, 1u, __ATOMIC_RELAXED, __HIP_MEMORY_SCOPE_AGENT);
+        s_last = (tk == gridDim.x - 1) ? 1u : 0u;
+        if (s_last) __builtin_amdgcn_fence(__ATOMIC_ACQUIRE, "agent");
+    }
+    __syncthreads();
+    if (!s_last) return;
+    const int nrows = (int)gridDim.x;
+    const double lb = t.scal[S_LOSS0];
+    if (threadIdx.x < 2 * LK_NSL) {
+        const int lc = threadIdx.x & 1, sl = threadIdx.x >> 1;
+        const float* __restrict__ col = partials + COL0 + lc;
+        double a = 0.0;
+        constexpr int U = 16;
+        for (int b0 = sl; b0 < nrows; b0 += U * LK_NSL) {
+            float v[U];
+#pragma unroll
+            for (int u = 0; u < U; ++u) { const int b = b0 + u * LK_NSL; v[u] = __hip_atomic_load(col + (size_t)(b < nrows ? b : sl) * STRIDE, __ATOMIC_RELAXED, __HIP_MEMORY_SCOPE_AGENT); }
+#pragma unroll
+            for (int u = 0; u < U; ++u) if (b0 + u * LK_NSL < nrows) a += (double)v[u];
+        }
+        fsh[sl][lc] = a;
+    }
+    __syncthreads();
+    double loss = 0.0, kl = 0.0;
+    for (int w = 0; w < LK_NSL; ++w) { loss += fsh[w][0]; kl += fsh[w][1]; }
+    if (threadIdx.x == 0) { lk[0] = loss; lk[1] = kl; }
+    cg_tail_ls(t, loss, kl, lb);
+    if (threadIdx.x == 0) __hip_atomic_store(t.ticket, 0u, __ATOMIC_RELAXED, __HIP_MEMORY_SCOPE_AGENT);
+}
+
+template <int NS, int NA, int PH, int MODE_, bool FOLD = false>
+__device__ __forceinline__ void pol_body(const PolK& k, const float* __restrict__ theta, const float* __restrict__ v, float* __restrict__ partials,
+                                         const CgTail* ft = nullptr, double* lk = nullptr) {
+    static_assert(!FOLD || MODE_ == OP_LOSSKL, "only the loss / KL evaluation reduces its own rows");
     using I = PolImg<NS, NA, PH>;
     constexpr bool CACHED = (MODE_ == OP_FVPC), VPG = (MODE_ == OP_VPG), PPOKL = (MODE_ == OP_PPOKL), PPO = (MODE_ == OP_PPO) || PPOKL;
     constexpr int MODE = CACHED ? OP_FVP : (VPG || PPO) ? OP_GRAD : MODE_;
@@ -72,7 +111,10 @@
     extern __shared__ __attribute__((aligned(16))) float lds[];
     const int tid = threadIdx.x, lane = tid & 63, wave = __builtin_amdgcn_readfirstlane(tid >> 6);
     const int c = lane & 15, q = lane >> 4;
-    if (MODE_ == OP_LOSSKL && k.skip != nullptr && k.skip[0] >= 0.0) return;
+    if (MODE_ == OP_LOSSKL && k.skip != nullptr && k.skip[0] >= 0.0) {
+        if constexpr (FOLD) { if (ft->pub_dst != nullptr && blockIdx.x == 0) ls_publish(ft->scal, ft->pub_dst, ft->pub_stamp); }
+        return;
+    }
     float* IMG = lds;
     float* TL = lds + I::TOTAL + wave * WTL;
     PT_MARK(0)
@@ -608,9 +650,15 @@
         float a = 0.f;
 #pragma unroll
         for (int w = 0; w < NWAVES; w += 4) a += (RB[w * ROW + i] + RB[(w + 1) * ROW + i]) + (RB[(w + 2) * ROW + i] + RB[(w + 3) * ROW + i]);
-        out[i] = a;
+        if constexpr (FOLD) {
+#if !defined(__gfx942__) && !defined(__gfx950__) && defined(__HIP_DEVICE_COMPILE__)
+#error "the fence-free hand-over of the partial rows is written for gfx942 / gfx950 (sc1 write-through stores)"
+#endif
+            __hip_atomic_store(out + i, a, __ATOMIC_RELAXED, __HIP_MEMORY_SCOPE_AGENT);
+        } else out[i] = a;
     }
     PT_MARK(6)
+    if constexpr (FOLD) losskl_fold_tail<P, ROW>(*ft, partials, lk);
 }
 
 template <int NS, int NA, int PH, int MODE_>
@@ -622,6 +670,11 @@
     pol_body<NS, NA, PH, MODE_>(k, theta, v, partials);
 }
 
+
+template <int NS, int NA, int PH>
+__global__ void __launch_bounds__(NWAVES * 64, 1) k_policy_mfma_ls(PolK k, const float* __restrict__ theta, float* __restrict__ partials, CgTail tail, double* lk) {
+    pol_body<NS, NA, PH, OP_LOSSKL, true>(k, theta, nullptr, partials, &tail, lk);
+}
 
 template <int NS, int NA, int PH>
 static void pol_image_map(std::vector<int>& map) {
@@ -654,7 +707,8 @@
 }
 
 typedef void (*pol_kernel_t)(PolK, const float*, const float*, float*);
-struct PolEntry { int ns, na, ph; pol_kernel_t kern[7] ; int lds_floats, lds_floats_eval; void (*build_map)(std::vector<int>&); };
+typedef void (*pol_ls_kernel_t)(PolK, const float*, float*, CgTail, double*);
+struct PolEntry { int ns, na, ph; pol_kernel_t kern[7] ; int lds_floats, lds_floats_eval; void (*build_map)(std::vector<int>&); pol_ls_kernel_t kern_ls; };
 template <int NS, int NA, int PH> constexpr int pol_lds() {
     constexpr int HB = cdiv_(PH, 16);
     constexpr int a = PolImg<NS, NA, PH>::TOTAL + NWAVES * (3 * HB + (NA <= 2 ? 0 : 1)) * 16 * 20;
@@ -667,7 +721,7 @@
     constexpr int a = PolImg<NS, NA, PH>::TOTAL, b = NWAVES * (P + PART_EXTRA);
     return a > b ? a : b;
 }
-#define PENTRY(NS, NA, PH) {NS, NA, PH, {k_policy_mfma<NS, NA, PH, OP_GRAD>, k_policy_mfma<NS, NA, PH, OP_FVP>, k_policy_mfma<NS, NA, PH, OP_LOSSKL>, k_policy_mfma<NS, NA, PH, OP_FVPC>, k_policy_mfma<NS, NA, PH, OP_VPG>, k_policy_mfma<NS, NA, PH, OP_PPO>, k_policy_mfma<NS, NA, PH, OP_PPOKL>}, pol_lds<NS, NA, PH>(), pol_lds_eval<NS, NA, PH>(), pol_image_map<NS, NA, PH>}
+#define PENTRY(NS, NA, PH) {NS, NA, PH, {k_policy_mfma<NS, NA, PH, OP_GRAD>, k_policy_mfma<NS, NA, PH, OP_FVP>, k_policy_mfma<NS, NA, PH, OP_LOSSKL>, k_policy_mfma<NS, NA, PH, OP_FVPC>, k_policy_mfma<NS, NA, PH, OP_VPG>, k_policy_mfma<NS, NA, PH, OP_PPO>, k_policy_mfma<NS, NA, PH, OP_PPOKL>}, pol_lds<NS, NA, PH>(), pol_lds_eval<NS, NA, PH>(), pol_image_map<NS, NA, PH>, k_policy_mfma_ls<NS, NA, PH>}
 static const PolEntry kPol[] = {
     PENTRY(10, 2, 32),
     PENTRY(18, 6, 32),
@@ -707,6 +761,10 @@
     HIP_TRY(c, hipMemset(c->d_pol_imgval.p, 0, sizeof(float) * map.size()));
     c->pol_img_idx = idx;
     return METRPO_OK;
+}
+
+bool policy_mfma_reduces_itself(const metrpo_ctx* c, const UpdCall& u) {
+    return c->pol_mfma >= 0 && u.op == OP_LOSSKL && u.tail != nullptr && u.tail->op == 4 && c->xg_world <= 1 && !u.scope.exchange_in_tail && u.adam == nullptr;
 }
 
 int policy_mfma_launch(metrpo_ctx* c, const UpdCall& u, float* partials, int nblocks, hipStream_t st) {
@@ -726,6 +784,12 @@
     }
     size_t sh = sizeof(float) * (size_t)en.lds_floats;
     if (mode == OP_LOSSKL) sh = sizeof(float) * (size_t)en.lds_floats_eval;
+    if (policy_mfma_reduces_itself(c, u)) {
+        if (sh > 64 * 1024) HIP_TRY(c, hipFuncSetAttribute((const void*)en.kern_ls, hipFuncAttributeMaxDynamicSharedMemorySize, (int)sh));
+        hipLaunchKernelGGL(en.kern_ls, dim3(nblocks), dim3(NWAVES * 64), sh, st, k, u.theta, partials, *u.tail, u.out);
+        HIP_TRY(c, hipGetLastError());
+        return METRPO_OK;
+    }
     if (sh > 64 * 1024) HIP_TRY(c, hipFuncSetAttribute((const void*)en.kern[mode], hipFuncAttributeMaxDynamicSharedMemorySize, (int)sh));
     hipLaunchKernelGGL(en.kern[mode], dim3(nblocks), dim3(NWAVES * 64), sh, st, k, u.theta, u.vf, partials);
     HIP_TRY(c, hipGetLastError());
diff --git a/me-trpo_amd/csrc/policy_update.hip b/me-trpo_amd/csrc/policy_update.hip
--- a/me-trpo_amd/csrc/policy_update.hip
+++ b/me-trpo_amd/csrc/policy_update.hip
@@ -292,6 +292,7 @@
 }
 
 #define FIN_C 32
+static_assert(1024 / FIN_C == LK_NSL, "policy_mfma.hip's losskl_fold_tail adds the rows in k_finalize's slice order");
 #ifdef FIN_TIMING
 #define FT_MARK(i) { if (threadIdx.x == 0 && tail.op == 1 && blockIdx.x < 512) g_fin_phase[blockIdx.x][i] = __builtin_readcyclecounter(); }
 extern "C" int32_t metrpo_debug_fin_phases(unsigned long long* out) { return hipMemcpyFromSymbol(out, HIP_SYMBOL(g_fin_phase), sizeof(unsigned long long) * 4096) == hipSuccess ? 0 : -1; }
@@ -432,7 +433,7 @@
     return METRPO_OK;
 }
 
-struct PartRows { int rc, nrows, stride, lk_col; };
+struct PartRows { int rc, nrows, stride, lk_col; bool reduced = false;  };
 
 static void finalize(metrpo_ctx* c, const UpdCall& u, const PartRows& r, hipStream_t st) {
     const int mode = (u.op == OP_LOSSKL) ? 2 : (u.op == OP_FVP) ? 1 : 0;
@@ -496,7 +497,7 @@
 static PartRows run_mode(metrpo_ctx* c, const UpdCall& u, hipStream_t st) {
     const int P = c->pd.P;
     const long long tiles = (u.k.N + 15) / 16;
-    PartRows r = {METRPO_OK, 0, P + PART_EXTRA, P};
+    PartRows r; r.rc = METRPO_OK; r.nrows = 0; r.stride = P + PART_EXTRA; r.lk_col = P;
     const bool mfma = c->pol_mfma >= 0;
     if (mfma || f3_active(c, u.k.gm != nullptr)) {
         const long long per_block = (mfma ? 8ll : 4ll) * std::max(1, c->upd_tiles_per_wave);
@@ -504,6 +505,7 @@
         r.nrows = (int)std::max<long long>(1, std::min<long long>((tiles + per_block - 1) / per_block, max_blocks));
         const bool fvpc = mfma && u.scope.cache_activations && u.op == OP_FVP && u.k.gm == nullptr;
         c->upd_last = {mfma ? 1 : 3, fvpc ? (int)OP_FVPC : (int)u.op, mfma ? c->pol_mfma : -1, 0, r.nrows, 0, 0};
+        r.reduced = mfma && policy_mfma_reduces_itself(c, u);
         if (!(r.rc = ensure_partials(c, r.nrows)))
             r.rc = mfma ? policy_mfma_launch(c, u, c->d_partials.p, r.nrows, st) : policy_f3_launch(c, u, c->d_partials.p, r.nrows, st);
         return r;
@@ -529,7 +531,7 @@
     const PartRows r = run_mode(c, u, st);
     if (r.rc) return r.rc;
     if (timed) { HIP_TRY(c, hipEventRecord(c->fvp_ev[c->fvp_ev_n + 1], st)); c->fvp_ev_n += 2; }
-    finalize(c, u, r, st);
+    if (!r.reduced) finalize(c, u, r, st);
     HIP_TRY(c, hipGetLastError());
     return METRPO_OK;
 }
diff --git a/me-trpo_amd/csrc/process.hip b/me-trpo_amd/csrc/process.hip
--- a/me-trpo_amd/csrc/process.hip
+++ b/me-trpo_amd/csrc/process.hip
@@ -174,14 +174,20 @@
     }
 }
 
+__device__ __forceinline__ void center_scale(const double* __restrict__ stats, double& mean, double& inv) {
+    const double n = stats[2];
+    mean = stats[0] / n;
+    const double var = fmax(stats[1] / n - mean * mean, 0.0);
+    inv = 1.0 / (sqrt(var) + 1e-8);
+}
+__device__ __forceinline__ float center_one(float a, bool ok, double mean, double inv) { return ok ? (float)(((double)a - mean) * inv) : 0.0f; }
+
 __global__ void k_center(float* __restrict__ adv, const uint8_t* __restrict__ valid, int64_t N,
                          const double* __restrict__ stats) {
-    const double n = stats[2];
-    const double mean = stats[0] / n;
-    const double var = fmax(stats[1] / n - mean * mean, 0.0);
-    const double inv = 1.0 / (sqrt(var) + 1e-8);
+    double mean, inv;
+    center_scale(stats, mean, inv);
     for (int64_t i = (int64_t)blockIdx.x * blockDim.x + threadIdx.x; i < N; i += (int64_t)gridDim.x * blockDim.x)
-        adv[i] = (valid == nullptr || valid[i]) ? (float)(((double)adv[i] - mean) * inv) : 0.0f;
+        adv[i] = center_one(adv[i], valid == nullptr || valid[i], mean, inv);
 }
 
 #define GRAM_TILE 64
@@ -232,57 +238,65 @@
 }
 
 typedef float f32x4 __attribute__((ext_vector_type(4)));
-template <int NFB>
+#ifndef GRAM_PF_DEPTH
+#define GRAM_PF_DEPTH 3
+#endif
+template <int NFB, int D, bool CENTER>
 __global__ void __launch_bounds__(256) k_gram_mfma(const float* __restrict__ obs, const float* __restrict__ ret,
                                                    const int32_t* __restrict__ tpath, const uint8_t* __restrict__ valid,
-                                                   long long N, int ns, double* __restrict__ part) {
+                                                   long long N, int ns, double* __restrict__ part, float* adv, const double* __restrict__ stats) {
     extern __shared__ __attribute__((aligned(16))) double red[];
     constexpr int M = NFB * 16;
-    const int lane = threadIdx.x & 63, wave = threadIdx.x >> 6, c = lane & 15, q = lane >> 4;
+    const int lane = threadIdx.x & 63, wave = __builtin_amdgcn_readfirstlane(threadIdx.x >> 6), c = lane & 15, q = lane >> 4;
     const int F = 2 * ns + 4;
     double acc[NFB][NFB][4];
 #pragma unroll
     for (int a = 0; a < NFB; ++a)
 #pragma unroll
-        for (int b = 0; b < NFB; ++b)
+        for (int b = a; b < NFB; ++b)
 #pragma unroll
             for (int r = 0; r < 4; ++r) acc[a][b][r] = 0.0;
+    double mean = 0.0, inv = 0.0;
+    if (CENTER) center_scale(stats, mean, inv);
     const long long ntiles = (N + 15) / 16;
-    struct TileIn { float o[4][NFB]; float rv[4]; int tp[4]; int ok[4]; };
-    auto fetch = [&](long long tile, TileIn& in) {
+    struct TileIn { float o[4][NFB]; float rv[4]; int tp[4]; int ok[4]; float av; int vc; };
+    const uint8_t* __restrict__ vsrc = (valid != nullptr) ? valid : (const uint8_t*)tpath;
+    int fo[NFB];
+#pragma unroll
+    for (int cb = 0; cb < NFB; ++cb) { const int f = 16 * cb + c; fo[cb] = (f < ns) ? f : ((f < 2 * ns) ? f - ns : 0); }
+    auto fetch = [&](long long tile_, TileIn& in) {
+        const long long tile = (tile_ < ntiles) ? tile_ : ntiles - 1;
+        const long long n0 = tile * 16;
+        const int nrem = (int)((N - n0 < 16) ? N - n0 : 16);
+        const float* __restrict__ ob = obs + n0 * ns;
+        const float* __restrict__ rt = ret + n0;
+        const int32_t* __restrict__ tp = tpath + n0;
+        const uint8_t* __restrict__ vs = vsrc + n0;
 #pragma unroll
         for (int s = 0; s < 4; ++s) {
-            const long long n = tile * 16 + 4 * s + q;
-            const bool inr = tile < ntiles && n < N;
-            const long long nc = inr ? n : 0;
-            in.ok[s] = inr ? ((valid == nullptr) ? 1 : (int)valid[nc]) : 0;
-            in.tp[s] = tpath[nc];
-            in.rv[s] = ret[nc];
-#pragma unroll
-            for (int cb = 0; cb < NFB; ++cb) {
-                const int f = 16 * cb + c;
-                const int fo = (f < ns) ? f : ((f < 2 * ns) ? f - ns : 0);
-                in.o[s][cb] = obs[nc * ns + fo];
-            }
-        }
+            const int sl = 4 * s + q, slc = (sl < nrem) ? sl : nrem - 1;
+            in.ok[s] = (int)vs[slc];
+            in.tp[s] = tp[slc];
+            in.rv[s] = rt[slc];
+#pragma unroll
+            for (int cb = 0; cb < NFB; ++cb) in.o[s][cb] = ob[slc * ns + fo[cb]];
+        }
+        if (CENTER) { const int cl = (c < nrem) ? c : nrem - 1; in.av = adv[n0 + cl]; in.vc = (int)vs[cl]; }
     };
-    TileIn nxt;
-    fetch((long long)blockIdx.x * 4 + wave, nxt);
-    __builtin_amdgcn_s_waitcnt(0x0F70);
-    for (long long tile = (long long)blockIdx.x * 4 + wave; tile < ntiles; tile += (long long)gridDim.x * 4) {
-        const TileIn in = nxt;
-        fetch(tile + (long long)gridDim.x * 4, nxt);
-        asm volatile("" ::: "memory");
+    auto consume = [&](long long tile, const TileIn& in) {
+        const long long n0 = tile * 16;
+        const int nrem = (int)((N - n0 < 16) ? N - n0 : 16);
         f32x4 g[NFB][NFB];
 #pragma unroll
         for (int a = 0; a < NFB; ++a)
 #pragma unroll
-            for (int b = 0; b < NFB; ++b) g[a][b] = f32x4{0.f, 0.f, 0.f, 0.f};
+            for (int b = a; b < NFB; ++b) g[a][b] = f32x4{0.f, 0.f, 0.f, 0.f};
         float val[4][NFB];
 #pragma unroll
         for (int s = 0; s < 4; ++s) {
             const float al = (float)in.tp[s] / 100.0f;
             const float rv = in.rv[s];
+            const bool ok = (4 * s + q < nrem) && (valid == nullptr || in.ok[s] != 0);
 #pragma unroll
             for (int cb = 0; cb < NFB; ++cb) {
                 const int f = 16 * cb + c;
@@ -295,7 +309,7 @@
                 x = (kq == 3) ? 1.0f : x;
                 x = (f == F) ? rv : x;
                 x = (f > F) ? 0.0f : x;
-                val[s][cb] = in.ok[s] ? x : 0.0f;
+                val[s][cb] = ok ? x : 0.0f;
             }
         }
 #pragma unroll
@@ -303,21 +317,44 @@
 #pragma unroll
             for (int a = 0; a < NFB; ++a)
 #pragma unroll
-                for (int b = 0; b < NFB; ++b) g[a][b] = __builtin_amdgcn_mfma_f32_16x16x4f32(val[s][a], val[s][b], g[a][b], 0, 0, 0);
+                for (int b = a; b < NFB; ++b) g[a][b] = __builtin_amdgcn_mfma_f32_16x16x4f32(val[s][a], val[s][b], g[a][b], 0, 0, 0);
 #pragma unroll
         for (int a = 0; a < NFB; ++a)
 #pragma unroll
-            for (int b = 0; b < NFB; ++b)
+            for (int b = a; b < NFB; ++b)
 #pragma unroll
                 for (int r = 0; r < 4; ++r) acc[a][b][r] += (double)g[a][b][r];
+        if (CENTER) {
+            if (q == 0 && c < nrem) adv[n0 + c] = center_one(in.av, valid == nullptr || in.vc != 0, mean, inv);
+        }
+    };
+    const long long stride = (long long)gridDim.x * 4;
+    long long tile = (long long)blockIdx.x * 4 + wave;
+    TileIn ring[D];
+#pragma unroll
+    for (int d = 0; d < D; ++d) fetch(tile + d * stride, ring[d]);
+    __builtin_amdgcn_s_waitcnt(0x0F70);
+    while (tile < ntiles) {
+#pragma unroll
+        for (int d = 0; d < D; ++d) {
+            if (tile >= ntiles) break;
+            const TileIn in = ring[d];
+            fetch(tile + D * stride, ring[d]);
+            asm volatile("" ::: "memory");
+            consume(tile, in);
+            tile += stride;
+        }
     }
     double* mine = red + (size_t)wave * M * M;
 #pragma unroll
     for (int a = 0; a < NFB; ++a)
 #pragma unroll
-        for (int b = 0; b < NFB; ++b)
-#pragma unroll
-            for (int r = 0; r < 4; ++r) mine[(16 * a + 4 * q + r) * M + 16 * b + c] = acc[a][b][r];
+        for (int b = a; b < NFB; ++b)
+#pragma unroll
+            for (int r = 0; r < 4; ++r) {
+                mine[(16 * a + 4 * q + r) * M + 16 * b + c] = acc[a][b][r];
+                if (a != b) mine[(16 * b + c) * M + 16 * a + 4 * q + r] = acc[a][b][r];
+            }
     __syncthreads();
     const int nout = F * F + F;
     double* out = part + (size_t)blockIdx.x * nout;
@@ -469,7 +506,7 @@
 
 template <int NFB>
 static int launch_gram_mfma(metrpo_ctx* c, const float* obs, const float* ret, const int32_t* tpath, const uint8_t* valid,
-                            int64_t N, double* AtA, double* Aty, hipStream_t st) {
+                            int64_t N, double* AtA, double* Aty, float* adv, const double* stats, hipStream_t st) {
     constexpr int M = NFB * 16;
     const int F = 2 * c->pd.ns + 4;
     const long long tiles = (N + 15) / 16;
@@ -477,8 +514,10 @@
     const size_t need = (size_t)g * (F * F + F);
     { const int rc = ws_grow(c, c->d_gram_part, need * sizeof(double)); if (rc) return rc; }
     const size_t sh = sizeof(double) * 4 * M * M;
-    if (sh > 64 * 1024) HIP_TRY(c, hipFuncSetAttribute((const void*)k_gram_mfma<NFB>, hipFuncAttributeMaxDynamicSharedMemorySize, (int)sh));
-    hipLaunchKernelGGL(k_gram_mfma<NFB>, dim3(g), dim3(256), sh, st, obs, ret, tpath, valid, (long long)N, c->pd.ns, c->d_gram_part.p);
+    const void* kfn = adv ? (const void*)k_gram_mfma<NFB, GRAM_PF_DEPTH, true> : (const void*)k_gram_mfma<NFB, GRAM_PF_DEPTH, false>;
+    if (sh > 64 * 1024) HIP_TRY(c, hipFuncSetAttribute(kfn, hipFuncAttributeMaxDynamicSharedMemorySize, (int)sh));
+    if (adv) hipLaunchKernelGGL((k_gram_mfma<NFB, GRAM_PF_DEPTH, true>), dim3(g), dim3(256), sh, st, obs, ret, tpath, valid, (long long)N, c->pd.ns, c->d_gram_part.p, adv, stats);
+    else hipLaunchKernelGGL((k_gram_mfma<NFB, GRAM_PF_DEPTH, false>), dim3(g), dim3(256), sh, st, obs, ret, tpath, valid, (long long)N, c->pd.ns, c->d_gram_part.p, (float*)nullptr, (const double*)nullptr);
     const int nout = F * F + F;
     hipLaunchKernelGGL(k_gram_final, dim3((nout + 15) / 16), dim3(1024), 0, st, c->d_gram_part.p, g, M, F, AtA, Aty);
     HIP_TRY(c, hipGetLastError());
@@ -650,12 +689,13 @@
 }
 
 int launch_gram(metrpo_ctx* c, const float* obs, const float* ret, const int32_t* tpath, const uint8_t* valid,
-                int64_t N, double* AtA, double* Aty, hipStream_t st) {
+                int64_t N, double* AtA, double* Aty, float* adv, const double* stats, hipStream_t st) {
     const int F = 2 * c->pd.ns + 4;
     const int nfb = (F + 1 + 15) / 16;
-    if (nfb <= 2) return launch_gram_mfma<2>(c, obs, ret, tpath, valid, N, AtA, Aty, st);
-    if (nfb == 3) return launch_gram_mfma<3>(c, obs, ret, tpath, valid, N, AtA, Aty, st);
-    if (nfb == 4) return launch_gram_mfma<4>(c, obs, ret, tpath, valid, N, AtA, Aty, st);
+    if (nfb <= 2) return launch_gram_mfma<2>(c, obs, ret, tpath, valid, N, AtA, Aty, adv, stats, st);
+    if (nfb == 3) return launch_gram_mfma<3>(c, obs, ret, tpath, valid, N, AtA, Aty, adv, stats, st);
+    if (nfb == 4) return launch_gram_mfma<4>(c, obs, ret, tpath, valid, N, AtA, Aty, adv, stats, st);
+    if (adv) { const int rc = launch_center(c, adv, valid, N, stats, st); if (rc) return rc; }
     if (nfb == 5) return launch_gram_mfma_wide<5>(c, obs, ret, tpath, valid, N, AtA, Aty, st);
     if (nfb == 6) return launch_gram_mfma_wide<6>(c, obs, ret, tpath, valid, N, AtA, Aty, st);
     if (nfb == 7) return launch_gram_mfma_wide<7>(c, obs, ret, tpath, valid, N, AtA, Aty, st);
diff --git a/me-trpo_amd/engine.py b/me-trpo_amd/engine.py
--- a/me-trpo_amd/engine.py
+++ b/me-trpo_amd/engine.py
@@ -422,6 +422,15 @@
                                            _ptr(AtA), _ptr(Aty), self._stream()))
         return AtA, Aty
 
+    def baseline_gram_center(self, obs, ret, tpath, valid, adv, stats, out=None):
+        F = 2 * self.ns + 4
+        if out is None:
+            out = torch.zeros(F * F + F, dtype=torch.float64, device=self.device)
+        AtA, Aty = out[:F * F].view(F, F), out[F * F:]
+        self._chk(lib.metrpo_baseline_gram_center(self._ctx, _ptr(obs), _ptr(ret), _ptr(tpath), _ptr(valid), ret.numel(),
+                                                  _ptr(AtA), _ptr(Aty), _ptr(adv), _ptr(stats), self._stream()))
+        return AtA, Aty
+
     def baseline_solve(self, gram, reg_coeff=1e-5, out=None):
         F = 2 * self.ns + 4
         assert gram.is_cuda and gram.dtype == torch.float64 and gram.numel() == F * F + F and gram.is_contiguous()
diff --git a/me-trpo_amd/sampler.py b/me-trpo_amd/sampler.py
--- a/me-trpo_amd/sampler.py
+++ b/me-trpo_amd/sampler.py
@@ -48,14 +48,18 @@
         comm.allreduce_sum_(stats)
         static = (eng.env_name != 'ant') and (tr.T % tr.H == 0)
         n_global = comm.world * tr.T * tr.B if static and self._uniform_B(comm, tr.B) else int(stats[2].item())
-        if algo.center_adv:
+        fused_center = algo.center_adv and not algo.positive_adv
+        if algo.center_adv and not fused_center:
             eng.center_advantages(adv, valid, stats)
         if algo.positive_adv:
             lo = torch.where(valid.bool(), adv, torch.full_like(adv, float('inf'))).min().reshape(1)
             comm.allreduce_min_(lo)
             adv.sub_(lo).add_(1e-8)
         gram = acc[3:]
-        eng.baseline_gram(tr.obs, ret, tr.tpath, valid, out=gram)
+        if fused_center:
+            eng.baseline_gram_center(tr.obs, ret, tr.tpath, valid, adv, stats, out=gram)
+        else:
+            eng.baseline_gram(tr.obs, ret, tr.tpath, valid, out=gram)
         comm.allreduce_sum_(gram)
         if getattr(algo, 'device_baseline_fit', False) and gram.is_cuda and hasattr(algo.baseline, 'solve_device'):
             algo.baseline.solve_device(eng, gram)
```

Measured after the change: 1.954 billion (median of 6 runs). No clear change (+0.3%).
